# SamsungLabs/imvoxelnet

Hardware: AMD Instinct MI355X
Metric: images/sec/node (KITTI 3x384x1280, 216x248x12 vox) (higher is better)
Workload: dtype f32 (fp16 (hi, lo) pair MFMA operands: the Winograd-domain neck GEMMs and the chained 2-D trunk); 1 GPU; kitti_mono_1x3x384x1280_vox216x248x12_resnet50_fpn64_kittineck_anchor3dhead; batch_per_gpu=4, global_batch=4, parallelism=dp1, api=ImVoxelNet.simple_test(img, img_metas), detections_last_step=64

## Files before the change

imvoxelnet_amd/_lib.py:

```python
import ctypes as C
import os

_HERE = os.path.dirname(os.path.abspath(__file__))
LIB_PATH = os.environ.get('IVX_LIB_PATH') or os.path.join(_HERE, 'csrc', 'libimvoxel_hip.so')
_lib = None


class IvxError(RuntimeError):
    pass


class ConvDesc(C.Structure):
    _fields_ = [(n, C.c_int32) for n in
                ('B', 'D', 'H', 'W', 'Cin', 'Cout', 'KD', 'KH', 'KW', 'sd', 'sh', 'sw', 'pd', 'ph', 'pw',
                 'relu', 'res_mode', 'res_h', 'res_w', 'wgt_layout', 'out_mode', 'res_after_act')] + [('post_scale', C.c_float),
                                                                  ('in_dtype', C.c_int32), ('out_dtype', C.c_int32), ('res_scale', C.c_float),
                                                                  ('wino_operands', C.c_int32)]


class ConvRouteOpts(C.Structure):
    _fields_ = [(n, C.c_int32) for n in ('winograd', 'winograd_tile', 'wino_operands', 'split')] + [('winograd_min_pos', C.c_int64), ('winograd_2d_min_ch', C.c_int32)]


class ConvRoute(C.Structure):
# ... 22 lines not shown
                ('sampling', C.c_int32)]


SAMPLING = {'nearest': 0, 'bilinear': 1}


def sampling_id(sampling):
    try:
        return SAMPLING[sampling]
    except (KeyError, TypeError):
        raise ValueError(f"sampling must be 'nearest' or 'bilinear', got {sampling!r}") from None


class BackprojectDesc(C.Structure):
    _fields_ = [(n, C.c_int32) for n in ('B', 'V', 'FH', 'FW', 'C', 'X', 'Y', 'Z')] + [('voxel_size', C.c_float * 3)] + \
               [(n, C.c_int32) for n in ('feat_dtype', 'mode', 'sampling', 'first')]


class LiftLists(C.Structure):
    _fields_ = [('S', C.c_int32), ('R', C.c_int32), ('view_slot', C.c_void_p), ('row', C.c_void_p), ('first', C.c_void_p)]


class PairIO(C.Structure):
    _fields_ = [('in_scale', C.c_void_p), ('res_scale', C.c_void_p), ('res_dtype', C.c_int32), ('out_scale', C.c_void_p), ('amax_in', C.c_void_p),
                ('amax_res', C.c_void_p), ('amax_out', C.c_void_p), ('wbound', C.c_float), ('sbound', C.c_float)]


class BottleneckDesc(C.Structure):
    _fields_ = [(n, C.c_int32) for n in ('B', 'H', 'W', 'P')]


class BottleneckIO(C.Structure):
    _fields_ = [('in_scale', C.c_void_p), ('amax_in', C.c_void_p), ('out_scale', C.c_void_p), ('amax_out', C.c_void_p), ('wbound', C.c_float * 3),
                ('sbound', C.c_float * 3)]


class SampleMeta(C.Structure):
    _fields_ = [('intrinsic', C.c_float * 16), ('extrinsics', C.c_void_p), ('origin', C.c_float * 3), ('img_h', C.c_int32), ('img_w', C.c_int32),
                ('ori_h', C.c_int32)]


class IndoorTailDesc(C.Structure):
    _fields_ = [('B', C.c_int32), ('n_levels', C.c_int32), ('k', C.c_int32 * 4), ('n_classes', C.c_int32), ('n_reg', C.c_int32),
                ('use_rotate_nms', C.c_int32), ('max_num', C.c_int32), ('score_thr', C.c_float), ('nms_thr', C.c_float)]


class TraceRec(C.Structure):
    _fields_ = [('step', C.c_int32), ('stage', C.c_int32), ('is3d', C.c_int32), ('ms', C.c_float), ('start_ms', C.c_float), ('flops', C.c_double),
                ('bytes', C.c_double), ('name', C.c_char * 48)]


class PlanInfo(C.Structure):
    _fields_ = [(n, C.c_int64) for n in ('cam_bytes', 'arena', 'ws_off', 'ws_bytes', 'ws2_off', 'ws2_bytes', 'total', 'scal_off', 'scal_bytes')] + \
               [(n, C.c_int32) for n in ('slot_bytes', 'n_sides', 's0', 's1', 'n_steps', 'n_tensors')]


class PlanStep(C.Structure):
    _fields_ = [(n, C.c_int32) for n in ('kind', 'in_', 'res', 'out', 'out2', 'fuse_out', 'fuse', 'side', 'join', 'tile', 'pio', 'amax_n', 'amax_in_n',
                                         'n_extra_in', 'n_extra_out')] + \
               [('extra_in', C.c_int32 * 12), ('extra_out', C.c_int32 * 4)] + \
               [(n, C.c_int64) for n in ('split', 'ws', 'amax_out', 'amax_in')] + [('name', C.c_char * 48)]


class PlanTensor(C.Structure):
    _fields_ = [(n, C.c_int64) for n in ('off', 'bytes', 'used', 'slot')] + \
               [(n, C.c_int32) for n in ('first', 'last', 'fmt', 'esz', 'caller_owned', 'boundary')]


class ImagePrepDesc(C.Structure):
    _fields_ = [(n, C.c_int32) for n in ('src_h', 'src_w', 'src_row_bytes', 'dst_h', 'dst_w', 'pad_h', 'pad_w', 'to_rgb')] + \
               [('mean', C.c_float * 3), ('std', C.c_float * 3)]


def declare_plan_view(L):
    key = [C.c_void_p, C.c_char_p, C.c_int32, C.c_int32, C.c_int32, C.c_int32]
    L.ivx_model_plan_info.argtypes = key + [C.POINTER(PlanInfo)]
    L.ivx_model_plan_step.argtypes = key + [C.c_int32, C.POINTER(PlanStep)]
    L.ivx_model_plan_tensor.argtypes = key + [C.c_int32, C.POINTER(PlanTensor)]


EXPORTS = ['ivx_model_plan_info', 'ivx_model_plan_step', 'ivx_model_plan_tensor', 'ivx_bottleneck_proj_supported', 'ivx_bottleneck_proj_pack', 'ivx_bottleneck_proj_fwd_pio', 'ivx_anchor_head_decode', 'ivx_fcos3d_head_decode', 'ivx_nms_rotated_bev', 'ivx_nms_aligned3d', 'ivx_bottleneck_supported', 'ivx_bottleneck_fwd_pio', 'ivx_amax_f32', 'ivx_stem_pool_filter_bytes', 'ivx_stem_pool_pack_filters', 'ivx_stem_pool_out_dims', 'ivx_stem_pool_fwd_pair', 'ivx_conv_winograd_set_variant', 'ivx_ubench_mfma', 'ivx_ubench_copy', 'ivx_version', 'ivx_last_error', 'ivx_conv_out_dims', 'ivx_conv_fwd', 'ivx_conv_fwd_naive', 'ivx_conv_set_tile_override', 'ivx_conv_set_epilogue_mode', 'ivx_conv_set_plan_mode', 'ivx_topk_set_mode', 'ivx_conv_workspace_bytes', 'ivx_conv_fwd_ws', 'ivx_conv_set_halo_mode', 'ivx_bf16_pair_split', 'ivx_f16_pair_split', 'ivx_conv_pair_supported', 'ivx_bf16_pair_pack_filters', 'ivx_conv_route', 'ivx_conv_pio_workspace_bytes', 'ivx_conv_fwd_pio', 'ivx_conv_fwd_pio_naive', 'ivx_pair_pack_filters', 'ivx_nchw_to_nhwc_amax', 'ivx_maxpool2d_fwd_pair', 'ivx_f16_pair_merge', 'ivx_model_calibrate_fp8', 'ivx_model_calibrate_fp8_ex', 'ivx_amax_bf16', 'ivx_conv_winograd_output_blocks', 'ivx_conv_winograd_issued_fraction', 'ivx_conv_winograd_output_amax', 'ivx_conv_winograd_input_amax', 'ivx_conv_winograd_fused_supported', 'ivx_conv_winograd_fused_blocks', 'ivx_conv_winograd_gemm_output_amax',
           'ivx_conv_winograd_bg_supported', 'ivx_conv_winograd_bg_bytes', 'ivx_conv_winograd_bg_layer_offset', 'ivx_conv_winograd_bg_plan',
           'ivx_conv_winograd_input_bg', 'ivx_conv_winograd_gemm_bg', 'ivx_conv_winograd_output_bg',
           'ivx_conv_winograd_supported', 'ivx_conv_winograd_weight_elems', 'ivx_conv_winograd_weights', 'ivx_conv_winograd_workspace_bytes',
           'ivx_conv_winograd_input', 'ivx_conv_winograd_gemm', 'ivx_conv_winograd_output', 'ivx_conv_winograd_fwd',
           'ivx_maxpool2d_fwd', 'ivx_maxpool2d_fwd_bf16', 'ivx_maxpool2d_fwd_fp8', 'ivx_global_avgpool_fwd', 'ivx_global_avgpool_fwd_bf16', 'ivx_upsample_trilinear2x_fwd', 'ivx_dcn_im2col_fwd', 'ivx_dcn_im2col_fwd_bf16', 'ivx_dcn_im2col_fwd_pair', 'ivx_nchw_to_nhwc', 'ivx_image_s2d_bf16', 'ivx_nhwc_to_nchw', 'ivx_backproject_mean_fwd', 'ivx_backproject_mean_fwd_amax', 'ivx_backproject_amax_blocks', 'ivx_backproject_mean_fwd_bf16', 'ivx_upsample_trilinear2x_fwd_bf16', 'ivx_backproject_sum_fwd', 'ivx_volume_normalize_fwd',
           'ivx_backproject_accum_fwd', 'ivx_backproject_accum_fwd_bf16', 'ivx_volume_mean_fwd', 'ivx_backproject_fwd_ex', 'ivx_backproject_gather_fwd',
           'ivx_backproject_lists_fwd',
           'ivx_anchor_head_workspace_bytes', 'ivx_anchor_head_get_bboxes', 'ivx_fcos_head_workspace_bytes',
           'ivx_fcos_head_level_candidates', 'ivx_nms_workspace_bytes',
           'ivx_nms_bev', 'ivx_boxes_overlap_bev', 'ivx_aligned_3d_nms', 'ivx_aligned_3d_nms_workspace_bytes', 'ivx_aligned_3d_nms_ws', 'ivx_multiclass_nms_workspace_bytes', 'ivx_multiclass_nms_bev',
           'ivx_create', 'ivx_destroy', 'ivx_weights_load', 'ivx_weights_finalize', 'ivx_model_workspace_bytes', 'ivx_model_forward',
           'ivx_backbone_fpn_workspace_bytes', 'ivx_backbone_fpn_fwd', 'ivx_neck3d_workspace_bytes', 'ivx_neck3d_out_dims',
           'ivx_neck3d_kitti_fwd', 'ivx_neck3d_nuscenes_fwd', 'ivx_neck3d_levels', 'ivx_neck3d_fast_fwd', 'ivx_neck3d_unet_fwd',
           'ivx_model_forward_levels', 'ivx_model_anchors', 'ivx_compute_projection', 'ivx_voxel_new_origin', 'ivx_fold_batchnorm',
           'ivx_model_trace', 'ivx_model_trace_count', 'ivx_model_trace_read',
           'ivx_model_detect_workspace_bytes', 'ivx_model_max_detections', 'ivx_model_detect', 'ivx_layout_head_decode', 'ivx_layout_extrinsics',
           'ivx_indoor_tail_workspace_bytes', 'ivx_indoor_tail_get_bboxes',
           'ivx_rescale_size', 'ivx_image_prep_u8',
           'ivx_kitti_image_box_overlap', 'ivx_kitti_compute_statistics', 'ivx_kitti_collect_scores', 'ivx_kitti_fused_statistics']


def lib():
    global _lib
    if _lib is not None:
        return _lib
    if not os.path.exists(LIB_PATH):
        raise IvxError(f'{LIB_PATH} is missing: build it with `python -m imvoxelnet_amd._build` '
                       '(or __graft_entry__.build()).  There is no CPU fallback.')
    L = C.CDLL(LIB_PATH)
    vp, i32, i64, f32 = C.c_void_p, C.c_int32, C.c_int64, C.c_float
    L.ivx_version.restype = C.c_int
    L.ivx_last_error.restype = C.c_char_p
    L.ivx_conv_out_dims.argtypes = [C.POINTER(ConvDesc), C.POINTER(i32), C.POINTER(i32), C.POINTER(i32)]
    for name in ('ivx_conv_fwd', 'ivx_conv_fwd_naive'):
        getattr(L, name).argtypes = [C.POINTER(ConvDesc), vp, vp, vp, vp, vp, vp, vp]
    L.ivx_conv_set_tile_override.argtypes = [C.c_int]
    L.ivx_conv_set_halo_mode.argtypes = [C.c_int]
    L.ivx_conv_set_epilogue_mode.argtypes = [C.c_int]
    L.ivx_conv_set_plan_mode.argtypes = [C.c_int]
    L.ivx_conv_winograd_output_blocks.argtypes = [C.POINTER(ConvDesc), i32]
    L.ivx_conv_winograd_output_blocks.restype = i32
    L.ivx_conv_winograd_output_amax.argtypes = [C.POINTER(ConvDesc), i32, vp, vp, vp, vp, vp, i64, vp, vp]
    L.ivx_conv_winograd_input_amax.argtypes = [C.POINTER(ConvDesc), i32, vp, vp, i64, vp, i32, vp]
    L.ivx_conv_winograd_fused_supported.argtypes = [C.POINTER(ConvDesc), i32]
    L.ivx_conv_winograd_fused_blocks.argtypes = [C.POINTER(ConvDesc), i32]
    L.ivx_conv_winograd_fused_blocks.restype = i32
    L.ivx_conv_winograd_gemm_output_amax.argtypes = [C.POINTER(ConvDesc), i32, vp, vp, vp, vp, vp, vp, i64, vp, vp]
    L.ivx_conv_winograd_bg_supported.argtypes = [C.POINTER(ConvDesc), i32]
    L.ivx_conv_winograd_bg_bytes.argtypes = [C.POINTER(ConvDesc), i32]
    L.ivx_conv_winograd_bg_bytes.restype = i64
    L.ivx_conv_winograd_bg_layer_offset.argtypes = [C.POINTER(ConvDesc), i32]
    L.ivx_conv_winograd_bg_layer_offset.restype = i64
    L.ivx_conv_winograd_bg_plan.argtypes = [C.POINTER(ConvDesc), vp, i32, C.POINTER(i32), vp, i64, vp]
    L.ivx_conv_winograd_input_bg.argtypes = [C.POINTER(ConvDesc), i32, vp, vp, i64, vp, i32, vp, vp]
    L.ivx_conv_winograd_gemm_bg.argtypes = [C.POINTER(ConvDesc), i32, vp, vp, i64, vp, vp]
    L.ivx_conv_winograd_output_bg.argtypes = [C.POINTER(ConvDesc), i32, vp, vp, vp, vp, vp, i64, vp, vp, vp]
    L.ivx_bf16_pair_split.argtypes = [vp, i64, vp, vp]
    L.ivx_f16_pair_split.argtypes = [vp, i64, f32, vp, vp]
    L.ivx_conv_pair_supported.argtypes = [C.POINTER(ConvDesc)]
    L.ivx_bf16_pair_pack_filters.argtypes = [vp, i32, i32, i32, i32, vp]
    L.ivx_conv_route.argtypes = [C.POINTER(ConvDesc), i32, C.POINTER(ConvRouteOpts), C.POINTER(ConvRoute)]
    L.ivx_conv_pio_workspace_bytes.argtypes = [C.POINTER(ConvDesc), C.POINTER(PairIO)]
    L.ivx_conv_pio_workspace_bytes.restype = i64
    L.ivx_amax_f32.argtypes = [vp, i64, vp, vp]
    L.ivx_stem_pool_filter_bytes.restype = i64
    L.ivx_stem_pool_filter_bytes.argtypes = []
    L.ivx_stem_pool_pack_filters.argtypes = [vp, vp, vp, vp]
    L.ivx_stem_pool_out_dims.argtypes = [i32, i32, C.POINTER(i32), C.POINTER(i32)]
    L.ivx_stem_pool_fwd_pair.argtypes = [vp, i32, i32, i32, vp, vp, vp, f32, f32, vp, vp, vp, vp, vp]
    L.ivx_bottleneck_supported.argtypes = [C.POINTER(BottleneckDesc)]
    L.ivx_bottleneck_fwd_pio.argtypes = [C.POINTER(BottleneckDesc), C.POINTER(BottleneckIO)] + [vp] * 12
    L.ivx_bottleneck_proj_supported.argtypes = [C.POINTER(BottleneckDesc), i32]
    L.ivx_bottleneck_proj_pack.argtypes = [vp, vp, vp, vp, vp, vp, i32, i32, vp, vp, vp, C.POINTER(f32), C.POINTER(f32), C.POINTER(f32)]
    L.ivx_bottleneck_proj_fwd_pio.argtypes = [C.POINTER(BottleneckDesc), i32, C.POINTER(BottleneckIO), f32] + [vp] * 12
    L.ivx_conv_fwd_pio.argtypes = [C.POINTER(ConvDesc), C.POINTER(PairIO), vp, vp, vp, vp, vp, vp, vp, i64, vp]
    L.ivx_conv_fwd_pio_naive.argtypes = [C.POINTER(ConvDesc), C.POINTER(PairIO), vp, vp, vp, vp, vp, vp, vp]
    L.ivx_pair_pack_filters.argtypes = [vp, i32, i32, i32, vp, vp, vp, vp, C.POINTER(f32), C.POINTER(f32)]
    L.ivx_nchw_to_nhwc_amax.argtypes = [vp, i32, i32, i64, i32, vp, vp, vp]
    L.ivx_maxpool2d_fwd_pair.argtypes = [vp, i32, i32, i32, i32, i32, i32, i32, vp, vp, f32, f32, vp, vp, vp]
    L.ivx_f16_pair_merge.argtypes = [vp, i64, vp, vp, vp]
    L.ivx_conv_workspace_bytes.argtypes = [C.POINTER(ConvDesc)]
    L.ivx_conv_workspace_bytes.restype = i64
    L.ivx_conv_fwd_ws.argtypes = [C.POINTER(ConvDesc), vp, vp, vp, vp, vp, vp, vp, i64, vp]
    D = C.POINTER(ConvDesc)
    L.ivx_conv_winograd_supported.argtypes = [D, i32]
    L.ivx_conv_winograd_issued_fraction.argtypes = [D]
    L.ivx_conv_winograd_issued_fraction.restype = C.c_float
    L.ivx_conv_winograd_weight_elems.argtypes = [D, i32]
    L.ivx_conv_winograd_weight_elems.restype = i64
    L.ivx_conv_winograd_weights.argtypes = [D, i32, vp, vp, vp]
    L.ivx_conv_winograd_workspace_bytes.argtypes = [D, i32]
    L.ivx_conv_winograd_workspace_bytes.restype = i64
    L.ivx_conv_winograd_input.argtypes = [D, i32, vp, vp, i64, vp]
    L.ivx_conv_winograd_gemm.argtypes = [D, i32, vp, vp, i64, vp]
    L.ivx_conv_winograd_output.argtypes = [D, i32, vp, vp, vp, vp, vp, i64, vp]
    L.ivx_conv_winograd_fwd.argtypes = [D, i32, vp, vp, vp, vp, vp, vp, vp, i64, vp]
    L.ivx_maxpool2d_fwd.argtypes = [vp, i32, i32, i32, i32, i32, i32, i32, vp, vp]
    L.ivx_global_avgpool_fwd.argtypes = [vp, i32, i64, i32, vp, vp]
    L.ivx_global_avgpool_fwd_bf16.argtypes = [vp, i32, i64, i32, vp, vp]
    L.ivx_upsample_trilinear2x_fwd.argtypes = [vp, i32, i32, i32, i32, i32, vp, vp]
    L.ivx_dcn_im2col_fwd.argtypes = [vp, vp] + [i32] * 10 + [vp, vp]
    L.ivx_dcn_im2col_fwd_bf16.argtypes = [vp, vp] + [i32] * 10 + [vp, vp]
    L.ivx_dcn_im2col_fwd_pair.argtypes = [vp, vp, vp] + [i32] * 10 + [vp, vp, vp, vp]
    L.ivx_nchw_to_nhwc.argtypes = [vp, i32, i32, i64, i32, vp, vp]
    L.ivx_nhwc_to_nchw.argtypes = [vp, i32, i64, i32, vp, vp]
    L.ivx_rescale_size.argtypes = [i32, i32, i32, i32, C.POINTER(i32), C.POINTER(i32)]
    L.ivx_image_prep_u8.argtypes = [C.POINTER(ImagePrepDesc), vp, i64, i32, vp, vp]
    L.ivx_backproject_mean_fwd.argtypes = [vp, i32, i32, i32, i32, i32, vp, vp, vp, C.POINTER(f32), i32, i32, i32,
                                           vp, vp, vp]
    L.ivx_backproject_sum_fwd.argtypes = L.ivx_backproject_mean_fwd.argtypes
    L.ivx_backproject_mean_fwd_bf16.argtypes = L.ivx_backproject_mean_fwd.argtypes
    L.ivx_upsample_trilinear2x_fwd_bf16.argtypes = [vp, i32, i32, i32, i32, i32, vp, vp]
    L.ivx_volume_normalize_fwd.argtypes = [vp, vp, i64, i32, vp, vp]
    L.ivx_backproject_accum_fwd.argtypes = [vp, i32, i32, i32, i32, i32, vp, vp, vp, C.POINTER(f32), i32, i32, i32, vp, vp, i32, vp, vp, vp]
    L.ivx_backproject_accum_fwd_bf16.argtypes = L.ivx_backproject_accum_fwd.argtypes
    L.ivx_volume_mean_fwd.argtypes = [vp, vp, i64, i32, vp, i32, vp, vp]
    if hasattr(L, 'ivx_backproject_fwd_ex'):
        L.ivx_backproject_fwd_ex.argtypes = [C.POINTER(BackprojectDesc), vp, vp, vp, vp, vp, vp, vp, vp, vp]
    if hasattr(L, 'ivx_backproject_gather_fwd'):
        L.ivx_backproject_gather_fwd.argtypes = [C.POINTER(BackprojectDesc), i32, vp, vp, vp, vp, vp, vp, vp, vp]
    if hasattr(L, 'ivx_backproject_lists_fwd'):
        L.ivx_backproject_lists_fwd.argtypes = [C.POINTER(BackprojectDesc), C.POINTER(LiftLists), vp, vp, vp, vp, vp, vp, vp, vp, vp]
    L.ivx_anchor_head_workspace_bytes.argtypes = [C.POINTER(AnchorHeadDesc)]
    L.ivx_anchor_head_workspace_bytes.restype = i64
    L.ivx_anchor_head_get_bboxes.argtypes = [C.POINTER(AnchorHeadDesc), vp, vp, vp, i64, vp, vp, vp, vp, vp, vp, vp, vp]
    L.ivx_fcos_head_workspace_bytes.argtypes = [i32, i32, i32]
    L.ivx_fcos_head_workspace_bytes.restype = i64
    L.ivx_fcos_head_level_candidates.argtypes = [vp, vp, vp, vp, f32] + [i32] * 12 + [vp, i64, vp, vp, vp, vp]
    L.ivx_nms_workspace_bytes.argtypes = [i32]
    L.ivx_nms_workspace_bytes.restype = i64
    L.ivx_nms_bev.argtypes = [vp, i32, f32, i32, vp, i64, vp, vp, vp]
    L.ivx_boxes_overlap_bev.argtypes = [vp, i32, vp, i32, i32, vp, vp]
    L.ivx_aligned_3d_nms.argtypes = [vp, vp, vp, i32, f32, vp, vp, vp]
    L.ivx_aligned_3d_nms_workspace_bytes.argtypes = [i32]
    L.ivx_aligned_3d_nms_workspace_bytes.restype = i64
    L.ivx_aligned_3d_nms_ws.argtypes = [vp, vp, vp, i32, f32, vp, i64, vp, vp, vp]
    L.ivx_multiclass_nms_workspace_bytes.argtypes = [i32, i32]
    L.ivx_multiclass_nms_workspace_bytes.restype = i64
    L.ivx_multiclass_nms_bev.argtypes = [vp, vp, i32, i32, i32, f32, f32, i32, i32, vp, i64, vp, vp, vp, vp]
# ... 59 lines not shown
```

imvoxelnet_amd/csrc/api_common.cpp:

```cpp
#include <stdarg.h>
#include <stdio.h>
#include <string.h>

#include "../../include/imvoxel.h"

static thread_local char g_err[512] = "";

void ivx_set_error(const char *fmt, ...) {
  va_list ap;
  va_start(ap, fmt);
  vsnprintf(g_err, sizeof(g_err), fmt, ap);
  va_end(ap);
}

extern "C" int ivx_version(void) { return 470;  }
extern "C" const char *ivx_last_error(void) { return g_err; }

extern "C" __attribute__((weak)) int ivx_dcn_im2col_fwd_bf16(const void *, const float *, int32_t, int32_t, int32_t, int32_t, int32_t, int32_t, int32_t,
                                                             int32_t, int32_t, int32_t, void *, ivx_stream_t) {
  ivx_set_error("ivx_dcn_im2col_fwd_bf16: bf16 storage is not available in this build");
  return IVX_ERR_UNSUPPORTED;
}
extern "C" __attribute__((weak)) int ivx_global_avgpool_fwd_bf16(const void *, int32_t, int64_t, int32_t, float *, ivx_stream_t) {
  ivx_set_error("ivx_global_avgpool_fwd_bf16: bf16 storage is not available in this build");
  return IVX_ERR_UNSUPPORTED;
}

extern "C" __attribute__((weak)) int ivx_backproject_fwd_ex(const ivx_backproject_desc *, const void *, const float *, const float *, const int32_t *, void *,
                                                            int32_t *, void *, uint8_t *, ivx_stream_t) {
  ivx_set_error("ivx_backproject_fwd_ex: bilinear sampling is not available in this build");
  return IVX_ERR_UNSUPPORTED;
}

extern "C" int ivx_anchor_head_decode(const ivx_anchor_head_desc *d, const float *head_out, const float *anchors, void *workspace, int64_t workspace_bytes,
                                      float *out_boxes, float *out_scores, int64_t *out_labels, int32_t *out_count, int64_t *cand_idx, float *cand_boxes,
                                      float *cand_scores, ivx_stream_t stream) {
  return ivx_anchor_head_get_bboxes(d, head_out, anchors, workspace, workspace_bytes, out_boxes, out_scores, out_labels, out_count, cand_idx, cand_boxes,
                                    cand_scores, stream);
}
extern "C" int ivx_fcos3d_head_decode(const float *head_out, const uint8_t *valid0, const float *level_vs, const float *level_new_origin, float scale,
                                      int32_t B, int32_t nx, int32_t ny, int32_t nz, int32_t CH, int32_t n_classes, int32_t n_reg, int32_t level, int32_t X,
                                      int32_t Y, int32_t Z, int32_t nms_pre, void *workspace, int64_t workspace_bytes, float *cand_boxes,
                                      float *cand_scores, int32_t *cand_count, ivx_stream_t stream) {
  return ivx_fcos_head_level_candidates(head_out, valid0, level_vs, level_new_origin, scale, B, nx, ny, nz, CH, n_classes, n_reg, level, X, Y, Z, nms_pre,
                                        workspace, workspace_bytes, cand_boxes, cand_scores, cand_count, stream);
}
extern "C" int ivx_nms_rotated_bev(const float *boxes_sorted, int32_t n, float thresh, void *workspace, int64_t workspace_bytes, int64_t *keep,
                                   int32_t *num_out, ivx_stream_t stream) {
  return ivx_nms_bev(boxes_sorted, n, thresh, 1, workspace, workspace_bytes, keep, num_out, stream);
}
extern "C" int ivx_nms_aligned3d(const float *boxes, const float *scores, const int64_t *classes, int32_t n, float thresh, int64_t *pick,
                                 int32_t *num_out, ivx_stream_t stream) {
  return ivx_aligned_3d_nms(boxes, scores, classes, n, thresh, pick, num_out, stream);
}

static const int WINO_MIN_CH = 64;
static const int WINO_2D_MIN_CH = 128;
static const int64_t WINO_MIN_POS = 2000;
static const int64_t WINO_TILE6_MIN_PLANE = 16384;
static const int SPLIT_MIN_COUT = 64;
static const int64_t SPLIT_MIN_POS = 256;
static const int WINO_OVER_PAIR_MIN_CH = 256;
static const int64_t WINO_OVER_PAIR_MIN_POS = 200000;

static int32_t wino_operands(const ivx_conv_desc *d, int32_t cin_real, const ivx_conv_route_opts *o, int tile) {
  return tile >= 4 && o->wino_operands == IVX_F16_PAIR && cin_real % (d->wgt_layout == 1 ? 32 : 16) == 0 ? IVX_F16_PAIR : 0;
}

extern "C" int ivx_conv_route(const ivx_conv_desc *d, int32_t cin_real, const ivx_conv_route_opts *o, ivx_conv_route_out *r) {
  if (!d || !o || !r) {
    ivx_set_error("ivx_conv_route: null argument");
    return IVX_ERR_INVALID_ARG;
  }
  memset(r, 0, sizeof(*r));
  r->run = *d;
  const bool f32 = d->in_dtype == IVX_F32 && d->out_dtype == IVX_F32 && d->Cin == cin_real;
  const bool wino2d = d->KD == 1 && d->KH == 3 && d->KW == 3 && d->sd == 1 && d->sh == 1 && d->sw == 1;
  const bool wino3d = d->KD == 3 && d->KH == 3 && d->sd == 1 && d->sh == 1;
  const int min_ch = !wino2d ? WINO_MIN_CH : o->winograd_2d_min_ch > 0 ? o->winograd_2d_min_ch : WINO_2D_MIN_CH;
  r->wino_candidate = f32 && (wino2d || wino3d) && d->Cout % 4 == 0 && cin_real % 4 == 0 && (cin_real >= min_ch || d->Cout >= min_ch);
  r->split_candidate = f32 && o->split && o->wino_operands == IVX_F16_PAIR && d->KD == 3 && d->KH == 3 && d->KW == 3 && cin_real % 32 == 0 &&
                       d->Cout >= SPLIT_MIN_COUT;
  ivx_conv_desc w = *d;
  if (r->wino_candidate && wino2d) {
    w.D = d->H; w.H = d->W; w.W = d->B > 0 ? 1 : 0;
    w.KD = 3; w.KH = 3; w.KW = 1;
    w.pd = d->ph; w.ph = d->pw; w.pw = 0;
  }
  if (d->B <= 0) {
    r->run = w;
    r->run.wino_operands = wino_operands(d, cin_real, o, o->winograd_tile);
    return IVX_OK;
  }
  const int64_t npos = (int64_t)d->B * d->D * d->H * d->W;
  r->prefers_winograd = r->wino_candidate && wino2d && o->winograd && o->wino_operands == IVX_F16_PAIR && cin_real >= WINO_OVER_PAIR_MIN_CH &&
                        d->Cout >= WINO_OVER_PAIR_MIN_CH && cin_real % 32 == 0 && npos >= WINO_OVER_PAIR_MIN_POS;
  if (r->wino_candidate && o->winograd && (d->res_mode == 0 || d->res_mode == 1) &&
      npos >= (o->winograd_min_pos >= 0 ? o->winograd_min_pos : WINO_MIN_POS)) {
// ... 58 lines not shown
```

imvoxelnet_amd/csrc/model.cpp:

```cpp
#include <hip/hip_runtime_api.h>
#include <math.h>
#include <stdarg.h>
#include <string.h>

#include <algorithm>
#include <cstdlib>
#include <map>
#include <memory>
#include <string>
#include <vector>

#include "../../include/imvoxel.h"
#include "../../include/imvoxel_lab.h"

void ivx_set_error(const char *fmt, ...);

extern "C" {
__attribute__((weak)) int ivx_conv_winograd_bg_supported(const ivx_conv_desc *d, int32_t tile);
__attribute__((weak)) int64_t ivx_conv_winograd_bg_bytes(const ivx_conv_desc *d, int32_t n_layers);
__attribute__((weak)) int64_t ivx_conv_winograd_bg_layer_offset(const ivx_conv_desc *d, int32_t layer);
__attribute__((weak)) int ivx_conv_winograd_bg_plan(const ivx_conv_desc *d, const uint8_t *valid, int32_t n_layers, const int32_t *out_slices, void *block,
                                                    int64_t block_bytes, ivx_stream_t stream);
__attribute__((weak)) int ivx_conv_winograd_input_bg(const ivx_conv_desc *d, int32_t tile, const void *in, void *workspace, int64_t workspace_bytes,
                                                     const float *partials, int32_t n_partials, const int32_t *bg, ivx_stream_t stream);
__attribute__((weak)) int ivx_conv_winograd_gemm_bg(const ivx_conv_desc *d, int32_t tile, const float *u, void *workspace, int64_t workspace_bytes,
                                                    const int32_t *bg, ivx_stream_t stream);
__attribute__((weak)) int ivx_conv_winograd_output_bg(const ivx_conv_desc *d, int32_t tile, const float *scale, const float *shift, const void *res,
                                                      void *out, void *workspace, int64_t workspace_bytes, float *partials, const int32_t *bg,
                                                      ivx_stream_t stream);
}

#define M_REQUIRE(cond, ...)        \
  do {                              \
    if (!(cond)) {                  \
      ivx_set_error(__VA_ARGS__);   \
      return IVX_ERR_INVALID_ARG;   \
    }                               \
  } while (0)
#define M_HIP(call, what)                                                        \
  do {                                                                           \
    hipError_t e_ = (call);                                                      \
    if (e_ != hipSuccess) {                                                      \
      ivx_set_error("%s: %s", what, hipGetErrorString(e_));                      \
      return IVX_ERR_HIP;                                                        \
    }                                                                            \
  } while (0)
#define M_TRY(call)                 \
  do {                              \
    int rc_ = (call);               \
    if (rc_ != IVX_OK) return rc_;  \
  } while (0)

namespace {

inline int64_t align256(int64_t v) { return (v + 255) / 256 * 256; }

inline uint16_t f32_to_f16_bits(float f) {
  uint32_t x;
  memcpy(&x, &f, 4);
  const uint32_t sign = (x >> 16) & 0x8000u, ax = x & 0x7fffffffu;
  if (ax >= 0x7f800000u) return (uint16_t)(sign | (ax > 0x7f800000u ? 0x7e00u : 0x7c00u));
  if (ax < 0x38800000u) {
    float a;
    memcpy(&a, &ax, 4);
    const float r = a * 16777216.0f;
    return (uint16_t)(sign | (uint32_t)lrintf(r));
  }
  const uint32_t mant = ax & 0x7fffffu, exp = (ax >> 23) - 127 + 15;
  uint32_t h = (exp << 10) | (mant >> 13);
  const uint32_t rem = mant & 0x1fffu;
  if (rem > 0x1000u || (rem == 0x1000u && (h & 1u))) ++h;
  return (uint16_t)(sign | h);
}
inline uint16_t f32_to_bf16_bits(float f) {
  uint32_t x;
  memcpy(&x, &f, 4);
  if ((x & 0x7fffffffu) > 0x7f800000u) return (uint16_t)((x >> 16) | 0x40u);
  x += 0x7fffu + ((x >> 16) & 1u);
  return (uint16_t)(x >> 16);
}
inline float f16_bits_to_f32(uint16_t h) {
  const uint32_t sign = (uint32_t)(h & 0x8000u) << 16, e = (h >> 10) & 31u, m = h & 0x3ffu;
  float f;
  if (e == 0) {
    f = (float)m * 5.9604644775390625e-08f;
    uint32_t x;
    memcpy(&x, &f, 4);
    x |= sign;
    memcpy(&f, &x, 4);
    return f;
  }
  const uint32_t x = sign | (e == 31 ? 0x7f800000u | (m << 13) : ((e - 15 + 127) << 23) | (m << 13));
  memcpy(&f, &x, 4);
  return f;
}

struct HostTensor {
  std::vector<int64_t> shape;
  std::vector<float> data;
};

struct ConvLayer {
  std::string name;
  int dims = 3;
  int cin = 0, cout = 0;
  int k[3] = {1, 1, 1}, s[3] = {1, 1, 1}, p[3] = {0, 0, 0};
  bool relu = false;
  bool conv_t = false;
  bool dcn_cols = false;
  int cout_zero = 0;
  bool linear = false;
  std::vector<std::string> w_keys;
  std::vector<std::string> b_keys;
  std::string bn;
  int cin_pad = 0, layout = 0;
  bool wino_cand = false, identity_epilogue = true;
  float *w = nullptr, *w0 = nullptr, *scale = nullptr, *shift = nullptr;
  std::map<int, float *> u;
  bool stem_s2d = false;
  bool out_f32 = false;
  bool f32 = false;
  int fp8_role = 0;
  int stage = -1;
  int fp8_eff = 0;
  std::vector<float> w_tap, scale_h, shift_h;
  float *wq = nullptr, *scale_q = nullptr, *shift_q = nullptr;
  int layout_q = 0;
  double out_scale_q = 1.0;
  bool pair_ok = false;
  float *wpair = nullptr, *scale_p = nullptr;
  bool split_cand = false;
  float *wsplit = nullptr;
  float wbound = 0.f, sbound = 0.f;
  int proj_peer = -1;
  bool proj_keep = false;
  float *wproj = nullptr, *scale_proj = nullptr, *shift_proj = nullptr;
  float proj_wb3 = 0.f, proj_sb = 0.f, proj_wbd = 0.f;
  float *wstem = nullptr;
};

enum StepKind { ST_IMG2CL, ST_IMG_S2D, ST_CONV, ST_MAXPOOL, ST_LIFT, ST_TAIL, ST_UPSAMPLE, ST_DCN_COL, ST_AVGPOOL, ST_LAYOUT, ST_FCOS, ST_INDOOR_TAIL };

struct Step {
  StepKind kind;
  int layer = -1;
  int in = -1, res = -1, out = -1, out2 = -1;
  int res_mode = 0;
  int res_after_act = 0;
  float post_scale = 1.0f;
  int aux = 0;
};

struct TInfo {
  int B = 0, D = 0, H = 0, W = 0, C = 0;
  int64_t bytes = 0, off = -1;
  int first = -1, last = -1;
  bool raw = false;
  int esz = 4;
  int fmt = 0;
  int64_t slot = -1;
  int64_t elems() const { return (int64_t)B * D * H * W * C; }
};

struct PlanStep {
  ivx_conv_desc d;
  int tile = 0;
  int64_t ws = 0;
  int64_t amax_out = -1, amax_in = -1;
  int amax_n = 0, amax_in_n = 0;
  int pio = 0;
  int64_t split = 0;
  int bound_layer = -1;
  int fuse = 0, fuse_out = -1;
  int side = 0, join = 0;
  int64_t bg = -1;
};

struct Plan {
  std::vector<TInfo> t;
  std::vector<PlanStep> ps;
  int64_t arena = 0, ws_off = 0, ws_bytes = 0, tail_ws = 0, total = 0;
  ivx_anchor_head_desc tail;
  int64_t cam_bytes = 0, cam_proj = 0, cam_origin = 0, cam_crop = 0, cam_lvl_vs[3] = {0, 0, 0}, cam_lvl_no[3] = {0, 0, 0};
  int n_views = 1;
  ivx_indoor_tail_desc itail;
  int max_det = 0;
  int64_t scal_off = 0, scal_bytes = 0;
  int64_t ws2_off = 0, ws2_bytes = 0;
  int n_sides = 0;
  int s0 = 0, s1 = 0;
  int bg_first = -1, bg_layers = 0;
  int64_t bg_off = -1, bg_bytes = 0;
  int32_t bg_zo[9] = {0, 0, 0, 0, 0, 0, 0, 0, 0};
};

}

struct ivx_model {
  ivx_model_cfg cfg;
  std::vector<ConvLayer> layers;
  std::vector<Step> steps;
  int n_tensors = 0;
  int trunk0 = 0, trunk1 = 0, lift_step = -1, neck0 = 0, neck1 = 0, head_step = -1, tail_step = -1;
  int t_img = -1, t_fpn0 = -1, t_volume = -1, t_valid = -1, t_neck = -1, t_head = -1;
  std::vector<int> t_levels;
  int head0 = -1;
  std::vector<int> t_headout, t_cb, t_cs, t_cc;
  float head_scales[3] = {1.f, 1.f, 1.f};
  int t_c5 = -1, t_angle = -1, t_layout = -1, layout_step = -1;
  std::vector<std::vector<char>> cam_ring;
  size_t cam_next = 0;
  std::map<std::string, HostTensor> weights;
  bool finalized = false;
  std::vector<float> anchors_host;
  int anchors_h = 0, anchors_w = 0;
  float *anchors_dev = nullptr;
  size_t anchors_cap = 0;
  std::vector<float> anchors_given;
  std::map<std::string, std::unique_ptr<Plan>> plans;
  std::vector<void *> owned;
  std::vector<float> pack_a, pack_b;
  bool fp8_on = false;
  float *calib_dev = nullptr;
  bool trace_on = false;
  bool trace_skip = false;
  int trace_level = 2;
  struct TraceRec {
    int step, stage, is3d; double flops, bytes; hipEvent_t e0, e1; std::string name;
    const int32_t *rows_dev = nullptr;
    double rows_dense = 0.0;
  };
  std::vector<TraceRec> trace;
  std::vector<hipEvent_t> event_pool;
  size_t events_used = 0;
  hipStream_t side = nullptr;
  hipEvent_t ev_fork = nullptr;
  std::vector<hipEvent_t> ev_join;
};

namespace {

int new_tensor(ivx_model *m) { return m->n_tensors++; }

int add_conv(ivx_model *m, ConvLayer L, int in, int res = -1, int res_mode = 0) {
  m->layers.push_back(std::move(L));
  Step s;
  s.kind = ST_CONV;
  s.layer = (int)m->layers.size() - 1;
  s.in = in;
  s.res = res;
  s.res_mode = res >= 0 ? (res_mode ? res_mode : 1) : 0;
  s.out = new_tensor(m);
  m->steps.push_back(s);
  return s.out;
}

ConvLayer conv2d(const std::string &name, int cin, int cout, int k, int stride, int pad, bool relu, const std::string &w,
                 const std::string &b, const std::string &bn) {
  ConvLayer L;
  L.name = name; L.dims = 2; L.cin = cin; L.cout = cout;
  L.k[0] = 1; L.k[1] = k; L.k[2] = k;
  L.s[0] = 1; L.s[1] = stride; L.s[2] = stride;
  L.p[0] = 0; L.p[1] = pad; L.p[2] = pad;
  L.relu = relu; L.w_keys = {w}; L.b_keys = {b}; L.bn = bn;
  return L;
}

ConvLayer conv3d(const std::string &name, int cin, int cout, const int s[3], const int p[3], bool relu, const std::string &w,
                 const std::string &b, const std::string &bn) {
  ConvLayer L;
  L.name = name; L.dims = 3; L.cin = cin; L.cout = cout;
  for (int a = 0; a < 3; ++a) { L.k[a] = 3; L.s[a] = s[a]; L.p[a] = p[a]; }
  L.relu = relu; L.w_keys = {w}; L.b_keys = {b}; L.bn = bn;
  return L;
}

// ... 791 lines not shown
      if (!(pl->ps[i].pio && pl->ps[i + 1].pio && pl->ps[i + 2].pio) || s1.res >= 0 || s2.res >= 0 || s2.in != s1.out || s3.in != s2.out ||
          s3.res != s1.in || s3.res_mode != 1 || s3.res_after_act || s3.post_scale != 1.0f)
        continue;
      if (!is1x1(L1) || !is1x1(L3) || !(L2.k[0] == 1 && L2.k[1] == 3 && L2.k[2] == 3 && L2.s[1] == 1 && L2.s[2] == 1 && L2.p[1] == 1 && L2.p[2] == 1) ||
          L2.dcn_cols || !L1.relu || !L2.relu || !L3.relu || L1.cin != 4 * P || L2.cin != P || L2.cout != P || L3.cin != P || L3.cout != 4 * P)
        continue;
      if (x.fmt != IVX_F16_PAIR || y1.fmt != IVX_F16_PAIR || y2.fmt != IVX_F16_PAIR || o.fmt != IVX_F16_PAIR || x.D != 1 || x.slot < 0 || o.slot < 0 ||
          y1.last != i + 1 || y2.last != i + 2)
        continue;
      ivx_bottleneck_desc bd = {x.B, x.H, x.W, P};
      if (!ivx_bottleneck_supported(&bd)) continue;
      pl->ps[i].fuse = 1; pl->ps[i].fuse_out = s3.out;
      pl->ps[i + 1].fuse = pl->ps[i + 2].fuse = 2;
      pl->t[s3.out].first = i;
      i += 2;
    }
  static const bool side_on = !(getenv("IVX_SIDE_STREAM") && atoi(getenv("IVX_SIDE_STREAM")) == 0);
  if (side_on && c.with_trunk)
    for (int i = std::max(r.s0, m->trunk0); i + 2 < std::min(r.s1, m->trunk1); ++i) {
      const Step &s0 = m->steps[i];
      if (s0.kind != ST_CONV || pl->ps[i].tile != 0 || pl->ps[i].fuse != 0 || s0.res >= 0) continue;
      const std::string &nm = m->layers[s0.layer].name;
      if (nm.size() < 10 || nm.compare(nm.size() - 10, 10, "downsample") != 0) continue;
      int j = -1;
      for (int k = i + 1; k < std::min(r.s1, m->trunk1) && k <= i + 6; ++k)
        if (m->steps[k].res == s0.out) { j = k; break; }
      if (j < 0 || j < i + 2) continue;
      bool ok = true;
      for (int k = i + 1; k < j && ok; ++k) ok = m->steps[k].in != s0.out && m->steps[k].res != s0.out && pl->ps[k].side == 0 && pl->ps[k].join == 0;
      if (!ok) continue;
      pl->ps[i].side = pl->ps[j].join = ++pl->n_sides;
      pl->t[s0.in].last = std::max(pl->t[s0.in].last, j);
    }
  std::vector<int> keep = {m->t_fpn0, m->t_volume, m->t_valid, m->t_neck, m->t_head, m->t_angle, m->t_layout};
  keep.insert(keep.end(), m->t_levels.begin(), m->t_levels.end());
  for (int t : keep)
    if (t >= 0 && pl->t[t].first >= r.s0) pl->t[t].last = r.s1;
  struct Blk { int64_t off, size; };
  std::vector<Blk> free_list;
  int64_t top = 0;
  {
    const TInfo &vol = pl->t[m->t_volume];
    const int Bs = vol.B > 0 ? vol.B : 1;
    auto take = [&](int64_t bytes) { const int64_t at = top; top += align256(bytes); return at; };
    pl->n_views = n_views;
    pl->cam_proj = take((int64_t)Bs * n_views * 12 * 4);
    pl->cam_origin = take((int64_t)Bs * 3 * 4);
    pl->cam_crop = take((int64_t)Bs * 2 * 4);
    for (int l = 0; l < 3; ++l) { pl->cam_lvl_vs[l] = take((int64_t)Bs * 3 * 4); pl->cam_lvl_no[l] = take((int64_t)Bs * 3 * 4); }
    pl->cam_bytes = top;
  }
  auto release = [&](int64_t off, int64_t size) {
    free_list.push_back({off, size});
    std::sort(free_list.begin(), free_list.end(), [](const Blk &a, const Blk &b) { return a.off < b.off; });
    std::vector<Blk> merged;
    for (const Blk &b : free_list) {
      if (!merged.empty() && merged.back().off + merged.back().size == b.off) merged.back().size += b.size;
      else merged.push_back(b);
    }
    free_list.swap(merged);
  };
  for (int i = r.s0; i < r.s1; ++i) {
    const Step &s = m->steps[i];
    const int extra = s.kind == ST_FCOS ? m->t_cc[s.aux] : pl->ps[i].fuse_out;
    for (int t : {s.out, s.out2, extra}) {
      if (t < 0 || pl->t[t].first != i) continue;
      TInfo &ti = pl->t[t];
      bool placed = false;
      for (size_t f = 0; f < free_list.size(); ++f)
        if (free_list[f].size >= ti.bytes) {
          ti.off = free_list[f].off;
          free_list[f].off += ti.bytes; free_list[f].size -= ti.bytes;
          if (free_list[f].size == 0) free_list.erase(free_list.begin() + f);
          placed = true;
          break;
        }
      if (!placed) { ti.off = top; top += ti.bytes; }
    }
    for (int t = 0; t < m->n_tensors; ++t) {
      TInfo &ti = pl->t[t];
      if (ti.off >= 0 && ti.first >= r.s0 && ti.last == i && ti.first != -2) release(ti.off, ti.bytes);
    }
  }
  for (int i = r.s0; i < r.s1; ++i) {
    const Step &s = m->steps[i];
    PlanStep &pc = pl->ps[i];
    if (s.kind != ST_CONV || pc.tile == 0 || pc.d.wino_operands != IVX_F16_PAIR) continue;
    for (int j = i - 1; j >= r.s0; --j) {
      const Step &q = m->steps[j];
      if (q.out != s.in) continue;
      PlanStep &pp = pl->ps[j];
      if (q.kind == ST_LIFT && m->cfg.sampling == IVX_SAMPLE_NEAREST) {
        const TInfo &vol = pl->t[q.out];
        const int32_t nb = ivx_backproject_amax_blocks(vol.B, n_views, vol.D, vol.H, vol.W);
        if (nb > 0) {
          if (pp.amax_out < 0) { pp.amax_out = top; pp.amax_n = nb; top += align256((int64_t)nb * 4); }
          pc.amax_in = pp.amax_out;
          pc.amax_in_n = pp.amax_n;
        }
      }
      if (q.kind == ST_CONV && pp.tile > 0) {
        if (pp.amax_out < 0) {
          const int32_t nb = ivx_conv_winograd_output_blocks(&pp.d, pp.tile);
          M_REQUIRE(nb > 0, "layer %s: %s", m->layers[q.layer].name.c_str(), ivx_last_error());
          pp.amax_out = top;
          pp.amax_n = nb;
          top += align256((int64_t)nb * 4);
        }
        pc.amax_in = pp.amax_out;
        pc.amax_in_n = pp.amax_n;
      }
      break;
    }
  }
  const bool bg_on = !(getenv("IVX_NECK_BACKGROUND") && atoi(getenv("IVX_NECK_BACKGROUND")) == 0);
  if (bg_on && ivx_conv_winograd_bg_plan && ivx_conv_winograd_bg_supported && m->lift_step >= r.s0 && m->lift_step < r.s1 && c.storage == IVX_F32) {
    std::vector<int> chain_t = {m->steps[m->lift_step].out};
    std::vector<int> chain_s;
    for (int i = m->lift_step + 1; i < r.s1 && (int)chain_s.size() < 9; ++i) {
      const Step &s = m->steps[i];
      const PlanStep &ps = pl->ps[i];
      if (s.kind != ST_CONV || s.in != chain_t.back() || ps.tile != 6 || !ivx_conv_winograd_bg_supported(&ps.d, ps.tile)) break;
      if (s.res >= 0 && (s.res_mode != 1 || std::find(chain_t.begin(), chain_t.end(), s.res) == chain_t.end())) break;
      if (!chain_s.empty()) {
        const ivx_conv_desc &d0 = pl->ps[chain_s[0]].d;
        if (ps.d.B != d0.B || ps.d.D != d0.D || ps.d.H != d0.H) break;
      }
      int32_t xo, yo, zo;
      M_TRY(ivx_conv_out_dims(&ps.d, &xo, &yo, &zo));
      pl->bg_zo[chain_s.size()] = zo;
      chain_s.push_back(i);
      chain_t.push_back(s.out);
    }
    if (!chain_s.empty()) {
      const ivx_conv_desc &d0 = pl->ps[chain_s[0]].d;
      pl->bg_first = chain_s[0];
      pl->bg_layers = (int)chain_s.size();
      pl->bg_bytes = ivx_conv_winograd_bg_bytes(&d0, pl->bg_layers);
      M_REQUIRE(pl->bg_bytes > 0, "background plan: %s", ivx_last_error());
      top = align256(top);
      pl->bg_off = top;
      top += align256(pl->bg_bytes);
      for (size_t l = 0; l < chain_s.size(); ++l) pl->ps[chain_s[l]].bg = pl->bg_off + ivx_conv_winograd_bg_layer_offset(&d0, (int32_t)l);
    }
  }
  if (n_slots > 0) {
    top = align256(top);
    pl->scal_off = top;
    pl->scal_bytes = (int64_t)n_slots * 512;
    top += pl->scal_bytes;
  }
  pl->arena = align256(top);
  pl->ws_off = pl->arena;
  pl->ws_bytes = align256(pl->ws_bytes);
  pl->total = pl->arena + pl->ws_bytes;
  if (pl->n_sides > 0) {
    for (int i = r.s0; i < r.s1; ++i)
      if (pl->ps[i].side > 0) pl->ws2_bytes = std::max(pl->ws2_bytes, pl->ps[i].ws);
    pl->ws2_bytes = align256(pl->ws2_bytes);
    pl->ws2_off = pl->total;
    pl->total += pl->ws2_bytes;
  }
  return IVX_OK;
}

std::string plan_key(const char *what, int B, int V, int H, int W) {
  char buf[96];
  snprintf(buf, sizeof(buf), "%s:%d:%d:%d:%d", what, B, V, H, W);
  return buf;
}

TInfo tinfo(int B, int D, int H, int W, int C, int esz = 4) {
  TInfo t; t.B = B; t.D = D; t.H = H; t.W = W; t.C = C; t.esz = esz; t.bytes = align256(t.elems() * esz);
  return t;
}

int get_plan(ivx_model *m, const char *what, Range r, int B, int V, int H, int W, const std::map<int, TInfo> &inputs, Plan **out,
             hipStream_t stream) {
  M_REQUIRE(m->finalized, "%s: call ivx_weights_finalize first", what);
  const std::string key = plan_key(what, B, V, H, W);
  auto it = m->plans.find(key);
  if (it == m->plans.end()) {
    std::unique_ptr<Plan> pl(new Plan());
    M_TRY(make_plan(m, r, inputs, V, pl.get(), stream));
    it = m->plans.emplace(key, std::move(pl)).first;
  }
  *out = it->second.get();
  return IVX_OK;
}

struct Bind {
  std::map<int, void *> ext;
  const float *proj = nullptr, *new_origin = nullptr;
  const int32_t *crop = nullptr;
  int V = 1;
  float *boxes = nullptr, *scores = nullptr;
  int64_t *labels = nullptr;
  int32_t *count = nullptr;
  const float *lvl_vs[3] = {nullptr, nullptr, nullptr}, *lvl_no[3] = {nullptr, nullptr, nullptr};
  const ivx_sample_meta *metas = nullptr;
  float *proj_dev = nullptr;
  float *angles_host = nullptr, *layout_host = nullptr;
};

int trace_begin(ivx_model *m, int step, int stage, int is3d, double flops, double bytes, const std::string &name, hipStream_t st) {
  if (!m->trace_on) return IVX_OK;
  m->trace_skip = m->trace_level == 3 && stage != 2;
  if (m->trace_skip) return IVX_OK;
  while (m->event_pool.size() < m->events_used + 2) {
    hipEvent_t e;
    M_HIP(hipEventCreate(&e), "hipEventCreate");
    m->event_pool.push_back(e);
  }
  ivx_model::TraceRec r{step, stage, is3d, flops, bytes, m->event_pool[m->events_used], m->event_pool[m->events_used + 1], name};
  m->events_used += 2;
  M_HIP(hipEventRecord(r.e0, st), "hipEventRecord");
  m->trace.push_back(r);
  return IVX_OK;
}

int trace_end(ivx_model *m, hipStream_t st) {
  if (!m->trace_on || m->trace_skip) return IVX_OK;
  M_HIP(hipEventRecord(m->trace.back().e1, st), "hipEventRecord");
  return IVX_OK;
}

int ensure_anchors(ivx_model *m, const ivx_anchor_head_desc &d, hipStream_t st, const char *who) {
  if (m->anchors_h == d.H && m->anchors_w == d.W && m->anchors_dev) return IVX_OK;
  const size_t n = (size_t)d.H * d.W * d.num_anchors * 7;
  if (!m->anchors_given.empty()) {
    M_REQUIRE(m->anchors_given.size() == n, "%s: the loaded anchors have %zu values, the %d x %d grid needs %zu", who, m->anchors_given.size(),
              d.H, d.W, n);
    m->anchors_host = m->anchors_given;
  } else {
    make_anchors(m->cfg, d.H, d.W, &m->anchors_host);
  }
  M_HIP(hipStreamSynchronize(st), "hipStreamSynchronize (anchors)");
  if (m->anchors_dev && m->anchors_cap < n) {
    auto it = std::find(m->owned.begin(), m->owned.end(), (void *)m->anchors_dev);
    if (it != m->owned.end()) m->owned.erase(it);
    (void)hipFree(m->anchors_dev);
    m->anchors_dev = nullptr;
  }
  if (!m->anchors_dev) {
    void *p = nullptr;
    M_HIP(hipMalloc(&p, std::max<size_t>(n, 1) * sizeof(float)), "hipMalloc (anchors)");
    m->owned.push_back(p);
    m->anchors_dev = (float *)p;
    m->anchors_cap = n;
  }
  M_HIP(hipMemcpyAsync(m->anchors_dev, m->anchors_host.data(), n * sizeof(float), hipMemcpyHostToDevice, st), "hipMemcpyAsync (anchors)");
  M_HIP(hipStreamSynchronize(st), "hipStreamSynchronize (anchors)");
  m->anchors_h = d.H; m->anchors_w = d.W;
  return IVX_OK;
}

int run_steps(ivx_model *m, const Plan &pl, Range r, const Bind &bd, void *workspace, int64_t workspace_bytes, hipStream_t st,
              const char *who) {
  M_REQUIRE(workspace && ((uintptr_t)workspace & 255) == 0, "%s: workspace must be non-null and 256-byte aligned", who);
  if (workspace_bytes < pl.total) {
    ivx_set_error("%s: workspace too small (%lld < %lld); size it with the matching *_workspace_bytes call", who, (long long)workspace_bytes,
                  (long long)pl.total);
    return IVX_ERR_WORKSPACE;
  }
  char *base = (char *)workspace;
  void *ws = base + pl.ws_off;
  auto ptr = [&](int t) -> void * {
    auto it = bd.ext.find(t);
    if (it != bd.ext.end()) return it->second;
    return base + pl.t[t].off;
  };
  auto slotp = [&](int t) -> uint32_t * { return (t >= 0 && pl.t[t].slot >= 0) ? (uint32_t *)(base + pl.scal_off + pl.t[t].slot * 512) : nullptr; };
  auto scalep = [&](int t) -> float * { uint32_t *q = slotp(t); return q ? (float *)(q + IVX_AMAX_SLOTS) : nullptr; };
  if (pl.scal_bytes > 0 && r.s0 <= m->trunk0 && r.s1 > m->trunk0)
    M_HIP(hipMemsetAsync(base + pl.scal_off, 0, (size_t)pl.scal_bytes, st), "hipMemsetAsync (amax slots)");
  auto wino_input = [&](const PlanStep &ps, const void *in) -> int {
    const float *part = ps.amax_in >= 0 ? (const float *)(base + ps.amax_in) : nullptr;
    if (ps.bg >= 0) return ivx_conv_winograd_input_bg(&ps.d, ps.tile, in, ws, pl.ws_bytes, part, ps.amax_in_n, (const int32_t *)(base + ps.bg), st);
    return ivx_conv_winograd_input_amax(&ps.d, ps.tile, in, ws, pl.ws_bytes, part, ps.amax_in_n, st);
  };
  auto wino_gemm = [&](const PlanStep &ps, const ConvLayer &L) -> int {
    const float *u = L.u.at(ps.tile * 8 + ps.d.wino_operands);
    if (ps.bg >= 0) return ivx_conv_winograd_gemm_bg(&ps.d, ps.tile, u, ws, pl.ws_bytes, (const int32_t *)(base + ps.bg), st);
    return ivx_conv_winograd_gemm(&ps.d, ps.tile, u, ws, pl.ws_bytes, st);
  };
  auto wino_output = [&](const PlanStep &ps, const ConvLayer &L, const void *res, void *out) -> int {
    float *part = ps.amax_out >= 0 ? (float *)(base + ps.amax_out) : nullptr;
    if (ps.bg >= 0) return ivx_conv_winograd_output_bg(&ps.d, ps.tile, L.scale, L.shift, res, out, ws, pl.ws_bytes, part, (const int32_t *)(base + ps.bg), st);
    return ivx_conv_winograd_output_amax(&ps.d, ps.tile, L.scale, L.shift, res, out, ws, pl.ws_bytes, part, st);
  };
  auto bg_plan = [&](const Step &lift) -> int {
    if (pl.bg_first < 0) return IVX_OK;
    return ivx_conv_winograd_bg_plan(&pl.ps[pl.bg_first].d, (const uint8_t *)ptr(lift.out2), pl.bg_layers, pl.bg_zo, base + pl.bg_off, pl.bg_bytes, st);
  };
  const bool span2d = m->trace_on && m->trace_level == 1 && m->cfg.with_trunk;
  std::vector<char> forked((size_t)std::max(pl.n_sides, 1), 0);
  double span_flops = 0.0, span_bytes = 0.0;
  for (int i = r.s0; i < r.s1; ++i) {
    const Step &s = m->steps[i];
    const TInfo &in = pl.t[s.in];
    const bool in_span = span2d && i >= m->trunk0 && i < m->trunk1;
    if (in_span && i == m->trunk0) M_TRY(trace_begin(m, i, 6, 0, 0.0, 0.0, "2-D trunk (ResNet-50 + FPN level 0)", st));
    const bool was_on = m->trace_on;
    if (in_span) {
      m->trace_on = false;
      {
        const PlanStep &ps = pl.ps[i];
        auto tb = [&](int t) { return t >= 0 ? (double)pl.t[t].elems() * pl.t[t].esz : 0.0; };
        if (s.kind == ST_CONV && ps.fuse != 2) {
          const ConvLayer &L = m->layers[s.layer];
          if (ps.fuse == 1) {
            const ConvLayer &L2 = m->layers[m->steps[i + 1].layer], &L3 = m->layers[m->steps[i + 2].layer];
            span_bytes += tb(s.in) + tb(ps.fuse_out) + 4.0 * ((double)L.cout * L.cin + 9.0 * L2.cout * L2.cin + (double)L3.cout * L3.cin);
          } else if (ps.fuse == 5) {
            const ConvLayer &L2 = m->layers[m->steps[i + 1].layer], &L3 = m->layers[m->steps[i + 2].layer];
            span_bytes += tb(s.in) + tb(ps.fuse_out) + 4.0 * ((double)L.cout * L.cin + 9.0 * L2.cout * L2.cin + (double)L3.cout * (L3.cin + L.cin));
          } else {
            span_bytes += tb(s.in) + tb(s.out) + tb(s.res) + (double)pl.t[s.in].esz * L.cout * L.cin_pad * L.k[0] * L.k[1] * L.k[2];
          }
        } else if (s.kind == ST_MAXPOOL && ps.fuse == 4) {
          span_bytes += tb(s.out) + tb(m->t_img);
        } else if (s.kind == ST_IMG2CL && ps.fuse == 3) {
          span_bytes += tb(s.in);
        } else if (s.kind != ST_CONV && s.kind != ST_LAYOUT) {
          span_bytes += tb(s.in) + tb(s.out) + tb(s.res);
        }
      }
      if (s.kind == ST_CONV) {
        const PlanStep &ps = pl.ps[i];
        const TInfo &o = pl.t[s.out];
        const ConvLayer &L = m->layers[s.layer];
        if (ps.tile) {
          int32_t a_, b_, zo;
          M_TRY(ivx_conv_out_dims(&ps.d, &a_, &b_, &zo));
          const int n = ps.tile + 2;
          const double tiles = (double)o.B * ((ps.d.D + 2 * ps.d.pd - 2 + ps.tile - 1) / ps.tile) * ((ps.d.H + 2 * ps.d.ph - 2 + ps.tile - 1) / ps.tile);
          span_flops += (ps.d.wino_operands ? 3.0 : 1.0) * ivx_conv_winograd_issued_fraction(&ps.d) * 2.0 * n * n * tiles * zo * ps.d.Cout * ps.d.KW * ps.d.Cin;
        } else {
          span_flops += ((ps.pio || (ps.fuse == 2 && L.wstem)) ? 3.0 : 1.0) * 2.0 * o.elems() * L.cin * L.k[0] * L.k[1] * L.k[2];
        }
      }
    }
    struct Restore { ivx_model *m; bool on; ~Restore() { m->trace_on = on; } } restore{m, was_on};
    switch (s.kind) {
      case ST_IMG2CL:
        if (pl.ps[i].fuse == 3) {
          M_TRY(ivx_amax_f32((const float *)ptr(s.in), in.elems(), slotp(s.out), st));
          break;
        }
        if (slotp(s.out))
          M_TRY(ivx_nchw_to_nhwc_amax((const float *)ptr(s.in), in.B, 3, (int64_t)in.H * in.W, 4, (float *)ptr(s.out), slotp(s.out), st));
        else
          M_TRY(ivx_nchw_to_nhwc((const float *)ptr(s.in), in.B, 3, (int64_t)in.H * in.W, 4, (float *)ptr(s.out), st));
        break;
      case ST_IMG_S2D:
        M_TRY(ivx_image_s2d_bf16((const float *)ptr(s.in), in.B, in.H, in.W, ptr(s.out), st));
        break;
      case ST_MAXPOOL:
        if (m->cfg.storage == IVX_BF16) {
          M_TRY(ivx_maxpool2d_fwd_bf16(ptr(s.in), in.B, in.H, in.W, in.C, 3, 2, 1, ptr(s.out), st));
          break;
        }
        if (pl.ps[i].pio) {
          const ConvLayer &Ls = m->layers[pl.ps[i].bound_layer];
          int t_img4 = -1;
          for (int j = r.s0; j < i; ++j)
            if (m->steps[j].out == s.in) t_img4 = m->steps[j].in;
          M_REQUIRE(slotp(t_img4), "internal: the pair max-pool needs the image's amax slots");
          if (pl.ps[i].fuse == 4) {
            int t_img = -1;
            for (int j = r.s0; j < i; ++j)
              if (m->steps[j].out == t_img4) t_img = m->steps[j].in;
            M_REQUIRE(t_img >= 0, "internal: the one-launch stem needs the image");
            const TInfo &im = pl.t[t_img];
            const double px = (double)in.elems() / in.C;
// ... 1004 lines not shown
```

imvoxelnet_amd/csrc/winograd.hip:

```cpp
#include "ivx_common.h"
#include <stdlib.h>
int ivx_conv_launch_fold4w(const _Float16 *V, long long vs, const _Float16 *U, long long us, int M, int Cin_stored, int Cout, int Z, const IvxWinoFold &f,
                           hipStream_t st);

int ivx_conv_grouped_launch(const ivx_conv_desc *d, int groups, const float *in, long long g_in, const float *wgt, long long g_w,
                            float *out, long long g_out, hipStream_t st, const unsigned *cp_src, unsigned *cp_dst, const int *m_dev);
int ivx_conv_grouped_rows_dev_ok(const ivx_conv_desc *d, int groups);
int ivx_conv_grouped_fold4(const ivx_conv_desc *d, int groups, const float *in, long long g_in, const float *wgt, long long g_w, const IvxWinoFold *f,
                           hipStream_t st);
int ivx_conv_fold4_blocks(long long M, int Cout);

namespace {

constexpr int WINO_BG_HDR = 4;

struct WinoP {
  const float *in, *scale, *shift, *res;
  float *out;
  float *V, *Mw;
  long long vs, ms;
  int B, X, Y, Z, C;
  int Xo, Yo, Zo, Co;
  int TX, TY;
  int px, py;
  int relu, res_mode, res_after_act;
  float post_scale;
  float *pmax;
  const unsigned *hdr;
  const int *bg;
#ifdef IVX_CONV_TIMELINE
  unsigned long long *tl;
#endif
};
#ifdef IVX_CONV_TIMELINE
#define WINO_TL_BEGIN const unsigned long long wtl0 = __builtin_amdgcn_s_memrealtime();
#define WINO_TL_END(p)                                                                                              \
  if ((p).tl && threadIdx.x == 0) {                                                                                \
    unsigned long long *t_ = (p).tl + (size_t)blockIdx.x * 8;                                                       \
    t_[0] = wtl0; t_[1] = wtl0; t_[2] = wtl0; t_[3] = __builtin_amdgcn_s_memrealtime();                             \
    t_[4] = __builtin_amdgcn_s_getreg(63492); t_[5] = __builtin_amdgcn_s_getreg(63508);                             \
  }
#else
#define WINO_TL_BEGIN
#define WINO_TL_END(p)
#endif

__device__ __forceinline__ bool wino_amax_bad(const float amax) { return !(amax < 3.0e38f); }
__device__ __forceinline__ float wino_pow2_scale(const float amax, const float gain_log2) {
  if (wino_amax_bad(amax)) return 0.00390625f;
  if (!(amax > 0.f)) return 1.0f;
  int e;
  (void)frexpf(amax, &e);
  int k = 15 - (int)gain_log2 - e;
  k = k < -120 ? -120 : (k > 120 ? 120 : k);
  return ldexpf(1.0f, k);
}
__device__ __forceinline__ float wino_pair_vscale(const unsigned *hdr) { return wino_pow2_scale(__uint_as_float(hdr[0]), 8.f); }
__device__ __forceinline__ float wino_mscale(const unsigned *hdr) { return hdr ? 1.0f / (wino_pair_vscale(hdr) * __uint_as_float(hdr[1])) : 1.0f; }

__device__ __forceinline__ float vabsmax(const float v) { return fabsf(v); }
__device__ __forceinline__ float vabsmax(const float2 v) { return fmaxf(fabsf(v.x), fabsf(v.y)); }
__device__ __forceinline__ float vabsmax(const float4 v) { return fmaxf(fmaxf(fabsf(v.x), fabsf(v.y)), fmaxf(fabsf(v.z), fabsf(v.w))); }
__device__ __forceinline__ void wino_block_max_store(float m, float *pmax) {
#pragma unroll
  for (int o = 32; o > 0; o >>= 1) m = fmaxf(m, __shfl_xor(m, o));
  __shared__ float wmax[4];
  if ((threadIdx.x & 63) == 0) wmax[threadIdx.x >> 6] = m;
  __syncthreads();
  if (threadIdx.x == 0) pmax[blockIdx.x] = fmaxf(fmaxf(wmax[0], wmax[1]), fmaxf(wmax[2], wmax[3]));
}
__global__ __launch_bounds__(256) void wino_amax_partials_kernel(const float *__restrict__ part, int n, unsigned *out) {
  float m = 0.f;
  for (int t = blockIdx.x * blockDim.x + threadIdx.x; t < n; t += gridDim.x * blockDim.x) m = fmaxf(m, part[t]);
#pragma unroll
  for (int o = 32; o > 0; o >>= 1) m = fmaxf(m, __shfl_xor(m, o));
  if ((threadIdx.x & 63) == 0) atomicMax(out, __float_as_uint(m));
}

__global__ __launch_bounds__(1024) void wino_amax_partials_write_kernel(const float *__restrict__ part, int n, unsigned *out) {
  __shared__ float red[16];
  float m = 0.f;
  for (int t = threadIdx.x; t < n; t += 1024) m = fmaxf(m, part[t]);
#pragma unroll
  for (int o = 32; o > 0; o >>= 1) m = fmaxf(m, __shfl_xor(m, o));
  if ((threadIdx.x & 63) == 0) red[threadIdx.x >> 6] = m;
  __syncthreads();
  if (threadIdx.x < 64) {
    m = threadIdx.x < 16 ? red[threadIdx.x] : 0.f;
#pragma unroll
    for (int o = 8; o > 0; o >>= 1) m = fmaxf(m, __shfl_xor(m, o));
    if (threadIdx.x == 0) *out = __float_as_uint(m);
  }
}

typedef float wf32x4 __attribute__((ext_vector_type(4)));
__device__ __forceinline__ float wino_amax4(const wf32x4 v, const float m) {
  return fmaxf(fmaxf(m, fmaxf(fabsf(v[0]), fabsf(v[1]))), fmaxf(fabsf(v[2]), fabsf(v[3])));
}
__global__ __launch_bounds__(256) void wino_amax_kernel(const wf32x4 *__restrict__ x, size_t n4, unsigned *out) {
  float m = 0.f;
  const size_t stride = (size_t)gridDim.x * blockDim.x;
  size_t t = (size_t)blockIdx.x * blockDim.x + threadIdx.x;
  for (; t + 3 * stride < n4; t += 4 * stride) {
    const wf32x4 a = __builtin_nontemporal_load(x + t), b = __builtin_nontemporal_load(x + t + stride);
    const wf32x4 c = __builtin_nontemporal_load(x + t + 2 * stride), d = __builtin_nontemporal_load(x + t + 3 * stride);
    m = wino_amax4(d, wino_amax4(c, wino_amax4(b, wino_amax4(a, m))));
  }
  for (; t < n4; t += stride) m = wino_amax4(__builtin_nontemporal_load(x + t), m);
#pragma unroll
  for (int o = 32; o > 0; o >>= 1) m = fmaxf(m, __shfl_xor(m, o));
  __shared__ float wmax[4];
  if ((threadIdx.x & 63) == 0) wmax[threadIdx.x >> 6] = m;
  __syncthreads();
  if (threadIdx.x == 0) atomicMax(out, __float_as_uint(fmaxf(fmaxf(wmax[0], wmax[1]), fmaxf(wmax[2], wmax[3]))));
}

__global__ __launch_bounds__(256) void wino_pair_inplace_kernel(float *buf, size_t n16, unsigned *hdr) {
  const float s = wino_pow2_scale(__uint_as_float(hdr[0]), 0.f);
  const size_t t = (size_t)blockIdx.x * blockDim.x + threadIdx.x;
  if (t == 0) hdr[1] = __float_as_uint(s);
  if (t >= n16) return;
  float4 v[4];
#pragma unroll
  for (int q = 0; q < 4; ++q) v[q] = reinterpret_cast<const float4 *>(buf)[4 * t + q];
  typedef _Float16 h8 __attribute__((ext_vector_type(8)));
  h8 hi[2], lo[2];
#pragma unroll
  for (int q = 0; q < 4; ++q) {
    const float x[4] = {v[q].x, v[q].y, v[q].z, v[q].w};
#pragma unroll
    for (int e = 0; e < 4; ++e) {
      const float y = __builtin_fminf(__builtin_fmaxf(x[e] * s, -65504.f), 65504.f);
      const _Float16 h = (_Float16)y;
      hi[q >> 1][(q & 1) * 4 + e] = h;
      lo[q >> 1][(q & 1) * 4 + e] = (_Float16)(y - (float)h);
    }
  }
  h8 *o = reinterpret_cast<h8 *>(buf + 16 * t);
  o[0] = hi[0]; o[1] = hi[1]; o[2] = lo[0]; o[3] = lo[1];
}

template <int W> struct VecT;
template <> struct VecT<4> { typedef float4 T; };
template <> struct VecT<2> { typedef float2 T; };
template <> struct VecT<1> { typedef float T; };
__device__ __forceinline__ float vzero(float *) { return 0.f; }
__device__ __forceinline__ float vone(float *) { return 1.f; }
__device__ __forceinline__ float4 vzero(float4 *) { return make_float4(0.f, 0.f, 0.f, 0.f); }
__device__ __forceinline__ float2 vzero(float2 *) { return make_float2(0.f, 0.f); }
__device__ __forceinline__ float4 vone(float4 *) { return make_float4(1.f, 1.f, 1.f, 1.f); }
__device__ __forceinline__ float2 vone(float2 *) { return make_float2(1.f, 1.f); }
__device__ __forceinline__ float4 operator+(float4 a, float4 b) { return make_float4(a.x + b.x, a.y + b.y, a.z + b.z, a.w + b.w); }
// ... 36 lines not shown
  static __device__ __forceinline__ void out(const V (&m)[6], V (&y)[4]) {
    const V s1 = m[1] + m[2], d1 = m[1] - m[2], s2 = m[3] + m[4], d2 = m[3] - m[4];
    y[0] = (m[0] + s1) + s2;
    y[1] = d1 + 2.0f * d2;
    y[2] = s1 + 4.0f * s2;
    y[3] = (d1 + 8.0f * d2) + m[5];
  }
  static __device__ __forceinline__ void wgt(const float (&g)[3], float (&u)[6]) {
    u[0] = 0.25f * g[0];
    u[1] = (-1.0f / 6.0f) * (g[0] + g[1] + g[2]);
    u[2] = (-1.0f / 6.0f) * (g[0] - g[1] + g[2]);
    u[3] = (1.0f / 24.0f) * g[0] + (1.0f / 12.0f) * g[1] + (1.0f / 6.0f) * g[2];
    u[4] = (1.0f / 24.0f) * g[0] - (1.0f / 12.0f) * g[1] + (1.0f / 6.0f) * g[2];
    u[5] = g[2];
  }
};

template <typename V> struct Wino1D<6, V> {
  static __device__ __forceinline__ void in(const V (&d)[8], V (&t)[8]) {
    t[0] = (d[0] - d[6]) + 5.25f * (d[4] - d[2]);
    t[7] = (d[7] - d[1]) + 5.25f * (d[3] - d[5]);
    const V a12 = (d[2] + d[6]) - 4.25f * d[4], b12 = (d[1] + d[5]) - 4.25f * d[3];
    t[1] = a12 + b12;
    t[2] = a12 - b12;
    const V a34 = (d[6] + 0.25f * d[2]) - 1.25f * d[4], b34 = (0.5f * d[1] - 2.5f * d[3]) + 2.0f * d[5];
    t[3] = a34 + b34;
    t[4] = a34 - b34;
    const V a56 = d[6] + 4.0f * (d[2] - 1.25f * d[4]), b56 = (2.0f * d[1] - 2.5f * d[3]) + 0.5f * d[5];
    t[5] = a56 + b56;
    t[6] = a56 - b56;
  }
  static __device__ __forceinline__ void out(const V (&m)[8], V (&y)[6]) {
    const V sa = m[1] + m[2], da = m[1] - m[2], sb = m[3] + m[4], db = m[3] - m[4], sc = m[5] + m[6], dc = m[5] - m[6];
    y[0] = ((m[0] + sa) + sb) + sc;
    y[1] = (da + 2.0f * db) + 0.5f * dc;
    y[2] = (sa + 4.0f * sb) + 0.25f * sc;
    y[3] = (da + 8.0f * db) + 0.125f * dc;
    y[4] = (sa + 16.0f * sb) + 0.0625f * sc;
    y[5] = ((da + 32.0f * db) + 0.03125f * dc) + m[7];
  }
  static __device__ __forceinline__ void wgt(const float (&g)[3], float (&u)[8]) {
    u[0] = g[0];
    u[1] = (-2.0f / 9.0f) * (g[0] + g[1] + g[2]);
    u[2] = (-2.0f / 9.0f) * (g[0] - g[1] + g[2]);
    u[3] = (1.0f / 90.0f) * g[0] + (1.0f / 45.0f) * g[1] + (2.0f / 45.0f) * g[2];
    u[4] = (1.0f / 90.0f) * g[0] - (1.0f / 45.0f) * g[1] + (2.0f / 45.0f) * g[2];
    u[5] = (32.0f / 45.0f) * g[0] + (16.0f / 45.0f) * g[1] + (8.0f / 45.0f) * g[2];
    u[6] = (32.0f / 45.0f) * g[0] - (16.0f / 45.0f) * g[1] + (8.0f / 45.0f) * g[2];
    u[7] = g[2];
  }
};

typedef _Float16 wf16x2 __attribute__((ext_vector_type(2)));
typedef unsigned u32x2w __attribute__((ext_vector_type(2)));
__device__ __forceinline__ float wino_sat16(const float x) {
  return (x > 65504.f && x < __builtin_inff()) ? 65504.f : ((x < -65504.f && x > -__builtin_inff()) ? -65504.f : x);
}
__device__ __forceinline__ void wino_pair2(const float2 v, const float s, unsigned *hi, unsigned *lo, const bool sat = false) {
  float x0 = v.x * s, x1 = v.y * s;
  if (sat) { x0 = wino_sat16(x0); x1 = wino_sat16(x1); }
  wf16x2 h, l;
  h[0] = (_Float16)x0;
  h[1] = (_Float16)x1;
  l[0] = (_Float16)(x0 - (float)h[0]);
  l[1] = (_Float16)(x1 - (float)h[1]);
  *hi = __builtin_bit_cast(unsigned, h);
  *lo = __builtin_bit_cast(unsigned, l);
}

template <int MT, int VW, int PAIR = 0>
__global__ __launch_bounds__(256) void wino_input_kernel(const WinoP p) {
  WINO_TL_BEGIN
  typedef typename VecT<VW>::T V;
  constexpr int N = MT + 2;
  static_assert(!PAIR || VW == 2, "pair operands: two channels per lane (one dword of hi, one of lo)");
  const int CV = p.C / VW;
  const long long per_tile = (long long)p.Z * CV;
  const int *lst = p.bg ? p.bg + WINO_BG_HDR : nullptr;
  const long long total = (lst ? (long long)p.bg[0] : (long long)p.B * p.TX * p.TY) * per_tile;
  const V *in = reinterpret_cast<const V *>(p.in);
  V *Vw = reinterpret_cast<V *>(p.V);
  const float vscale = PAIR ? wino_pair_vscale(p.hdr) : 1.0f;
  const bool sat = PAIR ? wino_amax_bad(__uint_as_float(p.hdr[0])) : false;
  for (long long t = (long long)blockIdx.x * blockDim.x + threadIdx.x; t < total; t += (long long)gridDim.x * blockDim.x) {
    const long long zc = t % per_tile;
    long long q = t / per_tile;
    if (lst) q = lst[q];
    const int ty = (int)(q % p.TY);
    q /= p.TY;
    const int tx = (int)(q % p.TX);
    const int b = (int)(q / p.TX);
    const int x0 = MT * tx - p.px, y0 = MT * ty - p.py;
    V w[N][N];
#pragma unroll
    for (int j = 0; j < N; ++j) {
      const int y = y0 + j;
      V d[N];
#pragma unroll
      for (int i = 0; i < N; ++i) {
        const int x = x0 + i;
        const bool ok = (unsigned)x < (unsigned)p.X && (unsigned)y < (unsigned)p.Y;
        d[i] = ok ? in[(((long long)b * p.X + x) * p.Y + y) * per_tile + zc] : vzero((V *)nullptr);
      }
      V c[N];
      Wino1D<MT, V>::in(d, c);
#pragma unroll
      for (int i = 0; i < N; ++i) w[i][j] = c[i];
    }
#pragma unroll
    for (int i = 0; i < N; ++i) {
      V v[N];
      Wino1D<MT, V>::in(w[i], v);
      if constexpr (PAIR) {
        const int cv = (int)(zc % CV);
        const bool odd = cv & 1;
        const long long dw = 2 * (t - cv) + ((cv >> 3) << 4) + (cv & 6) + (odd ? 8 : 0);
        u32x2w *Vp = reinterpret_cast<u32x2w *>(reinterpret_cast<unsigned *>(p.V) + dw);
        const long long pstride = p.vs / 2;
#pragma unroll
        for (int j = 0; j < N; ++j) {
          unsigned hi, lo;
          wino_pair2(v[j], vscale, &hi, &lo, sat);
          const unsigned give = odd ? hi : lo, got = (unsigned)__shfl_xor((int)give, 1);
          u32x2w o;
          o.x = odd ? got : hi;
          o.y = odd ? lo : got;
          Vp[(long long)(N * i + j) * pstride] = o;
        }
      } else {
#pragma unroll
        for (int j = 0; j < N; ++j) Vw[(long long)(N * i + j) * (p.vs / VW) + t] = v[j];
      }
    }
  }
  WINO_TL_END(p)
}

__device__ __forceinline__ float wino_finish(const WinoP &p, float acc, float sc, float sf, float r) {
  float v = acc * sc + sf;
  if (p.res_mode && !p.res_after_act) v += r;
  if (p.relu) v = v > 0.f ? v : 0.f;
  if (p.res_mode && p.res_after_act) v += r;
  return v * p.post_scale;
}
__device__ __forceinline__ float4 wino_finish_v(const WinoP &p, float4 a, float4 sc, float4 sf, float4 r) {
  return make_float4(wino_finish(p, a.x, sc.x, sf.x, r.x), wino_finish(p, a.y, sc.y, sf.y, r.y), wino_finish(p, a.z, sc.z, sf.z, r.z),
                     wino_finish(p, a.w, sc.w, sf.w, r.w));
}
__device__ __forceinline__ float wino_finish_v(const WinoP &p, float a, float sc, float sf, float r) { return wino_finish(p, a, sc, sf, r); }
__device__ __forceinline__ float2 wino_finish_v(const WinoP &p, float2 a, float2 sc, float2 sf, float2 r) {
  return make_float2(wino_finish(p, a.x, sc.x, sf.x, r.x), wino_finish(p, a.y, sc.y, sf.y, r.y));
}

template <int MT, int VW>
__global__ __launch_bounds__(256) void wino_output_kernel(const WinoP p) {
  WINO_TL_BEGIN
  typedef typename VecT<VW>::T V;
  constexpr int N = MT + 2;
  const int CV = p.Co / VW;
  const long long per_tile = (long long)p.Zo * CV;
  const long long total = (long long)p.B * p.TX * p.TY * per_tile;
  const V *Mw = reinterpret_cast<const V *>(p.Mw);
  const V *res = reinterpret_cast<const V *>(p.res);
  V *out = reinterpret_cast<V *>(p.out);
  const float mscale = wino_mscale(p.hdr);
  const int *src = p.bg ? p.bg + WINO_BG_HDR + p.B * p.TX * p.TY : nullptr;
  float omax = 0.f;
  for (long long t = (long long)blockIdx.x * blockDim.x + threadIdx.x; t < total; t += (long long)gridDim.x * blockDim.x) {
    const long long zc = t % per_tile;
    const int cv = (int)(zc % CV);
    long long q = t / per_tile;
    const long long tm = src ? (long long)src[q] * per_tile + zc : t;
    const int ty = (int)(q % p.TY);
    q /= p.TY;
    const int tx = (int)(q % p.TX);
    const int b = (int)(q / p.TX);
    V r[MT][N];
#pragma unroll
    for (int j = 0; j < N; ++j) {
      V m[N];
#pragma unroll
      for (int i = 0; i < N; ++i) m[i] = Mw[(long long)(N * i + j) * (p.ms / VW) + tm];
      V y[MT];
      Wino1D<MT, V>::out(m, y);
#pragma unroll
      for (int a = 0; a < MT; ++a) r[a][j] = y[a];
    }
    const V sc = mscale * (p.scale ? reinterpret_cast<const V *>(p.scale)[cv] : vone((V *)nullptr));
    const V sf = p.shift ? reinterpret_cast<const V *>(p.shift)[cv] : vzero((V *)nullptr);
#pragma unroll
    for (int a = 0; a < MT; ++a) {
      const int x = MT * tx + a;
      if (x >= p.Xo) continue;
      V yy[MT];
      Wino1D<MT, V>::out(r[a], yy);
#pragma unroll
      for (int e = 0; e < MT; ++e) {
        const int y = MT * ty + e;
        if (y >= p.Yo) continue;
        const long long o = (((long long)b * p.Xo + x) * p.Yo + y) * per_tile + zc;
        V rr = vzero((V *)nullptr);
        if (p.res_mode) rr = res[o];
        const V val = wino_finish_v(p, yy[e], sc, sf, rr);
        out[o] = val;
        if (p.pmax) omax = fmaxf(omax, vabsmax(val));
      }
    }
  }
  if (p.pmax) wino_block_max_store(omax, p.pmax);
  WINO_TL_END(p)
}

template <int MT> struct WinoAt;
template <> struct WinoAt<6> {
  static __device__ __forceinline__ float c(int e, int j) {
    constexpr float A[6][8] = {{1, 1, 1, 1, 1, 1, 1, 0},          {0, 1, -1, 2, -2, 0.5f, -0.5f, 0},
                               {0, 1, 1, 4, 4, 0.25f, 0.25f, 0},   {0, 1, -1, 8, -8, 0.125f, -0.125f, 0},
                               {0, 1, 1, 16, 16, 0.0625f, 0.0625f, 0}, {0, 1, -1, 32, -32, 0.03125f, -0.03125f, 1}};
    return A[e][j];
  }
};
template <> struct WinoAt<4> {
  static __device__ __forceinline__ float c(int e, int j) {
    constexpr float A[4][6] = {{1, 1, 1, 1, 1, 0}, {0, 1, -1, 2, -2, 0}, {0, 1, 1, 4, 4, 0}, {0, 1, -1, 8, -8, 1}};
    return A[e][j];
  }
};
__device__ __forceinline__ float vfma(float s, float a, float c) { return fmaf(s, a, c); }
__device__ __forceinline__ float2 vfma(float s, float2 a, float2 c) { return make_float2(fmaf(s, a.x, c.x), fmaf(s, a.y, c.y)); }
__device__ __forceinline__ float4 vfma(float s, float4 a, float4 c) {
  return make_float4(fmaf(s, a.x, c.x), fmaf(s, a.y, c.y), fmaf(s, a.z, c.z), fmaf(s, a.w, c.w));
}

typedef unsigned u32x2 __attribute__((ext_vector_type(2)));
template <int VW> struct BufIO;
template <> struct BufIO<2> {
  static __device__ __forceinline__ float2 load(__amdgpu_buffer_rsrc_t r, unsigned voff, unsigned soff) {
    const u32x2 v = __builtin_amdgcn_raw_buffer_load_b64(r, voff, soff, 0);
    return make_float2(__uint_as_float(v.x), __uint_as_float(v.y));
  }
  static __device__ __forceinline__ void store(__amdgpu_buffer_rsrc_t r, unsigned voff, unsigned soff, float2 f) {
    u32x2 v;
    v.x = __float_as_uint(f.x);
    v.y = __float_as_uint(f.y);
    __builtin_amdgcn_raw_buffer_store_b64(v, r, voff, soff, 0);
  }
};
template <> struct BufIO<1> {
  static __device__ __forceinline__ float load(__amdgpu_buffer_rsrc_t r, unsigned voff, unsigned soff) {
    return __uint_as_float(__builtin_amdgcn_raw_buffer_load_b32(r, voff, soff, 0));
  }
  static __device__ __forceinline__ void store(__amdgpu_buffer_rsrc_t r, unsigned voff, unsigned soff, float f) {
    __builtin_amdgcn_raw_buffer_store_b32(__float_as_uint(f), r, voff, soff, 0);
  }
};

template <int J, typename V>
__device__ __forceinline__ void wino6_acc_column(V (&acc)[6], const V y) {
#pragma unroll
  for (int e = 0; e < 6; ++e) {
    const float cf = WinoAt<6>::c(e, J);
    if (cf == 1.0f) acc[e] = acc[e] + y;
    else if (cf == -1.0f) acc[e] = acc[e] - y;
    else if (cf != 0.0f) acc[e] = vfma(cf, y, acc[e]);
  }
}

template <int J, int VW> struct Wino6Columns {
  typedef typename VecT<VW>::T V;
  static __device__ __forceinline__ void run(V (&acc)[6][6], const V (&col)[8], const __amdgpu_buffer_rsrc_t rm, const unsigned vo,
                                             const unsigned ps) {
    V nxt[8];
    if (J + 1 < 8) {
#pragma unroll
      for (int i = 0; i < 8; ++i) nxt[i] = BufIO<VW>::load(rm, vo, (unsigned)(8 * i + J + 1) * ps);
    }
    __builtin_amdgcn_sched_barrier(0);
    V y[6];
    Wino1D<6, V>::out(col, y);
#pragma unroll
    for (int a = 0; a < 6; ++a) wino6_acc_column<J>(acc[a], y[a]);
    __builtin_amdgcn_sched_barrier(0);
    Wino6Columns<J + 1, VW>::run(acc, nxt, rm, vo, ps);
  }
};
template <int VW> struct Wino6Columns<8, VW> {
  typedef typename VecT<VW>::T V;
  static __device__ __forceinline__ void run(V (&)[6][6], const V (&)[8], const __amdgpu_buffer_rsrc_t, const unsigned, const unsigned) {}
};

template <int VW, int WPE, int RPF = 0>
__global__ __launch_bounds__(256, WPE) void wino_output_buf_kernel(const WinoP p, const unsigned m_bytes, const unsigned out_bytes) {
  WINO_TL_BEGIN
  typedef typename VecT<VW>::T V;
  constexpr int MT = 6, N = 8, EB = VW * 4;
  const int CV = p.Co / VW;
  const long long per_tile = (long long)p.Zo * CV;
  const long long total = (long long)p.B * p.TX * p.TY * per_tile;
  const __amdgpu_buffer_rsrc_t rm = __builtin_amdgcn_make_buffer_rsrc((void *)p.Mw, 0, m_bytes, 0x00020000);
  const __amdgpu_buffer_rsrc_t ro = __builtin_amdgcn_make_buffer_rsrc((void *)p.out, 0, out_bytes, 0x00020000);
  const __amdgpu_buffer_rsrc_t rr = __builtin_amdgcn_make_buffer_rsrc((void *)(p.res ? p.res : p.out), 0, p.res ? out_bytes : 0u, 0x00020000);
  const unsigned ps = (unsigned)(p.ms * 4);
  const float mscale = wino_mscale(p.hdr);
  const int *src = p.bg ? p.bg + WINO_BG_HDR + p.B * p.TX * p.TY : nullptr;
  float omax = 0.f;
  for (long long t = (long long)blockIdx.x * blockDim.x + threadIdx.x; t < total; t += (long long)gridDim.x * blockDim.x) {
    const long long zc = t % per_tile;
    const int cv = (int)(zc % CV);
    long long q = t / per_tile;
    const unsigned vo = (unsigned)((src ? (long long)src[q] * per_tile + zc : t) * EB);
    const int ty = (int)(q % p.TY);
    q /= p.TY;
    const int tx = (int)(q % p.TX);
    const int b = (int)(q / p.TX);
    const V sc = mscale * (p.scale ? reinterpret_cast<const V *>(p.scale)[cv] : vone((V *)nullptr));
    const V sf = p.shift ? reinterpret_cast<const V *>(p.shift)[cv] : vzero((V *)nullptr);
    const int xb = MT * tx, yb = MT * ty;
    const unsigned o00 = (unsigned)(((((long long)b * p.Xo + xb) * p.Yo + yb) * per_tile + zc) * EB);
    const unsigned row = (unsigned)(p.Yo * per_tile * EB), colb = (unsigned)(per_tile * EB);
    V rres[RPF ? MT : 1][RPF ? MT : 1];
    if constexpr (RPF) {
#pragma unroll
      for (int a = 0; a < MT; ++a)
#pragma unroll
        for (int e = 0; e < MT; ++e)
          rres[a][e] = BufIO<VW>::load(rr, (xb + a < p.Xo && yb + e < p.Yo) ? o00 : 0x80000000u, (unsigned)a * row + (unsigned)e * colb);
      __builtin_amdgcn_sched_barrier(0);
    }
    V acc[MT][MT];
#pragma unroll
    for (int a = 0; a < MT; ++a)
#pragma unroll
      for (int e = 0; e < MT; ++e) acc[a][e] = vzero((V *)nullptr);
    V col[N];
#pragma unroll
    for (int i = 0; i < N; ++i) col[i] = BufIO<VW>::load(rm, vo, (unsigned)(N * i) * ps);
    Wino6Columns<0, VW>::run(acc, col, rm, vo, ps);
#pragma unroll
    for (int a = 0; a < MT; ++a) {
#pragma unroll
      for (int e = 0; e < MT; ++e) {
        const unsigned vo_ae = (xb + a < p.Xo && yb + e < p.Yo) ? o00 : 0x80000000u;
        const unsigned so = (unsigned)a * row + (unsigned)e * colb;
        V rv;
        if constexpr (RPF) rv = rres[a][e];
        else rv = BufIO<VW>::load(rr, vo_ae, so);
        const V val = wino_finish_v(p, acc[a][e], sc, sf, rv);
        BufIO<VW>::store(ro, vo_ae, so, val);
        omax = fmaxf(omax, (vo_ae >> 31) ? 0.f : vabsmax(val));
      }
      __builtin_amdgcn_sched_barrier(0);
    }
  }
  if (p.pmax) wino_block_max_store(omax, p.pmax);
  WINO_TL_END(p)
}

template <int MT>
__global__ __launch_bounds__(256) void wino_weight_kernel(const float *__restrict__ w, float *__restrict__ U, int Co, int KW, int Ci,
                                                          int kmode, unsigned *amax) {
  constexpr int N = MT + 2;
  const long long total = (long long)Co * KW * Ci;
  long long t = (long long)blockIdx.x * blockDim.x + threadIdx.x;
  if (t >= total) t = total - 1;
  const int ci = (int)(t % Ci);
  const int kz = (int)((t / Ci) % KW);
  const int co = (int)(t / ((long long)Ci * KW));
  float h[N][3];
#pragma unroll
  for (int e = 0; e < 3; ++e) {
    float g[3], c[N];
#pragma unroll
    for (int a = 0; a < 3; ++a) g[a] = w[((((long long)co * 3 + a) * 3 + e) * KW + kz) * Ci + ci];
    Wino1D<MT, float>::wgt(g, c);
#pragma unroll
    for (int i = 0; i < N; ++i) h[i][e] = c[i];
  }
  const long long K = (long long)KW * Ci;
  float umax = 0.f;
  const long long k = kmode == 1 ? ((long long)(ci >> 5) * KW + kz) * 32 + (ci & 31) : (long long)kz * Ci + ci;
#pragma unroll
  for (int i = 0; i < N; ++i) {
    float u[N];
    Wino1D<MT, float>::wgt(h[i], u);
#pragma unroll
    for (int j = 0; j < N; ++j) {
      U[((long long)(N * i + j) * Co + co) * K + k] = u[j];
      umax = fmaxf(umax, fabsf(u[j]));
    }
  }
  if (amax) {
#pragma unroll
    for (int o = 32; o > 0; o >>= 1) umax = fmaxf(umax, __shfl_xor(umax, o));
    if ((threadIdx.x & 63) == 0) atomicMax(amax, __float_as_uint(umax));
  }
}

struct WinoDims {
  int Xo, Yo, Zo, TX, TY, n2;
  int64_t v_elems, m_elems;
  int64_t v_stride, m_stride;
};

thread_local int g_wino_out_variant = -1;
thread_local int g_wino_in_variant = -1;

int wino_dims(const ivx_conv_desc *d, int tile, WinoDims *w, const char *who) {
  IVX_REQUIRE(d, "%s: null descriptor", who);
  IVX_REQUIRE(tile == 2 || tile == 4 || tile == 6, "%s: tile must be 2, 4 or 6 (F(m x m, 3x3)), got %d", who, tile);
  IVX_REQUIRE(d->KD == 3 && d->KH == 3 && d->sd == 1 && d->sh == 1, "%s: needs a 3x3 kernel with stride 1 on the first two axes", who);
  IVX_REQUIRE(d->KW >= 1 && d->KW <= 8 && d->sw >= 1 && d->pd >= 0 && d->ph >= 0 && d->pw >= 0, "%s: bad z kernel / stride / padding", who);
  IVX_REQUIRE(d->B > 0 && d->D > 0 && d->H > 0 && d->W > 0, "%s: non-positive dims", who);
  IVX_REQUIRE(d->Cin > 0 && d->Cin % 4 == 0 && d->Cout > 0 && d->Cout % 4 == 0, "%s: Cin and Cout must be multiples of 4", who);
  IVX_REQUIRE(d->in_dtype == IVX_F32 && d->out_dtype == IVX_F32, "%s: fp32 only", who);
  IVX_REQUIRE(d->wino_operands == IVX_F32 || (d->wino_operands == IVX_F16_PAIR && tile >= 4 && d->Cin % 16 == 0 &&
                                               (d->wgt_layout == 0 || d->Cin % 32 == 0)),
              "%s: wino_operands is IVX_F32 or IVX_F16_PAIR (tile 4 / 6, Cin %% 16 == 0; wgt_layout 1: Cin %% 32 == 0)", who);
  IVX_REQUIRE(d->out_mode == 0 && (d->res_mode == 0 || d->res_mode == 1), "%s: out_mode 0 and res_mode 0/1 only", who);
  IVX_REQUIRE(d->wgt_layout == 0 || (d->wgt_layout == 1 && d->Cin % 32 == 0), "%s: wgt_layout 1 needs Cin %% 32 == 0", who);
  int32_t Xo, Yo, Zo;
  if (ivx_conv_out_dims(d, &Xo, &Yo, &Zo) != IVX_OK) return IVX_ERR_INVALID_ARG;
  w->Xo = Xo; w->Yo = Yo; w->Zo = Zo;
  w->TX = (Xo + tile - 1) / tile; w->TY = (Yo + tile - 1) / tile;
  w->n2 = (tile + 2) * (tile + 2);
  w->v_elems = (int64_t)d->B * w->TX * w->TY * d->W * d->Cin;
  w->m_elems = (int64_t)d->B * w->TX * w->TY * Zo * d->Cout;
  w->v_stride = w->v_elems;
  w->m_stride = w->m_elems;
  return IVX_OK;
}

ivx_conv_desc wino_group_desc(const ivx_conv_desc *d, const WinoDims &w) {
  ivx_conv_desc g = *d;
  g.D = w.TX; g.H = w.TY;
  g.KD = 1; g.KH = 1; g.pd = 0; g.ph = 0; g.sd = 1; g.sh = 1;
  g.relu = 0; g.res_mode = 0; g.res_h = 0; g.res_w = 0; g.res_after_act = 0; g.post_scale = 1.0f;
  return g;
// ... 23 lines not shown
  int *layers;
  int B, TX, TY, nl, lstride, nb;
  int zo[WINO_BG_MAXL];
};
constexpr int WINO_BG_LDS_TILES = 16384;

__device__ __forceinline__ int wino_bg_scan(const int v, int *wsum, int *total) {
  const int lane = threadIdx.x & 63, wave = threadIdx.x >> 6;
  int incl = v;
#pragma unroll
  for (int o = 1; o < 64; o <<= 1) {
    const int x = __shfl_up(incl, o);
    if (lane >= o) incl += x;
  }
  __syncthreads();
  if (lane == 63) wsum[wave] = incl;
  __syncthreads();
  int base = 0, tot = 0;
#pragma unroll
  for (int w = 0; w < 16; ++w) {
    const int x = wsum[w];
    base += w < wave ? x : 0;
    tot += x;
  }
  *total = tot;
  return base + incl - v;
}

__global__ __launch_bounds__(1024) void wino_bg_plan_kernel(const WinoBgPlanP p) {
  __shared__ int rep[WINO_BG_KEYS];
  __shared__ int wsum[16];
  __shared__ unsigned char qlds[2][WINO_BG_LDS_TILES];
  const int tid = threadIdx.x, l = blockIdx.x;
  const int n = p.B * p.TX * p.TY;
  const int chunk = (n + 1023) / 1024;
  const int t0 = min(tid * chunk, n), t1 = min(t0 + chunk, n);
  unsigned char *qa = n <= WINO_BG_LDS_TILES ? qlds[0] : p.scratch + (size_t)(2 * l) * p.nb;
  unsigned char *qb = n <= WINO_BG_LDS_TILES ? qlds[1] : p.scratch + (size_t)(2 * l + 1) * p.nb;
  const int cap = l, LK = cap + 1, K = LK * LK * LK * LK;
  int *blk = p.layers + (size_t)l * p.lstride, *list = blk + WINO_BG_HDR, *src = list + n;
  auto key = [&](int t) {
    const int ty = t % p.TY, tx = (t / p.TY) % p.TX;
    return ((min(tx, cap) * LK + min(p.TX - 1 - tx, cap)) * LK + min(ty, cap)) * LK + min(p.TY - 1 - ty, cap);
  };
  for (int t = tid; t < n; t += 1024) qa[t] = p.z1[t];
  for (int k = tid; k < K; k += 1024) rep[k] = 0x7fffffff;
  __syncthreads();
  for (int e = 0; e < l; ++e) {
    for (int t = tid; t < n; t += 1024) {
      const int ty = t % p.TY, tx = (t / p.TY) % p.TX, b0 = t - tx * p.TY - ty;
      int q = 1;
      for (int dx = -1; dx <= 1; ++dx)
        for (int dy = -1; dy <= 1; ++dy) {
          const int xx = tx + dx, yy = ty + dy;
          if ((unsigned)xx < (unsigned)p.TX && (unsigned)yy < (unsigned)p.TY) q &= qa[b0 + xx * p.TY + yy];
        }
      qb[t] = (unsigned char)q;
    }
    __syncthreads();
    unsigned char *sw = qa; qa = qb; qb = sw;
  }
  int cnt = 0;
  for (int t = t0; t < t1; ++t) {
    if (!qa[t]) ++cnt;
    else atomicMin(&rep[key(t)], t);
  }
  int na;
  int o = wino_bg_scan(cnt, wsum, &na);
  for (int t = t0; t < t1; ++t)
    if (!qa[t]) { list[o] = t; src[t] = o; ++o; }
  const int kchunk = (K + 1023) / 1024, k0 = min(tid * kchunk, K), k1 = min(k0 + kchunk, K);
  cnt = 0;
  for (int k = k0; k < k1; ++k) cnt += rep[k] != 0x7fffffff;
  int nk;
  int r = wino_bg_scan(cnt, wsum, &nk);
  for (int k = k0; k < k1; ++k)
    if (rep[k] != 0x7fffffff) { list[na + r] = rep[k]; rep[k] = r; ++r; }
  __syncthreads();
  for (int t = t0; t < t1; ++t)
    if (qa[t]) src[t] = na + rep[key(t)];
  if (tid == 0) { blk[0] = na + nk; blk[1] = (na + nk) * p.zo[l]; blk[2] = na; blk[3] = nk; }
}

struct WinoBgLayout { int64_t z1, scratch, layers, lstride, total, nb; int n; };
WinoBgLayout wino_bg_layout(int B, int TX, int TY, int n_layers) {
  WinoBgLayout L;
  L.n = B * TX * TY;
  L.nb = ivx_align_up((int64_t)L.n, 256);
  L.z1 = 0; L.scratch = L.nb;
  L.layers = L.nb + (L.n <= WINO_BG_LDS_TILES ? 0 : 2 * (int64_t)WINO_BG_MAXL * L.nb);
  L.lstride = ivx_align_up((int64_t)(WINO_BG_HDR + 2 * (int64_t)L.n) * 4, 256) / 4;
  L.total = L.layers + (int64_t)n_layers * L.lstride * 4;
  return L;
}
unsigned wino_blocks(int64_t items) {
  const int64_t b = (items + 255) / 256;
  return (unsigned)(b < 1 ? 1 : (b > (1 << 20) ? (1 << 20) : b));
}

}

extern "C" int ivx_conv_winograd_set_variant(int32_t output_variant, int32_t input_variant) {
  g_wino_out_variant = output_variant;
  g_wino_in_variant = input_variant;
  return IVX_OK;
}

extern "C" int ivx_conv_winograd_supported(const ivx_conv_desc *d, int32_t tile) {
  WinoDims w;
  if (wino_dims(d, tile, &w, "ivx_conv_winograd_supported") != IVX_OK) return 0;
  if (w.v_stride * 4 >= (1LL << 31) || w.m_stride >= (1LL << 31) - 512 * (int64_t)d->Cout) return 0;
  if ((int64_t)d->Cout * d->KW * d->Cin * 4 >= (1LL << 31)) return 0;
  return 1;
}

extern "C" int64_t ivx_conv_winograd_weight_elems(const ivx_conv_desc *d, int32_t tile) {
  WinoDims w;
  if (wino_dims(d, tile, &w, "ivx_conv_winograd_weight_elems") != IVX_OK) return -1;
  return (int64_t)(w.n2 + (d->wino_operands == IVX_F16_PAIR ? 1 : 0)) * d->Cout * d->KW * d->Cin;
}

extern "C" int ivx_conv_winograd_weights(const ivx_conv_desc *d, int32_t tile, const float *wgt, float *u, ivx_stream_t stream) {
  WinoDims w;
  int rc = wino_dims(d, tile, &w, "ivx_conv_winograd_weights");
  if (rc != IVX_OK) return rc;
  IVX_REQUIRE(wgt && u, "ivx_conv_winograd_weights: null argument");
  const int64_t total = (int64_t)d->Cout * d->KW * d->Cin;
  const dim3 grid((unsigned)((total + 255) / 256));
  const bool pair = d->wino_operands == IVX_F16_PAIR;
  unsigned *hdr = pair ? reinterpret_cast<unsigned *>(u + (int64_t)w.n2 * total) : nullptr;
  if (pair && hipMemsetAsync(hdr, 0, 8, (hipStream_t)stream) != hipSuccess) {
    ivx_set_error("ivx_conv_winograd_weights: hipMemsetAsync failed");
    return IVX_ERR_HIP;
  }
  if (tile == 2)
    hipLaunchKernelGGL(wino_weight_kernel<2>, grid, dim3(256), 0, (hipStream_t)stream, wgt, u, d->Cout, d->KW, d->Cin, d->wgt_layout, hdr);
  else if (tile == 4)
    hipLaunchKernelGGL(wino_weight_kernel<4>, grid, dim3(256), 0, (hipStream_t)stream, wgt, u, d->Cout, d->KW, d->Cin, d->wgt_layout, hdr);
  else
    hipLaunchKernelGGL(wino_weight_kernel<6>, grid, dim3(256), 0, (hipStream_t)stream, wgt, u, d->Cout, d->KW, d->Cin, d->wgt_layout, hdr);
  if (pair) {
    const size_t n16 = (size_t)w.n2 * total / 16;
    hipLaunchKernelGGL(wino_pair_inplace_kernel, dim3((unsigned)((n16 + 255) / 256)), dim3(256), 0, (hipStream_t)stream, u, n16, hdr);
  }
  IVX_CHECK_LAUNCH("ivx_conv_winograd_weights");
  return IVX_OK;
}

extern "C" int64_t ivx_conv_winograd_workspace_bytes(const ivx_conv_desc *d, int32_t tile) {
  WinoDims w;
  if (wino_dims(d, tile, &w, "ivx_conv_winograd_workspace_bytes") != IVX_OK) return -1;
  return ivx_align_up(w.n2 * w.v_stride * 4, 256) + ivx_align_up(w.n2 * w.m_stride * 4, 256) + 256;
}

namespace {
#ifdef IVX_CONV_TIMELINE
unsigned long long *g_wino_timeline = nullptr;
#endif
int wino_setup(const ivx_conv_desc *d, int tile, const void *in, const float *scale, const float *shift, const void *res, void *out,
               void *workspace, int64_t workspace_bytes, WinoDims *w, WinoP *p, const char *who) {
  int rc = wino_dims(d, tile, w, who);
  if (rc != IVX_OK) return rc;
  IVX_REQUIRE(workspace, "%s: null workspace", who);
  if (!ivx_conv_winograd_supported(d, tile)) {
    ivx_set_error("%s: one transformed plane must stay below 2 GiB (use ivx_conv_fwd)", who);
    return IVX_ERR_UNSUPPORTED;
  }
  const int64_t need = ivx_conv_winograd_workspace_bytes(d, tile);
  if (workspace_bytes < need) {
    ivx_set_error("%s: workspace too small (%lld < %lld); size it with ivx_conv_winograd_workspace_bytes", who,
                  (long long)workspace_bytes, (long long)need);
    return IVX_ERR_WORKSPACE;
  }
  p->in = (const float *)in; p->scale = scale; p->shift = shift; p->res = d->res_mode ? (const float *)res : nullptr;
  p->out = (float *)out;
  p->V = (float *)workspace;
  p->Mw = (float *)((char *)workspace + ivx_align_up(w->n2 * w->v_stride * 4, 256));
  p->vs = w->v_stride; p->ms = w->m_stride;
  p->B = d->B; p->X = d->D; p->Y = d->H; p->Z = d->W; p->C = d->Cin;
  p->Xo = w->Xo; p->Yo = w->Yo; p->Zo = w->Zo; p->Co = d->Cout;
  p->TX = w->TX; p->TY = w->TY; p->px = d->pd; p->py = d->ph;
  p->relu = d->relu; p->res_mode = d->res_mode; p->res_after_act = d->res_after_act;
  p->post_scale = d->post_scale == 0.f ? 1.0f : d->post_scale;
  p->pmax = nullptr;
  p->bg = nullptr;
#ifdef IVX_CONV_TIMELINE
  p->tl = g_wino_timeline;
#endif
  p->hdr = d->wino_operands == IVX_F16_PAIR
               ? (const unsigned *)((char *)workspace + ivx_align_up(w->n2 * w->v_stride * 4, 256) + ivx_align_up(w->n2 * w->m_stride * 4, 256))
               : nullptr;
  return IVX_OK;
}
}

static int wino_bg_check(const ivx_conv_desc *d, int32_t tile, const void *bg, const char *who) {
  if (bg && !ivx_conv_winograd_bg_supported(d, tile)) {
    ivx_set_error("%s: the layer does not take the background form (ivx_conv_winograd_bg_supported)", who);
    return IVX_ERR_UNSUPPORTED;
  }
  return IVX_OK;
}

static int wino_input_impl(const ivx_conv_desc *d, int32_t tile, const void *in, void *workspace, int64_t workspace_bytes,
                           const float *partials, int32_t n_partials, const int32_t *bg, ivx_stream_t stream) {
  WinoDims w;
  WinoP p;
  float dummy;
  IVX_REQUIRE(in, "ivx_conv_winograd_input: null argument");
  int rc = wino_setup(d, tile, in, nullptr, nullptr, &dummy, &dummy, workspace, workspace_bytes, &w, &p, "ivx_conv_winograd_input");
  if (rc != IVX_OK) return rc;
  if ((rc = wino_bg_check(d, tile, bg, "ivx_conv_winograd_input")) != IVX_OK) return rc;
  p.bg = bg;
  if (d->wino_operands == IVX_F16_PAIR) {
    static const bool one_wg = !(getenv("IVX_WINO_AMAX_ONE_WG") && atoi(getenv("IVX_WINO_AMAX_ONE_WG")) == 0);
    const bool write_form = partials && n_partials <= 65536 && one_wg;
    if (!write_form && hipMemsetAsync((void *)p.hdr, 0, 4, (hipStream_t)stream) != hipSuccess) {
      ivx_set_error("ivx_conv_winograd_input: hipMemsetAsync failed");
      return IVX_ERR_HIP;
    }
    if (write_form) {
      hipLaunchKernelGGL(wino_amax_partials_write_kernel, dim3(1), dim3(1024), 0, (hipStream_t)stream, partials, n_partials, (unsigned *)p.hdr);
    } else if (partials) {
      const int pb = (n_partials + 255) / 256;
      hipLaunchKernelGGL(wino_amax_partials_kernel, dim3((unsigned)(pb > 64 ? 64 : pb)), dim3(256), 0, (hipStream_t)stream, partials, n_partials,
                         (unsigned *)p.hdr);
    } else {
      const size_t n4 = (size_t)d->B * d->D * d->H * d->W * d->Cin / 4;
      const size_t ab = (n4 + 1023) / 1024;
      hipLaunchKernelGGL(wino_amax_kernel, dim3((unsigned)(ab > 1536 ? 1536 : (ab < 1 ? 1 : ab))), dim3(256), 0, (hipStream_t)stream,
                         (const wf32x4 *)in, n4, (unsigned *)p.hdr);
    }
    if (tile == 4)
      hipLaunchKernelGGL((wino_input_kernel<4, 2, 1>), dim3(wino_blocks(w.v_elems / 2)), dim3(256), 0, (hipStream_t)stream, p);
    else
      hipLaunchKernelGGL((wino_input_kernel<6, 2, 1>), dim3(wino_blocks(w.v_elems / 2)), dim3(256), 0, (hipStream_t)stream, p);
  } else if (tile == 2)
    hipLaunchKernelGGL((wino_input_kernel<2, 4>), dim3(wino_blocks(w.v_elems / 4)), dim3(256), 0, (hipStream_t)stream, p);
  else if (tile == 4)
    hipLaunchKernelGGL((wino_input_kernel<4, 2>), dim3(wino_blocks(w.v_elems / 2)), dim3(256), 0, (hipStream_t)stream, p);
  else if (g_wino_in_variant == 1)
    hipLaunchKernelGGL((wino_input_kernel<6, 1>), dim3(wino_blocks(w.v_elems)), dim3(256), 0, (hipStream_t)stream, p);
  else
    hipLaunchKernelGGL((wino_input_kernel<6, 2>), dim3(wino_blocks(w.v_elems / 2)), dim3(256), 0, (hipStream_t)stream, p);
  IVX_CHECK_LAUNCH("ivx_conv_winograd_input");
  return IVX_OK;
}

extern "C" int ivx_conv_winograd_input(const ivx_conv_desc *d, int32_t tile, const void *in, void *workspace, int64_t workspace_bytes,
                                       ivx_stream_t stream) {
  return wino_input_impl(d, tile, in, workspace, workspace_bytes, nullptr, 0, nullptr, stream);
}

extern "C" int ivx_conv_winograd_input_amax(const ivx_conv_desc *d, int32_t tile, const void *in, void *workspace, int64_t workspace_bytes,
                                            const float *partials, int32_t n_partials, ivx_stream_t stream) {
  IVX_REQUIRE(!partials || n_partials > 0, "ivx_conv_winograd_input_amax: partials without a count");
  return wino_input_impl(d, tile, in, workspace, workspace_bytes, partials, n_partials, nullptr, stream);
}

extern "C" int ivx_conv_winograd_input_bg(const ivx_conv_desc *d, int32_t tile, const void *in, void *workspace, int64_t workspace_bytes,
                                          const float *partials, int32_t n_partials, const int32_t *bg, ivx_stream_t stream) {
  IVX_REQUIRE(!partials || n_partials > 0, "ivx_conv_winograd_input_bg: partials without a count");
  return wino_input_impl(d, tile, in, workspace, workspace_bytes, partials, n_partials, bg, stream);
}

static int wino_gemm_impl(const ivx_conv_desc *d, int32_t tile, const float *u, void *workspace, int64_t workspace_bytes, const int32_t *bg,
                          ivx_stream_t stream) {
  WinoDims w;
  WinoP p;
  float dummy;
  IVX_REQUIRE(u, "ivx_conv_winograd_gemm: null argument");
  int rc = wino_setup(d, tile, &dummy, nullptr, nullptr, &dummy, &dummy, workspace, workspace_bytes, &w, &p, "ivx_conv_winograd_gemm");
  if (rc != IVX_OK) return rc;
  ivx_conv_desc g = wino_group_desc(d, w);
  const long long el = d->wino_operands == IVX_F16_PAIR ? 2 : 1;
  g.in_dtype = d->wino_operands;
  const unsigned *us = p.hdr ? reinterpret_cast<const unsigned *>(u + (int64_t)w.n2 * d->Cout * d->KW * d->Cin + 1) : nullptr;
  if ((rc = wino_bg_check(d, tile, bg, "ivx_conv_winograd_gemm")) != IVX_OK) return rc;
  rc = ivx_conv_grouped_launch(&g, w.n2, p.V, el * w.v_stride, u, el * d->Cout * d->KW * d->Cin, p.Mw, w.m_stride, (hipStream_t)stream, us,
                               p.hdr ? const_cast<unsigned *>(p.hdr) + 1 : nullptr, bg ? bg + 1 : nullptr);
  if (rc != IVX_OK) return rc;
  IVX_CHECK_LAUNCH("ivx_conv_winograd_gemm");
  return IVX_OK;
}

extern "C" int ivx_conv_winograd_gemm(const ivx_conv_desc *d, int32_t tile, const float *u, void *workspace, int64_t workspace_bytes,
                                      ivx_stream_t stream) {
  return wino_gemm_impl(d, tile, u, workspace, workspace_bytes, nullptr, stream);
}

extern "C" int ivx_conv_winograd_gemm_bg(const ivx_conv_desc *d, int32_t tile, const float *u, void *workspace, int64_t workspace_bytes,
                                         const int32_t *bg, ivx_stream_t stream) {
  return wino_gemm_impl(d, tile, u, workspace, workspace_bytes, bg, stream);
}

extern "C" int ivx_conv_winograd_fused_supported(const ivx_conv_desc *d, int32_t tile) {
  WinoDims w;
  if (tile != 4 || !d || d->wino_operands != IVX_F16_PAIR || d->KW != 3 || d->sw != 1 || d->pw != 1 || d->wgt_layout != 1 || d->Cin % 32 || d->Cout % 4)
    return 0;
  if (!ivx_conv_winograd_supported(d, tile) || wino_dims(d, tile, &w, "ivx_conv_winograd_fused_supported") != IVX_OK) return 0;
  if ((int64_t)w.n2 * w.v_stride * 4 >= (1LL << 31) || (int64_t)w.n2 * d->Cout * d->KW * d->Cin * 4 >= (1LL << 31)) return 0;
  return 1;
}

extern "C" int32_t ivx_conv_winograd_fused_blocks(const ivx_conv_desc *d, int32_t tile) {
  WinoDims w;
  if (!ivx_conv_winograd_fused_supported(d, tile) || wino_dims(d, tile, &w, "ivx_conv_winograd_fused_blocks") != IVX_OK) return -1;
  return ivx_conv_fold4_blocks((long long)d->B * w.TX * w.TY * w.Zo, d->Cout);
}

extern "C" int ivx_conv_winograd_gemm_output_amax(const ivx_conv_desc *d, int32_t tile, const float *u, const float *scale, const float *shift,
                                                  const void *res, void *out, void *workspace, int64_t workspace_bytes, float *partials,
                                                  ivx_stream_t stream) {
  WinoDims w;
  WinoP p;
  float dummy;
  IVX_REQUIRE(u && out, "ivx_conv_winograd_gemm_output: null argument");
  IVX_REQUIRE(!d || d->res_mode == 0 || res, "ivx_conv_winograd_gemm_output: res_mode set but res is NULL");
  if (!ivx_conv_winograd_fused_supported(d, tile)) {
    ivx_set_error("ivx_conv_winograd_gemm_output: the fused form takes F(4x4,3x3) on IVX_F16_PAIR operands, a 3-tap z kernel with stride 1 and padding 1, "
                  "wgt_layout 1, Cin %% 32 == 0, and all 36 planes of V below 2 GiB (ivx_conv_winograd_fused_supported)");
    return IVX_ERR_UNSUPPORTED;
  }
  int rc = wino_setup(d, tile, &dummy, scale, shift, res, out, workspace, workspace_bytes, &w, &p, "ivx_conv_winograd_gemm_output");
  if (rc != IVX_OK) return rc;
  ivx_conv_desc g = wino_group_desc(d, w);
  g.in_dtype = d->wino_operands;
  IvxWinoFold f;
  f.out = p.out; f.res = p.res; f.scale = p.scale; f.shift = p.shift;
  f.hdr_v = p.hdr;
  f.uscale = u + (int64_t)w.n2 * d->Cout * d->KW * d->Cin + 1;
  f.pmax = partials;
  f.B = d->B; f.TX = w.TX; f.TY = w.TY; f.Z = w.Zo; f.Xo = w.Xo; f.Yo = w.Yo; f.Co = d->Cout;
  f.relu = p.relu; f.res_mode = p.res_mode; f.res_after_act = p.res_after_act; f.post_scale = p.post_scale;
  static const int fold_waves = getenv("IVX_FOLD4_WAVES") ? atoi(getenv("IVX_FOLD4_WAVES")) : 1;
  if (fold_waves == 2 && d->Cout % 8 == 0)
    rc = ivx_conv_launch_fold4w(reinterpret_cast<const _Float16 *>(p.V), 2 * w.v_stride, reinterpret_cast<const _Float16 *>(u), 2LL * d->Cout * d->KW * d->Cin,
                                d->B * w.TX * w.TY * w.Zo, 2 * d->Cin, d->Cout, w.Zo, f, (hipStream_t)stream);
  else
    rc = ivx_conv_grouped_fold4(&g, w.n2, p.V, 2 * w.v_stride, u, 2LL * d->Cout * d->KW * d->Cin, &f, (hipStream_t)stream);
  if (rc != IVX_OK) return rc;
  IVX_CHECK_LAUNCH("ivx_conv_winograd_gemm_output");
  return IVX_OK;
}

namespace {
int wino_output_variant(const ivx_conv_desc *d, const WinoDims &w, bool with_partials) {
  const bool buf_ok = (int64_t)w.n2 * w.m_stride * 4 < (1LL << 32) && (int64_t)d->B * w.Xo * w.Yo * w.Zo * d->Cout * 4 < (1LL << 31);
  int v = (g_wino_out_variant >= 0 && !with_partials) ? g_wino_out_variant : (d->res_mode ? 4 : 1);
  if (v >= 2 && !buf_ok) v = 0;
  if (v >= 4 && !d->res_mode) v = v == 4 ? 2 : 3;
  return v;
}
unsigned wino_output_grid(const ivx_conv_desc *d, int tile, const WinoDims &w, bool with_partials) {
  if (tile == 2) return wino_blocks(w.m_elems / 4);
  if (tile == 4) return wino_blocks(w.m_elems / 2);
  const int v = wino_output_variant(d, w, with_partials);
  return (v == 2 || v == 0 || v == 4) ? wino_blocks(w.m_elems / 2) : wino_blocks(w.m_elems);
}
}

extern "C" int32_t ivx_conv_winograd_output_blocks(const ivx_conv_desc *d, int32_t tile) {
  WinoDims w;
  if (wino_dims(d, tile, &w, "ivx_conv_winograd_output_blocks") != IVX_OK) return -1;
  return (int32_t)wino_output_grid(d, tile, w, true);
}

static int wino_output_impl(const ivx_conv_desc *d, int32_t tile, const float *scale, const float *shift, const void *res, void *out,
                            void *workspace, int64_t workspace_bytes, float *partials, const int32_t *bg, ivx_stream_t stream) {
  WinoDims w;
  WinoP p;
  float dummy;
  IVX_REQUIRE(out, "ivx_conv_winograd_output: null argument");
  IVX_REQUIRE(!d || d->res_mode == 0 || res, "ivx_conv_winograd_output: res_mode set but res is NULL");
  int rc = wino_setup(d, tile, &dummy, scale, shift, res, out, workspace, workspace_bytes, &w, &p, "ivx_conv_winograd_output");
  if (rc != IVX_OK) return rc;
  if ((rc = wino_bg_check(d, tile, bg, "ivx_conv_winograd_output")) != IVX_OK) return rc;
  p.pmax = partials;
  p.bg = bg;
  if (tile == 2)
    hipLaunchKernelGGL((wino_output_kernel<2, 4>), dim3(wino_blocks(w.m_elems / 4)), dim3(256), 0, (hipStream_t)stream, p);
  else if (tile == 4)
    hipLaunchKernelGGL((wino_output_kernel<4, 2>), dim3(wino_blocks(w.m_elems / 2)), dim3(256), 0, (hipStream_t)stream, p);
  else {
    const int v = wino_output_variant(d, w, partials != nullptr);
    const unsigned mb = (unsigned)((int64_t)w.n2 * w.m_stride * 4), ob = (unsigned)((int64_t)d->B * w.Xo * w.Yo * w.Zo * d->Cout * 4);
    if (v == 2)
      hipLaunchKernelGGL((wino_output_buf_kernel<2, 3>), dim3(wino_blocks(w.m_elems / 2)), dim3(256), 0, (hipStream_t)stream, p, mb, ob);
    else if (v == 3)
      hipLaunchKernelGGL((wino_output_buf_kernel<1, 5>), dim3(wino_blocks(w.m_elems)), dim3(256), 0, (hipStream_t)stream, p, mb, ob);
    else if (v == 4)
      hipLaunchKernelGGL((wino_output_buf_kernel<2, 2, 1>), dim3(wino_blocks(w.m_elems / 2)), dim3(256), 0, (hipStream_t)stream, p, mb, ob);
    else if (v == 5)
      hipLaunchKernelGGL((wino_output_buf_kernel<1, 4, 1>), dim3(wino_blocks(w.m_elems)), dim3(256), 0, (hipStream_t)stream, p, mb, ob);
    else if (v == 1)
      hipLaunchKernelGGL((wino_output_kernel<6, 1>), dim3(wino_blocks(w.m_elems)), dim3(256), 0, (hipStream_t)stream, p);
    else
      hipLaunchKernelGGL((wino_output_kernel<6, 2>), dim3(wino_blocks(w.m_elems / 2)), dim3(256), 0, (hipStream_t)stream, p);
  }
  IVX_CHECK_LAUNCH("ivx_conv_winograd_output");
  return IVX_OK;
}

extern "C" int ivx_conv_winograd_output(const ivx_conv_desc *d, int32_t tile, const float *scale, const float *shift, const void *res,
                                        void *out, void *workspace, int64_t workspace_bytes, ivx_stream_t stream) {
  return wino_output_impl(d, tile, scale, shift, res, out, workspace, workspace_bytes, nullptr, nullptr, stream);
}

extern "C" int ivx_conv_winograd_output_amax(const ivx_conv_desc *d, int32_t tile, const float *scale, const float *shift, const void *res,
                                             void *out, void *workspace, int64_t workspace_bytes, float *partials, ivx_stream_t stream) {
  return wino_output_impl(d, tile, scale, shift, res, out, workspace, workspace_bytes, partials, nullptr, stream);
}

extern "C" int ivx_conv_winograd_output_bg(const ivx_conv_desc *d, int32_t tile, const float *scale, const float *shift, const void *res,
                                           void *out, void *workspace, int64_t workspace_bytes, float *partials, const int32_t *bg,
                                           ivx_stream_t stream) {
  return wino_output_impl(d, tile, scale, shift, res, out, workspace, workspace_bytes, partials, bg, stream);
}

extern "C" int ivx_conv_winograd_bg_supported(const ivx_conv_desc *d, int32_t tile) {
  WinoDims w;
  if (tile != 6 || !d || d->pd != 1 || d->ph != 1 || !ivx_conv_winograd_supported(d, tile)) return 0;
  if (wino_dims(d, tile, &w, "ivx_conv_winograd_bg_supported") != IVX_OK) return 0;
  ivx_conv_desc g = wino_group_desc(d, w);
  g.in_dtype = d->wino_operands;
  return ivx_conv_grouped_rows_dev_ok(&g, w.n2);
}

extern "C" int64_t ivx_conv_winograd_bg_bytes(const ivx_conv_desc *d, int32_t n_layers) {
  WinoDims w;
  if (wino_dims(d, 6, &w, "ivx_conv_winograd_bg_bytes") != IVX_OK) return -1;
  IVX_REQUIRE(n_layers >= 1 && n_layers <= WINO_BG_MAXL, "ivx_conv_winograd_bg_bytes: 1 .. %d layers", WINO_BG_MAXL) ;
  return wino_bg_layout(d->B, w.TX, w.TY, n_layers).total;
}

extern "C" int64_t ivx_conv_winograd_bg_layer_offset(const ivx_conv_desc *d, int32_t layer) {
  WinoDims w;
  if (wino_dims(d, 6, &w, "ivx_conv_winograd_bg_layer_offset") != IVX_OK) return -1;
  IVX_REQUIRE(layer >= 0 && layer < WINO_BG_MAXL, "ivx_conv_winograd_bg_layer_offset: bad layer");
  const WinoBgLayout L = wino_bg_layout(d->B, w.TX, w.TY, layer + 1);
  return L.layers + (int64_t)layer * L.lstride * 4;
}

extern "C" int ivx_conv_winograd_bg_plan(const ivx_conv_desc *d, const uint8_t *valid, int32_t n_layers, const int32_t *out_slices, void *block,
                                         int64_t block_bytes, ivx_stream_t stream) {
  WinoDims w;
  int rc = wino_dims(d, 6, &w, "ivx_conv_winograd_bg_plan");
  if (rc != IVX_OK) return rc;
  IVX_REQUIRE(valid && out_slices && block, "ivx_conv_winograd_bg_plan: null argument");
  IVX_REQUIRE(n_layers >= 1 && n_layers <= WINO_BG_MAXL, "ivx_conv_winograd_bg_plan: 1 .. %d layers", WINO_BG_MAXL);
  IVX_REQUIRE(d->pd == 1 && d->ph == 1, "ivx_conv_winograd_bg_plan: the chain's layers pad x and y by 1");
  const WinoBgLayout L = wino_bg_layout(d->B, w.TX, w.TY, n_layers);
  if (block_bytes < L.total) {
    ivx_set_error("ivx_conv_winograd_bg_plan: block too small (%lld < %lld); size it with ivx_conv_winograd_bg_bytes", (long long)block_bytes,
                  (long long)L.total);
    return IVX_ERR_WORKSPACE;
  }
  char *base = (char *)block;
  WinoBgPlanP p;
  p.z1 = (const unsigned char *)(base + L.z1); p.scratch = (unsigned char *)(base + L.scratch);
  p.layers = (int *)(base + L.layers);
  p.B = d->B; p.TX = w.TX; p.TY = w.TY; p.nl = n_layers; p.lstride = (int)L.lstride; p.nb = (int)L.nb;
  for (int l = 0; l < WINO_BG_MAXL; ++l) p.zo[l] = l < n_layers ? out_slices[l] : 0;
  hipLaunchKernelGGL(wino_bg_z1_kernel, dim3((unsigned)((L.n + 3) / 4)), dim3(256), 0, (hipStream_t)stream, valid, d->B, d->D, d->H, d->W, w.TX, w.TY,
                     (unsigned char *)(base + L.z1));
  hipLaunchKernelGGL(wino_bg_plan_kernel, dim3((unsigned)n_layers), dim3(1024), 0, (hipStream_t)stream, p);
  IVX_CHECK_LAUNCH("ivx_conv_winograd_bg_plan");
  return IVX_OK;
}

extern "C" int ivx_conv_winograd_fwd(const ivx_conv_desc *d, int32_t tile, const void *in, const float *u, const float *scale,
                                     const float *shift, const void *res, void *out, void *workspace, int64_t workspace_bytes,
                                     ivx_stream_t stream) {
  int rc = ivx_conv_winograd_input(d, tile, in, workspace, workspace_bytes, stream);
  if (rc != IVX_OK) return rc;
  rc = ivx_conv_winograd_gemm(d, tile, u, workspace, workspace_bytes, stream);
  if (rc != IVX_OK) return rc;
  return ivx_conv_winograd_output(d, tile, scale, shift, res, out, workspace, workspace_bytes, stream);
}

#ifdef IVX_CONV_TIMELINE
extern "C" int ivx_wino_set_timeline(void *buf) { g_wino_timeline = (unsigned long long *)buf; return 0; }
#endif
```

imvoxelnet_amd/ops.py:

```python
import ctypes as C

import torch

from . import _lib
from ._lib import ConvDesc, AnchorHeadDesc, check


def _stream():
    return C.c_void_p(torch.cuda.current_stream().cuda_stream)


FP8 = torch.float8_e4m3fn
_DT = {torch.float32: 0, torch.bfloat16: 1, FP8: 2}


def _chk(t, name, dtype=torch.float32):
    if not isinstance(t, torch.Tensor):
        raise TypeError(f'{name} must be a torch.Tensor')
    if not t.is_cuda:
        raise RuntimeError(f'{name} must be a device (HIP) tensor; the MI355X path has no CPU fallback')
    if t.dtype != dtype:
        raise TypeError(f'{name} must be {dtype}, got {t.dtype}')
    if not t.is_contiguous():
        raise ValueError(f'{name} must be contiguous')
# ... 123 lines not shown
    wsb = L.ivx_conv_workspace_bytes(C.byref(d))
    ws = torch.empty((wsb,), device=x.device, dtype=torch.uint8) if wsb > 0 else None
    check(L.ivx_conv_fwd_ws(C.byref(d), _ptr(x), _ptr(wgt), _ptr(scale), _ptr(shift), _ptr(res), _ptr(out), _ptr(ws), max(wsb, 0),
                            _stream()), 'ivx_conv_fwd_ws')
    return out


IVX_BF16_PAIR = 3


def bf16_pair_split(x, out=None):
    _chk(x, 'x')
    if x.shape[-1] % 16:
        raise ValueError('the channel count must be a multiple of 16')
    if out is None:
        out = torch.empty(x.shape[:-1] + (2 * x.shape[-1],), device=x.device, dtype=torch.bfloat16)
    else:
        _chk(out, 'out', torch.bfloat16)
    check(_lib.lib().ivx_bf16_pair_split(_ptr(x), x.numel(), _ptr(out), _stream()), 'ivx_bf16_pair_split')
    return out


def conv_pair_supported(x_shape, Cout, kernel, stride, padding, wgt_layout=1):
    B, D, H, W, Cin = x_shape
    d = ConvDesc(B, D, H, W, Cin, Cout, kernel[0], kernel[1], kernel[2], stride[0], stride[1], stride[2], padding[0], padding[1], padding[2],
                 0, 0, 0, 0, int(wgt_layout), 0, 0, 1.0, 0, 0, 1.0)
    return bool(_lib.lib().ivx_conv_pair_supported(C.byref(d)))


IVX_F16_PAIR = 4


def _wino_desc(B, D, H, W, Cin, Cout, kw, stride_w, padding, relu, wgt_layout, res_mode=0, res_after_act=False, post_scale=1.0, operands=0):
    return ConvDesc(B, D, H, W, Cin, Cout, 3, 3, kw, 1, 1, stride_w, padding[0], padding[1], padding[2], int(bool(relu)),
                    int(res_mode), 0, 0, int(wgt_layout), 0, int(bool(res_after_act)), float(post_scale), 0, 0, 1.0, int(operands))


def conv_winograd_supported(x_shape, Cout, kernel, stride, padding, tile=2, operands=0):
    if kernel[0] != 3 or kernel[1] != 3 or stride[0] != 1 or stride[1] != 1 or x_shape[4] % 4 or Cout % 4 or tile not in (2, 4, 6):
        return False
    B, D, H, W, Cin = x_shape
    d = _wino_desc(B, D, H, W, Cin, Cout, kernel[2], stride[2], padding, False, 0, operands=operands)
    return bool(_lib.lib().ivx_conv_winograd_supported(C.byref(d), tile))


def conv_winograd_weights(wgt, wgt_layout, tile=2, operands=0):
    _chk(wgt, 'wgt')
    Cout, kd, kh, kw, Cin = wgt.shape
    if kd != 3 or kh != 3:
        raise ValueError('Winograd F(m x m, 3x3) needs a 3x3 kernel on the first two axes')
    d = _wino_desc(1, 4, 4, max(kw, 1), Cin, Cout, kw, 1, (1, 1, kw // 2), False, wgt_layout, operands=operands)
    L = _lib.lib()
    n = L.ivx_conv_winograd_weight_elems(C.byref(d), tile)
    if n < 0:
        check(-1, 'ivx_conv_winograd_weight_elems')
    u = torch.empty(((tile + 2) ** 2 + (1 if operands else 0), Cout, kw * Cin), device=wgt.device, dtype=torch.float32)
    assert u.numel() == n
    check(L.ivx_conv_winograd_weights(C.byref(d), tile, _ptr(wgt), _ptr(u), _stream()), 'ivx_conv_winograd_weights')
    return u


winograd_trace = None


def winograd_bg_plan(valid, x_shape, Cout, out_slices, wgt_layout=1, operands=IVX_F16_PAIR):
    B, X, Y, Z, Cin = x_shape
    if tuple(valid.shape) != (B, X, Y, Z) or not valid.is_cuda or not valid.is_contiguous() or valid.element_size() != 1:
        raise ValueError('valid must be a contiguous [B,X,Y,Z] one-byte device tensor')
    d = _wino_desc(B, X, Y, Z, Cin, Cout, 3, 1, (1, 1, 1), False, wgt_layout, operands=operands)
    L = _lib.lib()
    nl = len(out_slices)
    nb = L.ivx_conv_winograd_bg_bytes(C.byref(d), nl)
    if nb < 0:
        check(-1, 'ivx_conv_winograd_bg_bytes')
    block = torch.zeros((nb,), device=valid.device, dtype=torch.uint8)
    zo = (C.c_int32 * nl)(*[int(z) for z in out_slices])
    check(L.ivx_conv_winograd_bg_plan(C.byref(d), _ptr(valid), nl, zo, _ptr(block), nb, _stream()), 'ivx_conv_winograd_bg_plan')
    n = B * ((X + 5) // 6) * ((Y + 5) // 6)
    views = []
    for l in range(nl):
        off = L.ivx_conv_winograd_bg_layer_offset(C.byref(d), l)
        views.append(block[off:off + 4 * (4 + 2 * n)].view(torch.int32))
    return block, views


def conv_winograd_fwd(x, u, scale=None, shift=None, kw=3, stride_w=1, padding=(1, 1, 1), relu=False, res=None, out=None,
                      wgt_layout=0, res_after_act=False, post_scale=1.0, operands=0, amax_in=None, want_amax=False, fused=False, bg=None):
    _chk(x, 'x')
    _chk(u, 'u')
    B, D, H, W, Cin = x.shape
    Cout = u.shape[1]
    tile = {16: 2, 36: 4, 64: 6}.get(u.shape[0] - (1 if operands else 0))
    if tile is None or tuple(u.shape[1:]) != (Cout, kw * Cin):
        raise ValueError(f'transformed filters {tuple(u.shape)} do not match kw {kw} / Cin {Cin}')
    d = _wino_desc(B, D, H, W, Cin, Cout, kw, stride_w, padding, relu, wgt_layout, 1 if res is not None else 0, res_after_act,
                   post_scale, operands)
    do, ho, wo = C.c_int32(), C.c_int32(), C.c_int32()
    L = _lib.lib()
    check(L.ivx_conv_out_dims(C.byref(d), C.byref(do), C.byref(ho), C.byref(wo)), 'ivx_conv_out_dims')
    oshape = (B, do.value, ho.value, wo.value, Cout)
    if res is not None:
        _chk(res, 'res')
        if tuple(res.shape) != oshape:
            raise ValueError(f'residual shape {tuple(res.shape)} != output shape')
    for t, n in ((scale, 'scale'), (shift, 'shift')):
        if t is not None:
            _chk(t, n)
            if t.numel() != Cout:
                raise ValueError(f'{n} must have {Cout} elements')
    if out is None:
        out = torch.empty(oshape, device=x.device, dtype=torch.float32)
    else:
        _chk(out, 'out')
    wsb = L.ivx_conv_winograd_workspace_bytes(C.byref(d), tile)
    if wsb < 0:
        check(-1, 'ivx_conv_winograd_workspace_bytes')
    ws = torch.empty((wsb,), device=x.device, dtype=torch.uint8)
    if fused:
        if not L.ivx_conv_winograd_fused_supported(C.byref(d), tile):
            raise ValueError('this layer does not take the fused GEMM + output form (ivx_conv_winograd_fused_supported)')
        part = None
        if want_amax:
            part = torch.empty((L.ivx_conv_winograd_fused_blocks(C.byref(d), tile),), device=x.device, dtype=torch.float32)
        if amax_in is not None:
            _chk(amax_in, 'amax_in')
        check(L.ivx_conv_winograd_input_amax(C.byref(d), tile, _ptr(x), _ptr(ws), wsb, _ptr(amax_in), 0 if amax_in is None else amax_in.numel(),
                                             _stream()), 'ivx_conv_winograd_input_amax')
        check(L.ivx_conv_winograd_gemm_output_amax(C.byref(d), tile, _ptr(u), _ptr(scale), _ptr(shift), _ptr(res), _ptr(out), _ptr(ws), wsb, _ptr(part),
                                                   _stream()), 'ivx_conv_winograd_gemm_output_amax')
        return (out, part) if want_amax else out
    if bg is not None:
        if not L.ivx_conv_winograd_bg_supported(C.byref(d), tile):
            raise ValueError('this layer does not take the background form (ivx_conv_winograd_bg_supported)')
        part = None
        if want_amax:
            part = torch.empty((L.ivx_conv_winograd_output_blocks(C.byref(d), tile),), device=x.device, dtype=torch.float32)
        if amax_in is not None:
            _chk(amax_in, 'amax_in')
        check(L.ivx_conv_winograd_input_bg(C.byref(d), tile, _ptr(x), _ptr(ws), wsb, _ptr(amax_in), 0 if amax_in is None else amax_in.numel(),
                                           _ptr(bg), _stream()), 'ivx_conv_winograd_input_bg')
        check(L.ivx_conv_winograd_gemm_bg(C.byref(d), tile, _ptr(u), _ptr(ws), wsb, _ptr(bg), _stream()), 'ivx_conv_winograd_gemm_bg')
        check(L.ivx_conv_winograd_output_bg(C.byref(d), tile, _ptr(scale), _ptr(shift), _ptr(res), _ptr(out), _ptr(ws), wsb, _ptr(part),
                                            _ptr(bg), _stream()), 'ivx_conv_winograd_output_bg')
        return (out, part) if want_amax else out
    if amax_in is not None or want_amax:
        part = None
        if want_amax:
            nb = L.ivx_conv_winograd_output_blocks(C.byref(d), tile)
            if nb < 0:
                check(-1, 'ivx_conv_winograd_output_blocks')
            part = torch.empty((nb,), device=x.device, dtype=torch.float32)
        if amax_in is not None:
            _chk(amax_in, 'amax_in')
        check(L.ivx_conv_winograd_input_amax(C.byref(d), tile, _ptr(x), _ptr(ws), wsb, _ptr(amax_in), 0 if amax_in is None else amax_in.numel(),
                                             _stream()), 'ivx_conv_winograd_input_amax')
        check(L.ivx_conv_winograd_gemm(C.byref(d), tile, _ptr(u), _ptr(ws), wsb, _stream()), 'ivx_conv_winograd_gemm')
        check(L.ivx_conv_winograd_output_amax(C.byref(d), tile, _ptr(scale), _ptr(shift), _ptr(res), _ptr(out), _ptr(ws), wsb, _ptr(part),
                                              _stream()), 'ivx_conv_winograd_output_amax')
        return (out, part) if want_amax else out
    if winograd_trace is None:
        check(L.ivx_conv_winograd_fwd(C.byref(d), tile, _ptr(x), _ptr(u), _ptr(scale), _ptr(shift), _ptr(res), _ptr(out), _ptr(ws),
                                      wsb, _stream()), 'ivx_conv_winograd_fwd')
        return out
    ev = [torch.cuda.Event(enable_timing=True) for _ in range(4)]
    ev[0].record()
    check(L.ivx_conv_winograd_input(C.byref(d), tile, _ptr(x), _ptr(ws), wsb, _stream()), 'ivx_conv_winograd_input')
# ... 818 lines not shown
```

include/imvoxel.h:

```cpp
#ifndef IMVOXEL_H_
#define IMVOXEL_H_

#include <stdint.h>

#ifdef __cplusplus
extern "C" {
#endif

#define IVX_OK 0
#define IVX_ERR_INVALID_ARG (-1)
#define IVX_ERR_HIP (-2)
#define IVX_ERR_UNSUPPORTED (-3)
#define IVX_ERR_WORKSPACE (-4)

typedef void *ivx_stream_t;

int ivx_version(void);
const char *ivx_last_error(void);

#define IVX_F32 0
#define IVX_BF16 1
#define IVX_FP8 2
#define IVX_BF16_PAIR 3
#define IVX_F16_PAIR 4
// ... 53 lines not shown
int64_t ivx_stem_pool_filter_bytes(void);
int ivx_stem_pool_pack_filters(const float *w, const float *scale, void *packed, float *scale_out);
int ivx_stem_pool_out_dims(int32_t H, int32_t W, int32_t *Hp, int32_t *Wp);
int ivx_stem_pool_fwd_pair(const float *img, int32_t B, int32_t H, int32_t W, const void *wfrag, const float *scale_p, const float *shift,
                           float wbound, float sbound, const uint32_t *amax_img, void *out, float *out_scale, uint32_t *amax_out,
                           ivx_stream_t stream);

typedef struct ivx_bottleneck_desc {
  int32_t B, H, W, P;
} ivx_bottleneck_desc;
typedef struct ivx_bottleneck_io {
  const float *in_scale;
  const uint32_t *amax_in;
  float *out_scale;
  uint32_t *amax_out;
  float wbound[3], sbound[3];
} ivx_bottleneck_io;
int ivx_bottleneck_supported(const ivx_bottleneck_desc *d);
int ivx_bottleneck_fwd_pio(const ivx_bottleneck_desc *d, const ivx_bottleneck_io *io, const void *in, const void *w1, const float *scale1,
                           const float *shift1, const void *w2, const float *scale2, const float *shift2, const void *w3, const float *scale3,
                           const float *shift3, void *out, ivx_stream_t stream);
int ivx_bottleneck_proj_supported(const ivx_bottleneck_desc *d, int32_t Cin);
int ivx_bottleneck_proj_pack(const float *w3, const float *scale3, const float *shift3, const float *wd, const float *scaled, const float *shiftd,
                             int32_t P, int32_t Cin, void *packed, float *scale_out, float *shift_out, float *wbound3, float *sbound, float *wboundd);
int ivx_bottleneck_proj_fwd_pio(const ivx_bottleneck_desc *d, int32_t Cin, const ivx_bottleneck_io *io, float wbound_shortcut, const void *in,
                                const void *w1, const float *scale1, const float *shift1, const void *w2, const float *scale2, const float *shift2,
                                const void *w3d, const float *scale3d, const float *shift3d, void *out, ivx_stream_t stream);

int ivx_conv_fwd_naive(const ivx_conv_desc *d, const void *in, const void *wgt, const float *scale,
                       const float *shift, const void *res, void *out, ivx_stream_t stream);

float ivx_conv_winograd_issued_fraction(const ivx_conv_desc *d);
int ivx_conv_winograd_supported(const ivx_conv_desc *d, int32_t tile);
int64_t ivx_conv_winograd_weight_elems(const ivx_conv_desc *d, int32_t tile);
int ivx_conv_winograd_weights(const ivx_conv_desc *d, int32_t tile, const float *wgt, float *u, ivx_stream_t stream);
int64_t ivx_conv_winograd_workspace_bytes(const ivx_conv_desc *d, int32_t tile);
int ivx_conv_winograd_input(const ivx_conv_desc *d, int32_t tile, const void *in, void *workspace, int64_t workspace_bytes,
                            ivx_stream_t stream);
int ivx_conv_winograd_gemm(const ivx_conv_desc *d, int32_t tile, const float *u, void *workspace, int64_t workspace_bytes,
                           ivx_stream_t stream);
int ivx_conv_winograd_output(const ivx_conv_desc *d, int32_t tile, const float *scale, const float *shift, const void *res,
                             void *out, void *workspace, int64_t workspace_bytes, ivx_stream_t stream);
int ivx_conv_winograd_fwd(const ivx_conv_desc *d, int32_t tile, const void *in, const float *u, const float *scale,
                          const float *shift, const void *res, void *out, void *workspace, int64_t workspace_bytes,
                          ivx_stream_t stream);
typedef struct ivx_conv_route_opts {
  int32_t winograd;
  int32_t winograd_tile;
  int32_t wino_operands;
  int32_t split;
  int64_t winograd_min_pos;
  int32_t winograd_2d_min_ch;
} ivx_conv_route_opts;
typedef struct ivx_conv_route {
  int32_t form;
  int32_t tile;
  int32_t wino_candidate, split_candidate;
  int32_t split_fits;
  int32_t prefers_winograd;
  ivx_conv_desc run;
} ivx_conv_route_out;
int ivx_conv_route(const ivx_conv_desc *d, int32_t cin_real, const ivx_conv_route_opts *o, ivx_conv_route_out *r);
int32_t ivx_conv_winograd_output_blocks(const ivx_conv_desc *d, int32_t tile);
int ivx_conv_winograd_output_amax(const ivx_conv_desc *d, int32_t tile, const float *scale, const float *shift, const void *res, void *out,
                                  void *workspace, int64_t workspace_bytes, float *partials, ivx_stream_t stream);
int ivx_conv_winograd_input_amax(const ivx_conv_desc *d, int32_t tile, const void *in, void *workspace, int64_t workspace_bytes,
                                 const float *partials, int32_t n_partials, ivx_stream_t stream);
int ivx_conv_winograd_fused_supported(const ivx_conv_desc *d, int32_t tile);
int32_t ivx_conv_winograd_fused_blocks(const ivx_conv_desc *d, int32_t tile);
int ivx_conv_winograd_gemm_output_amax(const ivx_conv_desc *d, int32_t tile, const float *u, const float *scale, const float *shift,
                                       const void *res, void *out, void *workspace, int64_t workspace_bytes, float *partials,
                                       ivx_stream_t stream);
int ivx_conv_winograd_bg_supported(const ivx_conv_desc *d, int32_t tile);
int64_t ivx_conv_winograd_bg_bytes(const ivx_conv_desc *d, int32_t n_layers);
int64_t ivx_conv_winograd_bg_layer_offset(const ivx_conv_desc *d, int32_t layer);
int ivx_conv_winograd_bg_plan(const ivx_conv_desc *d, const uint8_t *valid, int32_t n_layers, const int32_t *out_slices, void *block,
                              int64_t block_bytes, ivx_stream_t stream);
int ivx_conv_winograd_input_bg(const ivx_conv_desc *d, int32_t tile, const void *in, void *workspace, int64_t workspace_bytes,
                               const float *partials, int32_t n_partials, const int32_t *bg, ivx_stream_t stream);
int ivx_conv_winograd_gemm_bg(const ivx_conv_desc *d, int32_t tile, const float *u, void *workspace, int64_t workspace_bytes,
                              const int32_t *bg, ivx_stream_t stream);
int ivx_conv_winograd_output_bg(const ivx_conv_desc *d, int32_t tile, const float *scale, const float *shift, const void *res, void *out,
                                void *workspace, int64_t workspace_bytes, float *partials, const int32_t *bg, ivx_stream_t stream);


int ivx_dcn_im2col_fwd(const float *x, const float *offset_mask, int32_t B, int32_t H, int32_t W, int32_t C, int32_t kh,
                       int32_t kw, int32_t stride, int32_t pad, int32_t dil, int32_t om_channels, float *col,
                       ivx_stream_t stream);
int ivx_dcn_im2col_fwd_pair(const void *x, const float *x_scale, const float *offset_mask, int32_t B, int32_t H, int32_t W, int32_t C,
                            int32_t kh, int32_t kw, int32_t stride, int32_t pad, int32_t dil, int32_t om_channels, void *col,
                            float *col_scale, uint32_t *col_amax, ivx_stream_t stream);
int ivx_dcn_im2col_fwd_bf16(const void *x, const float *offset_mask, int32_t B, int32_t H, int32_t W, int32_t C, int32_t kh,
                            int32_t kw, int32_t stride, int32_t pad, int32_t dil, int32_t om_channels, void *col,
                            ivx_stream_t stream);

int ivx_maxpool2d_fwd(const float *in, int32_t B, int32_t H, int32_t W, int32_t C, int32_t k,
                      int32_t s, int32_t p, float *out, ivx_stream_t stream);
int ivx_maxpool2d_fwd_bf16(const void *in, int32_t B, int32_t H, int32_t W, int32_t C, int32_t k,
                           int32_t s, int32_t p, void *out, ivx_stream_t stream);
int ivx_maxpool2d_fwd_fp8(const void *in, int32_t B, int32_t H, int32_t W, int32_t C, int32_t k, int32_t s, int32_t p,
                          void *out, ivx_stream_t stream);

int ivx_upsample_trilinear2x_fwd(const float *in, int32_t B, int32_t D, int32_t H, int32_t W, int32_t C, float *out,
                                 ivx_stream_t stream);

int ivx_nchw_to_nhwc(const float *in, int32_t B, int32_t C, int64_t S, int32_t Cpad, float *out,
                     ivx_stream_t stream);
int ivx_image_s2d_bf16(const float *img, int32_t B, int32_t H, int32_t W, void *out, ivx_stream_t stream);
int ivx_nhwc_to_nchw(const float *in, int32_t B, int64_t S, int32_t C, float *out, ivx_stream_t stream);

#define IVX_IMAGE_PREP_MAX_DIM 32768
typedef struct ivx_image_prep_desc {
  int32_t src_h, src_w;
  int32_t src_row_bytes;
  int32_t dst_h, dst_w;
  int32_t pad_h, pad_w;
  int32_t to_rgb;
  float mean[3], std[3];
} ivx_image_prep_desc;

int ivx_rescale_size(int32_t src_h, int32_t src_w, int32_t scale_a, int32_t scale_b,
                     int32_t *dst_h, int32_t *dst_w);

int ivx_image_prep_u8(const ivx_image_prep_desc *d, const void *src, int64_t src_image_bytes,
                      int32_t n, float *out, ivx_stream_t stream);

int ivx_backproject_mean_fwd(const float *feat, int32_t B, int32_t V, int32_t FH, int32_t FW, int32_t C,
                             const float *proj, const float *new_origin, const int32_t *crop_hw,
                             const float *voxel_size , int32_t X, int32_t Y, int32_t Z,
                             float *volume, uint8_t *valid, ivx_stream_t stream);

int ivx_backproject_mean_fwd_bf16(const void *feat, int32_t B, int32_t V, int32_t FH, int32_t FW, int32_t C,
                                  const float *proj, const float *new_origin, const int32_t *crop_hw,
                                  const float *voxel_size, int32_t X, int32_t Y, int32_t Z, void *volume,
                                  uint8_t *valid, ivx_stream_t stream);
int ivx_upsample_trilinear2x_fwd_bf16(const void *in, int32_t B, int32_t D, int32_t H, int32_t W, int32_t C, void *out,
                                      ivx_stream_t stream);

int32_t ivx_backproject_amax_blocks(int32_t B, int32_t V, int32_t X, int32_t Y, int32_t Z);
int ivx_backproject_mean_fwd_amax(const float *feat, int32_t B, int32_t V, int32_t FH, int32_t FW, int32_t C, const float *proj,
                                  const float *new_origin, const int32_t *crop_hw, const float *voxel_size, int32_t X, int32_t Y,
                                  int32_t Z, float *volume, uint8_t *valid, float *partials, ivx_stream_t stream);
int ivx_backproject_sum_fwd(const float *feat, int32_t B, int32_t V, int32_t FH, int32_t FW, int32_t C,
                            const float *proj, const float *new_origin, const int32_t *crop_hw,
                            const float *voxel_size, int32_t X, int32_t Y, int32_t Z, float *volume_sum,
                            int32_t *count, ivx_stream_t stream);
int ivx_volume_normalize_fwd(float *volume, const int32_t *count, int64_t n_voxels, int32_t C, uint8_t *valid,
                             ivx_stream_t stream);

int ivx_backproject_accum_fwd(const float *feat, int32_t B, int32_t V, int32_t FH, int32_t FW, int32_t C, const float *proj,
                              const float *new_origin, const int32_t *crop_hw, const float *voxel_size , int32_t X, int32_t Y,
                              int32_t Z, float *volume_sum, int32_t *count, int32_t first, float *mean_out, uint8_t *valid_out,
                              ivx_stream_t stream);
int ivx_backproject_accum_fwd_bf16(const void *feat, int32_t B, int32_t V, int32_t FH, int32_t FW, int32_t C, const float *proj,
                                   const float *new_origin, const int32_t *crop_hw, const float *voxel_size , int32_t X, int32_t Y,
                                   int32_t Z, float *volume_sum, int32_t *count, int32_t first, void *mean_out, uint8_t *valid_out,
                                   ivx_stream_t stream);
int ivx_volume_mean_fwd(const float *volume_sum, const int32_t *count, int64_t n_voxels, int32_t C, void *out, int32_t out_dtype,
                        uint8_t *valid, ivx_stream_t stream);

#define IVX_SAMPLE_NEAREST 0
#define IVX_SAMPLE_BILINEAR 1
#define IVX_LIFT_MEAN 0
#define IVX_LIFT_SUM 1
#define IVX_LIFT_ACCUM 2
typedef struct ivx_backproject_desc {
// ... 227 lines not shown
```

Baseline: 282.0 images/s.

## Skip unread Winograd output tiles and chain amax through an in-launch atomic word

The neck background plan gains a consumer analysis: for each chained Winograd layer it records whether its output is read only by the next layer or a later residual, and a new need kernel builds a visit list so the output transform writes only the tiles a consumer will read. The output kernels also fold the per-block maxima into a single word with an atomic max, and the next layer's input transform reads that word directly instead of reducing partials in a separate pass. This removes output writes for unread tiles and the extra amax reduction per chained layer. The cost is extra planning logic, a visit-list indirection in the output loop, atomics, and the risk that a tensor read outside the chain is left stale if the consumer analysis misses a reader.

New measurement: 282.6 images/s, median of 2. About the same (+0.2%).

```diff
diff --git a/imvoxelnet_amd/_lib.py b/imvoxelnet_amd/_lib.py
--- a/imvoxelnet_amd/_lib.py
+++ b/imvoxelnet_amd/_lib.py
@@ -128,6 +128,8 @@
 EXPORTS = ['ivx_model_plan_info', 'ivx_model_plan_step', 'ivx_model_plan_tensor', 'ivx_bottleneck_proj_supported', 'ivx_bottleneck_proj_pack', 'ivx_bottleneck_proj_fwd_pio', 'ivx_anchor_head_decode', 'ivx_fcos3d_head_decode', 'ivx_nms_rotated_bev', 'ivx_nms_aligned3d', 'ivx_bottleneck_supported', 'ivx_bottleneck_fwd_pio', 'ivx_amax_f32', 'ivx_stem_pool_filter_bytes', 'ivx_stem_pool_pack_filters', 'ivx_stem_pool_out_dims', 'ivx_stem_pool_fwd_pair', 'ivx_conv_winograd_set_variant', 'ivx_ubench_mfma', 'ivx_ubench_copy', 'ivx_version', 'ivx_last_error', 'ivx_conv_out_dims', 'ivx_conv_fwd', 'ivx_conv_fwd_naive', 'ivx_conv_set_tile_override', 'ivx_conv_set_epilogue_mode', 'ivx_conv_set_plan_mode', 'ivx_topk_set_mode', 'ivx_conv_workspace_bytes', 'ivx_conv_fwd_ws', 'ivx_conv_set_halo_mode', 'ivx_bf16_pair_split', 'ivx_f16_pair_split', 'ivx_conv_pair_supported', 'ivx_bf16_pair_pack_filters', 'ivx_conv_route', 'ivx_conv_pio_workspace_bytes', 'ivx_conv_fwd_pio', 'ivx_conv_fwd_pio_naive', 'ivx_pair_pack_filters', 'ivx_nchw_to_nhwc_amax', 'ivx_maxpool2d_fwd_pair', 'ivx_f16_pair_merge', 'ivx_model_calibrate_fp8', 'ivx_model_calibrate_fp8_ex', 'ivx_amax_bf16', 'ivx_conv_winograd_output_blocks', 'ivx_conv_winograd_issued_fraction', 'ivx_conv_winograd_output_amax', 'ivx_conv_winograd_input_amax', 'ivx_conv_winograd_fused_supported', 'ivx_conv_winograd_fused_blocks', 'ivx_conv_winograd_gemm_output_amax',
            'ivx_conv_winograd_bg_supported', 'ivx_conv_winograd_bg_bytes', 'ivx_conv_winograd_bg_layer_offset', 'ivx_conv_winograd_bg_plan',
            'ivx_conv_winograd_input_bg', 'ivx_conv_winograd_gemm_bg', 'ivx_conv_winograd_output_bg',
+           'ivx_conv_winograd_bg_plan_ex', 'ivx_conv_winograd_bg_visit_offset', 'ivx_conv_winograd_output_bg_need', 'ivx_conv_winograd_amax_word',
+           'ivx_conv_winograd_input_bg_ready',
            'ivx_conv_winograd_supported', 'ivx_conv_winograd_weight_elems', 'ivx_conv_winograd_weights', 'ivx_conv_winograd_workspace_bytes',
            'ivx_conv_winograd_input', 'ivx_conv_winograd_gemm', 'ivx_conv_winograd_output', 'ivx_conv_winograd_fwd',
            'ivx_maxpool2d_fwd', 'ivx_maxpool2d_fwd_bf16', 'ivx_maxpool2d_fwd_fp8', 'ivx_global_avgpool_fwd', 'ivx_global_avgpool_fwd_bf16', 'ivx_upsample_trilinear2x_fwd', 'ivx_dcn_im2col_fwd', 'ivx_dcn_im2col_fwd_bf16', 'ivx_dcn_im2col_fwd_pair', 'ivx_nchw_to_nhwc', 'ivx_image_s2d_bf16', 'ivx_nhwc_to_nchw', 'ivx_backproject_mean_fwd', 'ivx_backproject_mean_fwd_amax', 'ivx_backproject_amax_blocks', 'ivx_backproject_mean_fwd_bf16', 'ivx_upsample_trilinear2x_fwd_bf16', 'ivx_backproject_sum_fwd', 'ivx_volume_normalize_fwd',
@@ -182,6 +184,13 @@
     L.ivx_conv_winograd_input_bg.argtypes = [C.POINTER(ConvDesc), i32, vp, vp, i64, vp, i32, vp, vp]
     L.ivx_conv_winograd_gemm_bg.argtypes = [C.POINTER(ConvDesc), i32, vp, vp, i64, vp, vp]
     L.ivx_conv_winograd_output_bg.argtypes = [C.POINTER(ConvDesc), i32, vp, vp, vp, vp, vp, i64, vp, vp, vp]
+    L.ivx_conv_winograd_bg_plan_ex.argtypes = [C.POINTER(ConvDesc), vp, i32, C.POINTER(i32), C.POINTER(i32), vp, i64, vp]
+    L.ivx_conv_winograd_bg_visit_offset.argtypes = [C.POINTER(ConvDesc)]
+    L.ivx_conv_winograd_bg_visit_offset.restype = i64
+    L.ivx_conv_winograd_output_bg_need.argtypes = [C.POINTER(ConvDesc), i32, vp, vp, vp, vp, vp, i64, vp, vp, i32, vp, vp]
+    L.ivx_conv_winograd_amax_word.argtypes = [C.POINTER(ConvDesc), i32, vp, i64]
+    L.ivx_conv_winograd_amax_word.restype = vp
+    L.ivx_conv_winograd_input_bg_ready.argtypes = [C.POINTER(ConvDesc), i32, vp, vp, i64, vp, vp, vp]
     L.ivx_bf16_pair_split.argtypes = [vp, i64, vp, vp]
     L.ivx_f16_pair_split.argtypes = [vp, i64, f32, vp, vp]
     L.ivx_conv_pair_supported.argtypes = [C.POINTER(ConvDesc)]
diff --git a/imvoxelnet_amd/csrc/api_common.cpp b/imvoxelnet_amd/csrc/api_common.cpp
--- a/imvoxelnet_amd/csrc/api_common.cpp
+++ b/imvoxelnet_amd/csrc/api_common.cpp
@@ -13,7 +13,7 @@
   va_end(ap);
 }
 
-extern "C" int ivx_version(void) { return 470;  }
+extern "C" int ivx_version(void) { return 480;  }
 extern "C" const char *ivx_last_error(void) { return g_err; }
 
 extern "C" __attribute__((weak)) int ivx_dcn_im2col_fwd_bf16(const void *, const float *, int32_t, int32_t, int32_t, int32_t, int32_t, int32_t, int32_t,
diff --git a/imvoxelnet_amd/csrc/model.cpp b/imvoxelnet_amd/csrc/model.cpp
--- a/imvoxelnet_amd/csrc/model.cpp
+++ b/imvoxelnet_amd/csrc/model.cpp
@@ -28,6 +28,14 @@
 __attribute__((weak)) int ivx_conv_winograd_output_bg(const ivx_conv_desc *d, int32_t tile, const float *scale, const float *shift, const void *res,
                                                       void *out, void *workspace, int64_t workspace_bytes, float *partials, const int32_t *bg,
                                                       ivx_stream_t stream);
+__attribute__((weak)) int ivx_conv_winograd_bg_plan_ex(const ivx_conv_desc *d, const uint8_t *valid, int32_t n_layers, const int32_t *out_slices,
+                                                       const int32_t *consumers, void *block, int64_t block_bytes, ivx_stream_t stream);
+__attribute__((weak)) int ivx_conv_winograd_output_bg_need(const ivx_conv_desc *d, int32_t tile, const float *scale, const float *shift, const void *res,
+                                                           void *out, void *workspace, int64_t workspace_bytes, float *partials, const int32_t *bg,
+                                                           int32_t need, void *amax_word, ivx_stream_t stream);
+__attribute__((weak)) void *ivx_conv_winograd_amax_word(const ivx_conv_desc *d, int32_t tile, void *workspace, int64_t workspace_bytes);
+__attribute__((weak)) int ivx_conv_winograd_input_bg_ready(const ivx_conv_desc *d, int32_t tile, const void *in, void *workspace, int64_t workspace_bytes,
+                                                           const int32_t *bg, const void *amax_word, ivx_stream_t stream);
 }
 
 #define M_REQUIRE(cond, ...)        \
@@ -174,6 +182,9 @@
   int fuse = 0, fuse_out = -1;
   int side = 0, join = 0;
   int64_t bg = -1;
+  int need = 0;
+  int amax_to = -1, amax_ready = 0;
+  int64_t tick = -1;
 };
 
 struct Plan {
@@ -192,6 +203,8 @@
   int bg_first = -1, bg_layers = 0;
   int64_t bg_off = -1, bg_bytes = 0;
   int32_t bg_zo[9] = {0, 0, 0, 0, 0, 0, 0, 0, 0};
+  int32_t bg_cons[27];
+  int64_t tick_off = 0, tick_bytes = 0;
 };
 
 }
@@ -1149,6 +1162,8 @@
       if (ti.off >= 0 && ti.first >= r.s0 && ti.last == i && ti.first != -2) release(ti.off, ti.bytes);
     }
   }
+  const bool inlaunch_on = !(getenv("IVX_WINO_AMAX_INLAUNCH") && atoi(getenv("IVX_WINO_AMAX_INLAUNCH")) == 0) && ivx_conv_winograd_output_bg_need &&
+                         ivx_conv_winograd_amax_word && ivx_conv_winograd_input_bg_ready;
   for (int i = r.s0; i < r.s1; ++i) {
     const Step &s = m->steps[i];
     PlanStep &pc = pl->ps[i];
@@ -1176,8 +1191,29 @@
         }
         pc.amax_in = pp.amax_out;
         pc.amax_in_n = pp.amax_n;
+        if (inlaunch_on && j == i - 1 && pp.amax_to == -1) {
+          pp.amax_to = i;
+          pc.amax_ready = 1;
+        } else {
+          if (pp.amax_to >= 0) pl->ps[pp.amax_to].amax_ready = 0;
+          pp.amax_to = -2;
+        }
       }
       break;
+    }
+  }
+  {
+    int n_tick = 0;
+    for (int i = r.s0; i < r.s1; ++i)
+      if (pl->ps[i].amax_to >= 0) ++n_tick;
+    if (n_tick > 0) {
+      top = align256(top);
+      pl->tick_off = top;
+      pl->tick_bytes = align256((int64_t)n_tick * 4);
+      n_tick = 0;
+      for (int i = r.s0; i < r.s1; ++i)
+        if (pl->ps[i].amax_to >= 0) pl->ps[i].tick = pl->tick_off + 4 * (int64_t)n_tick++;
+      top += pl->tick_bytes;
     }
   }
   const bool bg_on = !(getenv("IVX_NECK_BACKGROUND") && atoi(getenv("IVX_NECK_BACKGROUND")) == 0);
@@ -1209,6 +1245,38 @@
       pl->bg_off = top;
       top += align256(pl->bg_bytes);
       for (size_t l = 0; l < chain_s.size(); ++l) pl->ps[chain_s[l]].bg = pl->bg_off + ivx_conv_winograd_bg_layer_offset(&d0, (int32_t)l);
+      const bool skip_on = !(getenv("IVX_NECK_SKIP_UNREAD") && atoi(getenv("IVX_NECK_SKIP_UNREAD")) == 0) && ivx_conv_winograd_bg_plan_ex &&
+                           ivx_conv_winograd_output_bg_need;
+      std::vector<int> keep = {m->t_fpn0, m->t_volume, m->t_valid, m->t_neck, m->t_head, m->t_angle, m->t_layout};
+      keep.insert(keep.end(), m->t_levels.begin(), m->t_levels.end());
+      for (size_t l = 0; l < chain_s.size(); ++l) {
+        const int t = m->steps[chain_s[l]].out;
+        int32_t next = 0, resof = -1, other = skip_on ? 0 : 1;
+        if (std::find(keep.begin(), keep.end(), t) != keep.end() || pl->t[t].last >= r.s1) other = 1;
+        for (int j = 0; j < (int)m->steps.size(); ++j) {
+          const Step &q = m->steps[j];
+          const auto cj = std::find(chain_s.begin(), chain_s.end(), j);
+          const int lj = cj == chain_s.end() ? -1 : (int)(cj - chain_s.begin());
+          if (q.in == t) {
+            if (lj == (int)l + 1) next = 1;
+            else other = 1;
+          }
+          if (q.res == t) {
+            if (lj > (int)l && resof < 0) resof = lj;
+            else other = 1;
+          }
+          if (q.kind == ST_INDOOR_TAIL)
+            for (size_t v = 0; v < m->t_cb.size(); ++v)
+              if (m->t_cb[v] == t || m->t_cs[v] == t || m->t_cc[v] == t) other = 1;
+        }
+        pl->bg_cons[3 * l] = next; pl->bg_cons[3 * l + 1] = resof; pl->bg_cons[3 * l + 2] = other;
+        pl->ps[chain_s[l]].need = other ? 0 : 1;
+      }
+      for (size_t l = 0; l < chain_s.size(); ++l) {
+        const int t = m->steps[chain_s[l]].out;
+        M_REQUIRE(!pl->ps[chain_s[l]].need || (std::find(keep.begin(), keep.end(), t) == keep.end() && pl->t[t].last < r.s1),
+                  "internal: a kept tensor (%d) would be written in the need form", t);
+      }
     }
   }
   if (n_slots > 0) {
@@ -1341,8 +1409,18 @@
   auto scalep = [&](int t) -> float * { uint32_t *q = slotp(t); return q ? (float *)(q + IVX_AMAX_SLOTS) : nullptr; };
   if (pl.scal_bytes > 0 && r.s0 <= m->trunk0 && r.s1 > m->trunk0)
     M_HIP(hipMemsetAsync(base + pl.scal_off, 0, (size_t)pl.scal_bytes, st), "hipMemsetAsync (amax slots)");
+  if (pl.tick_bytes > 0)
+    M_HIP(hipMemsetAsync(base + pl.tick_off, 0, (size_t)pl.tick_bytes, st), "hipMemsetAsync (chained maxima)");
   auto wino_input = [&](const PlanStep &ps, const void *in) -> int {
     const float *part = ps.amax_in >= 0 ? (const float *)(base + ps.amax_in) : nullptr;
+    if (ps.amax_ready) {
+      const PlanStep *pp = nullptr;
+      for (int j = r.s0; j < r.s1 && !pp; ++j)
+        if (pl.ps[j].amax_to >= 0 && &pl.ps[pl.ps[j].amax_to] == &ps) pp = &pl.ps[j];
+      M_REQUIRE(pp && pp->tick >= 0, "internal: no producer word for the maxima of a chained layer");
+      return ivx_conv_winograd_input_bg_ready(&ps.d, ps.tile, in, ws, pl.ws_bytes, ps.bg >= 0 ? (const int32_t *)(base + ps.bg) : nullptr,
+                                              base + pp->tick, st);
+    }
     if (ps.bg >= 0) return ivx_conv_winograd_input_bg(&ps.d, ps.tile, in, ws, pl.ws_bytes, part, ps.amax_in_n, (const int32_t *)(base + ps.bg), st);
     return ivx_conv_winograd_input_amax(&ps.d, ps.tile, in, ws, pl.ws_bytes, part, ps.amax_in_n, st);
   };
@@ -1353,11 +1431,23 @@
   };
   auto wino_output = [&](const PlanStep &ps, const ConvLayer &L, const void *res, void *out) -> int {
     float *part = ps.amax_out >= 0 ? (float *)(base + ps.amax_out) : nullptr;
+    if (ps.need || ps.amax_to >= 0) {
+      void *word = nullptr;
+      if (ps.amax_to >= 0) {
+        M_REQUIRE(part && ps.tick >= 0, "internal: no word for the maxima of a chained layer");
+        word = base + ps.tick;
+      }
+      return ivx_conv_winograd_output_bg_need(&ps.d, ps.tile, L.scale, L.shift, res, out, ws, pl.ws_bytes, part,
+                                              ps.bg >= 0 ? (const int32_t *)(base + ps.bg) : nullptr, ps.need, word, st);
+    }
     if (ps.bg >= 0) return ivx_conv_winograd_output_bg(&ps.d, ps.tile, L.scale, L.shift, res, out, ws, pl.ws_bytes, part, (const int32_t *)(base + ps.bg), st);
     return ivx_conv_winograd_output_amax(&ps.d, ps.tile, L.scale, L.shift, res, out, ws, pl.ws_bytes, part, st);
   };
   auto bg_plan = [&](const Step &lift) -> int {
     if (pl.bg_first < 0) return IVX_OK;
+    if (ivx_conv_winograd_bg_plan_ex)
+      return ivx_conv_winograd_bg_plan_ex(&pl.ps[pl.bg_first].d, (const uint8_t *)ptr(lift.out2), pl.bg_layers, pl.bg_zo, pl.bg_cons, base + pl.bg_off,
+                                          pl.bg_bytes, st);
     return ivx_conv_winograd_bg_plan(&pl.ps[pl.bg_first].d, (const uint8_t *)ptr(lift.out2), pl.bg_layers, pl.bg_zo, base + pl.bg_off, pl.bg_bytes, st);
   };
   const bool span2d = m->trace_on && m->trace_level == 1 && m->cfg.with_trunk;
diff --git a/imvoxelnet_amd/csrc/winograd.hip b/imvoxelnet_amd/csrc/winograd.hip
--- a/imvoxelnet_amd/csrc/winograd.hip
+++ b/imvoxelnet_amd/csrc/winograd.hip
@@ -28,6 +28,9 @@
   float *pmax;
   const unsigned *hdr;
   const int *bg;
+  const int *vis;
+  unsigned *amax_dst;
+  unsigned *hdr_copy;
 #ifdef IVX_CONV_TIMELINE
   unsigned long long *tl;
 #endif
@@ -61,13 +64,17 @@
 __device__ __forceinline__ float vabsmax(const float v) { return fabsf(v); }
 __device__ __forceinline__ float vabsmax(const float2 v) { return fmaxf(fabsf(v.x), fabsf(v.y)); }
 __device__ __forceinline__ float vabsmax(const float4 v) { return fmaxf(fmaxf(fabsf(v.x), fabsf(v.y)), fmaxf(fabsf(v.z), fabsf(v.w))); }
-__device__ __forceinline__ void wino_block_max_store(float m, float *pmax) {
+__device__ __forceinline__ void wino_block_max_store(float m, float *pmax, unsigned *dst = nullptr) {
 #pragma unroll
   for (int o = 32; o > 0; o >>= 1) m = fmaxf(m, __shfl_xor(m, o));
   __shared__ float wmax[4];
   if ((threadIdx.x & 63) == 0) wmax[threadIdx.x >> 6] = m;
   __syncthreads();
-  if (threadIdx.x == 0) pmax[blockIdx.x] = fmaxf(fmaxf(wmax[0], wmax[1]), fmaxf(wmax[2], wmax[3]));
+  if (threadIdx.x == 0) {
+    const float v = fmaxf(fmaxf(wmax[0], wmax[1]), fmaxf(wmax[2], wmax[3]));
+    pmax[blockIdx.x] = v;
+    if (dst) (void)__hip_atomic_fetch_max(dst, __float_as_uint(v), __ATOMIC_RELAXED, __HIP_MEMORY_SCOPE_AGENT);
+  }
 }
 __global__ __launch_bounds__(256) void wino_amax_partials_kernel(const float *__restrict__ part, int n, unsigned *out) {
   float m = 0.f;
@@ -270,6 +277,7 @@
   V *Vw = reinterpret_cast<V *>(p.V);
   const float vscale = PAIR ? wino_pair_vscale(p.hdr) : 1.0f;
   const bool sat = PAIR ? wino_amax_bad(__uint_as_float(p.hdr[0])) : false;
+  if (PAIR && p.hdr_copy && blockIdx.x == 0 && threadIdx.x == 0) p.hdr_copy[0] = p.hdr[0];
   for (long long t = (long long)blockIdx.x * blockDim.x + threadIdx.x; t < total; t += (long long)gridDim.x * blockDim.x) {
     const long long zc = t % per_tile;
     long long q = t / per_tile;
@@ -347,7 +355,8 @@
   constexpr int N = MT + 2;
   const int CV = p.Co / VW;
   const long long per_tile = (long long)p.Zo * CV;
-  const long long total = (long long)p.B * p.TX * p.TY * per_tile;
+  const int *vis = p.vis;
+  const long long total = (vis ? (long long)vis[0] : (long long)p.B * p.TX * p.TY) * per_tile;
   const V *Mw = reinterpret_cast<const V *>(p.Mw);
   const V *res = reinterpret_cast<const V *>(p.res);
   V *out = reinterpret_cast<V *>(p.out);
@@ -358,6 +367,7 @@
     const long long zc = t % per_tile;
     const int cv = (int)(zc % CV);
     long long q = t / per_tile;
+    if (vis) q = vis[1 + q];
     const long long tm = src ? (long long)src[q] * per_tile + zc : t;
     const int ty = (int)(q % p.TY);
     q /= p.TY;
@@ -395,7 +405,7 @@
       }
     }
   }
-  if (p.pmax) wino_block_max_store(omax, p.pmax);
+  if (p.pmax) wino_block_max_store(omax, p.pmax, p.amax_dst);
   WINO_TL_END(p)
 }
 
@@ -484,7 +494,8 @@
   constexpr int MT = 6, N = 8, EB = VW * 4;
   const int CV = p.Co / VW;
   const long long per_tile = (long long)p.Zo * CV;
-  const long long total = (long long)p.B * p.TX * p.TY * per_tile;
+  const int *vis = p.vis;
+  const long long total = (vis ? (long long)vis[0] : (long long)p.B * p.TX * p.TY) * per_tile;
   const __amdgpu_buffer_rsrc_t rm = __builtin_amdgcn_make_buffer_rsrc((void *)p.Mw, 0, m_bytes, 0x00020000);
   const __amdgpu_buffer_rsrc_t ro = __builtin_amdgcn_make_buffer_rsrc((void *)p.out, 0, out_bytes, 0x00020000);
   const __amdgpu_buffer_rsrc_t rr = __builtin_amdgcn_make_buffer_rsrc((void *)(p.res ? p.res : p.out), 0, p.res ? out_bytes : 0u, 0x00020000);
@@ -496,6 +507,7 @@
     const long long zc = t % per_tile;
     const int cv = (int)(zc % CV);
     long long q = t / per_tile;
+    if (vis) q = vis[1 + q];
     const unsigned vo = (unsigned)((src ? (long long)src[q] * per_tile + zc : t) * EB);
     const int ty = (int)(q % p.TY);
     q /= p.TY;
@@ -540,7 +552,7 @@
       __builtin_amdgcn_sched_barrier(0);
     }
   }
-  if (p.pmax) wino_block_max_store(omax, p.pmax);
+  if (p.pmax) wino_block_max_store(omax, p.pmax, p.amax_dst);
   WINO_TL_END(p)
 }
 
@@ -730,15 +742,67 @@
   if (tid == 0) { blk[0] = na + nk; blk[1] = (na + nk) * p.zo[l]; blk[2] = na; blk[3] = nk; }
 }
 
-struct WinoBgLayout { int64_t z1, scratch, layers, lstride, total, nb; int n; };
+struct WinoBgNeedP {
+  int *layers;
+  unsigned char *mark;
+  int B, TX, TY, nl, lstride, nb;
+  int next[WINO_BG_MAXL], resof[WINO_BG_MAXL], dense[WINO_BG_MAXL];
+};
+__global__ __launch_bounds__(1024) void wino_bg_need_kernel(const WinoBgNeedP p) {
+  __shared__ int wsum[16];
+  __shared__ unsigned char mlds[WINO_BG_LDS_TILES];
+  const int tid = threadIdx.x, l = blockIdx.x;
+  const int n = p.B * p.TX * p.TY;
+  int *vis = p.layers + (size_t)l * p.lstride + WINO_BG_HDR + 2 * (size_t)n;
+  bool all = false;
+  for (int c = l; c >= 0 && c < p.nl; c = p.resof[c])
+    if (p.dense[c]) { all = true; break; }
+  if (all) {
+    for (int t = tid; t < n; t += 1024) vis[1 + t] = t;
+    if (tid == 0) vis[0] = n;
+    return;
+  }
+  unsigned char *mk = n <= WINO_BG_LDS_TILES ? mlds : p.mark + (size_t)l * p.nb;
+  for (int t = tid; t < n; t += 1024) mk[t] = 0;
+  __syncthreads();
+  for (int c = l; c >= 0 && c < p.nl; c = p.resof[c]) {
+    const int *cb = p.layers + (size_t)c * p.lstride;
+    for (int i = cb[2] + tid; i < cb[0]; i += 1024) mk[cb[WINO_BG_HDR + i]] = 1;
+    if (p.next[c] && c + 1 < p.nl) {
+      const int *nb = p.layers + (size_t)(c + 1) * p.lstride;
+      for (int i = tid; i < nb[0]; i += 1024) {
+        const int t = nb[WINO_BG_HDR + i];
+        const int ty = t % p.TY, tx = (t / p.TY) % p.TX, b0 = t - tx * p.TY - ty;
+        for (int dx = -1; dx <= 1; ++dx)
+          for (int dy = -1; dy <= 1; ++dy) {
+            const int xx = tx + dx, yy = ty + dy;
+            if ((unsigned)xx < (unsigned)p.TX && (unsigned)yy < (unsigned)p.TY) mk[b0 + xx * p.TY + yy] = 1;
+          }
+      }
+    }
+  }
+  __syncthreads();
+  const int chunk = (n + 1023) / 1024;
+  const int t0 = min(tid * chunk, n), t1 = min(t0 + chunk, n);
+  int cnt = 0;
+  for (int t = t0; t < t1; ++t) cnt += mk[t] != 0;
+  int nv;
+  int o = wino_bg_scan(cnt, wsum, &nv);
+  for (int t = t0; t < t1; ++t)
+    if (mk[t]) vis[1 + o++] = t;
+  if (tid == 0) vis[0] = nv;
+}
+
+struct WinoBgLayout { int64_t z1, scratch, layers, lstride, mark, total, nb; int n; };
 WinoBgLayout wino_bg_layout(int B, int TX, int TY, int n_layers) {
   WinoBgLayout L;
   L.n = B * TX * TY;
   L.nb = ivx_align_up((int64_t)L.n, 256);
   L.z1 = 0; L.scratch = L.nb;
   L.layers = L.nb + (L.n <= WINO_BG_LDS_TILES ? 0 : 2 * (int64_t)WINO_BG_MAXL * L.nb);
-  L.lstride = ivx_align_up((int64_t)(WINO_BG_HDR + 2 * (int64_t)L.n) * 4, 256) / 4;
-  L.total = L.layers + (int64_t)n_layers * L.lstride * 4;
+  L.lstride = ivx_align_up((int64_t)(WINO_BG_HDR + 3 * (int64_t)L.n + 1) * 4, 256) / 4;
+  L.mark = L.layers + (int64_t)n_layers * L.lstride * 4;
+  L.total = L.mark + (L.n <= WINO_BG_LDS_TILES ? 0 : (int64_t)n_layers * L.nb);
   return L;
 }
 unsigned wino_blocks(int64_t items) {
@@ -832,6 +896,7 @@
   p->post_scale = d->post_scale == 0.f ? 1.0f : d->post_scale;
   p->pmax = nullptr;
   p->bg = nullptr;
+  p->vis = nullptr; p->amax_dst = nullptr; p->hdr_copy = nullptr;
 #ifdef IVX_CONV_TIMELINE
   p->tl = g_wino_timeline;
 #endif
@@ -851,7 +916,8 @@
 }
 
 static int wino_input_impl(const ivx_conv_desc *d, int32_t tile, const void *in, void *workspace, int64_t workspace_bytes,
-                           const float *partials, int32_t n_partials, const int32_t *bg, ivx_stream_t stream) {
+                           const float *partials, int32_t n_partials, const int32_t *bg, ivx_stream_t stream, bool ready = false,
+                           const void *amax_word = nullptr) {
   WinoDims w;
   WinoP p;
   float dummy;
@@ -860,7 +926,16 @@
   if (rc != IVX_OK) return rc;
   if ((rc = wino_bg_check(d, tile, bg, "ivx_conv_winograd_input")) != IVX_OK) return rc;
   p.bg = bg;
-  if (d->wino_operands == IVX_F16_PAIR) {
+  if (d->wino_operands == IVX_F16_PAIR && ready) {
+    if (amax_word) {
+      p.hdr_copy = const_cast<unsigned *>(p.hdr);
+      p.hdr = (const unsigned *)amax_word;
+    }
+    if (tile == 4)
+      hipLaunchKernelGGL((wino_input_kernel<4, 2, 1>), dim3(wino_blocks(w.v_elems / 2)), dim3(256), 0, (hipStream_t)stream, p);
+    else
+      hipLaunchKernelGGL((wino_input_kernel<6, 2, 1>), dim3(wino_blocks(w.v_elems / 2)), dim3(256), 0, (hipStream_t)stream, p);
+  } else if (d->wino_operands == IVX_F16_PAIR) {
     static const bool one_wg = !(getenv("IVX_WINO_AMAX_ONE_WG") && atoi(getenv("IVX_WINO_AMAX_ONE_WG")) == 0);
     const bool write_form = partials && n_partials <= 65536 && one_wg;
     if (!write_form && hipMemsetAsync((void *)p.hdr, 0, 4, (hipStream_t)stream) != hipSuccess) {
@@ -910,6 +985,21 @@
                                           const float *partials, int32_t n_partials, const int32_t *bg, ivx_stream_t stream) {
   IVX_REQUIRE(!partials || n_partials > 0, "ivx_conv_winograd_input_bg: partials without a count");
   return wino_input_impl(d, tile, in, workspace, workspace_bytes, partials, n_partials, bg, stream);
+}
+
+extern "C" void *ivx_conv_winograd_amax_word(const ivx_conv_desc *d, int32_t tile, void *workspace, int64_t workspace_bytes) {
+  WinoDims w;
+  WinoP p;
+  float dummy;
+  if (!d || d->wino_operands != IVX_F16_PAIR) return nullptr;
+  if (wino_setup(d, tile, &dummy, nullptr, nullptr, &dummy, &dummy, workspace, workspace_bytes, &w, &p, "ivx_conv_winograd_amax_word") != IVX_OK) return nullptr;
+  return const_cast<unsigned *>(p.hdr);
+}
+
+extern "C" int ivx_conv_winograd_input_bg_ready(const ivx_conv_desc *d, int32_t tile, const void *in, void *workspace, int64_t workspace_bytes,
+                                                const int32_t *bg, const void *amax_word, ivx_stream_t stream) {
+  IVX_REQUIRE(d && d->wino_operands == IVX_F16_PAIR, "ivx_conv_winograd_input_bg_ready: for IVX_F16_PAIR operands (only they have a scale)");
+  return wino_input_impl(d, tile, in, workspace, workspace_bytes, nullptr, 0, bg, stream, true, amax_word);
 }
 
 static int wino_gemm_impl(const ivx_conv_desc *d, int32_t tile, const float *u, void *workspace, int64_t workspace_bytes, const int32_t *bg,
@@ -1015,17 +1105,22 @@
 }
 
 static int wino_output_impl(const ivx_conv_desc *d, int32_t tile, const float *scale, const float *shift, const void *res, void *out,
-                            void *workspace, int64_t workspace_bytes, float *partials, const int32_t *bg, ivx_stream_t stream) {
+                            void *workspace, int64_t workspace_bytes, float *partials, const int32_t *bg, ivx_stream_t stream, bool need = false,
+                            void *amax_word = nullptr) {
   WinoDims w;
   WinoP p;
   float dummy;
   IVX_REQUIRE(out, "ivx_conv_winograd_output: null argument");
+  IVX_REQUIRE(!need || (bg && tile == 6), "ivx_conv_winograd_output: the need form visits the tiles of a background block (F(6x6,3x3))");
+  IVX_REQUIRE(!amax_word || partials, "ivx_conv_winograd_output: the in-launch reduction goes with the partial maxima");
   IVX_REQUIRE(!d || d->res_mode == 0 || res, "ivx_conv_winograd_output: res_mode set but res is NULL");
   int rc = wino_setup(d, tile, &dummy, scale, shift, res, out, workspace, workspace_bytes, &w, &p, "ivx_conv_winograd_output");
   if (rc != IVX_OK) return rc;
   if ((rc = wino_bg_check(d, tile, bg, "ivx_conv_winograd_output")) != IVX_OK) return rc;
   p.pmax = partials;
   p.bg = bg;
+  if (need) p.vis = bg + WINO_BG_HDR + 2 * (int64_t)d->B * w.TX * w.TY;
+  p.amax_dst = (unsigned *)amax_word;
   if (tile == 2)
     hipLaunchKernelGGL((wino_output_kernel<2, 4>), dim3(wino_blocks(w.m_elems / 4)), dim3(256), 0, (hipStream_t)stream, p);
   else if (tile == 4)
@@ -1066,6 +1161,12 @@
   return wino_output_impl(d, tile, scale, shift, res, out, workspace, workspace_bytes, partials, bg, stream);
 }
 
+extern "C" int ivx_conv_winograd_output_bg_need(const ivx_conv_desc *d, int32_t tile, const float *scale, const float *shift, const void *res,
+                                                void *out, void *workspace, int64_t workspace_bytes, float *partials, const int32_t *bg,
+                                                int32_t need, void *amax_word, ivx_stream_t stream) {
+  return wino_output_impl(d, tile, scale, shift, res, out, workspace, workspace_bytes, partials, bg, stream, need != 0, amax_word);
+}
+
 extern "C" int ivx_conv_winograd_bg_supported(const ivx_conv_desc *d, int32_t tile) {
   WinoDims w;
   if (tile != 6 || !d || d->pd != 1 || d->ph != 1 || !ivx_conv_winograd_supported(d, tile)) return 0;
@@ -1090,8 +1191,14 @@
   return L.layers + (int64_t)layer * L.lstride * 4;
 }
 
-extern "C" int ivx_conv_winograd_bg_plan(const ivx_conv_desc *d, const uint8_t *valid, int32_t n_layers, const int32_t *out_slices, void *block,
-                                         int64_t block_bytes, ivx_stream_t stream) {
+extern "C" int64_t ivx_conv_winograd_bg_visit_offset(const ivx_conv_desc *d) {
+  WinoDims w;
+  if (wino_dims(d, 6, &w, "ivx_conv_winograd_bg_visit_offset") != IVX_OK) return -1;
+  return (int64_t)(WINO_BG_HDR + 2 * (int64_t)d->B * w.TX * w.TY) * 4;
+}
+
+extern "C" int ivx_conv_winograd_bg_plan_ex(const ivx_conv_desc *d, const uint8_t *valid, int32_t n_layers, const int32_t *out_slices,
+                                            const int32_t *consumers, void *block, int64_t block_bytes, ivx_stream_t stream) {
   WinoDims w;
   int rc = wino_dims(d, 6, &w, "ivx_conv_winograd_bg_plan");
   if (rc != IVX_OK) return rc;
@@ -1112,9 +1219,26 @@
   for (int l = 0; l < WINO_BG_MAXL; ++l) p.zo[l] = l < n_layers ? out_slices[l] : 0;
   hipLaunchKernelGGL(wino_bg_z1_kernel, dim3((unsigned)((L.n + 3) / 4)), dim3(256), 0, (hipStream_t)stream, valid, d->B, d->D, d->H, d->W, w.TX, w.TY,
                      (unsigned char *)(base + L.z1));
+  WinoBgNeedP q;
+  q.layers = p.layers; q.mark = (unsigned char *)(base + L.mark);
+  q.B = d->B; q.TX = w.TX; q.TY = w.TY; q.nl = n_layers; q.lstride = (int)L.lstride; q.nb = (int)L.nb;
+  for (int l = 0; l < WINO_BG_MAXL; ++l) {
+    q.next[l] = 0; q.resof[l] = -1; q.dense[l] = 1;
+    if (l >= n_layers || !consumers) continue;
+    q.next[l] = consumers[3 * l] != 0; q.resof[l] = consumers[3 * l + 1]; q.dense[l] = consumers[3 * l + 2] != 0;
+    IVX_REQUIRE(!q.next[l] || l + 1 < n_layers, "ivx_conv_winograd_bg_plan: layer %d has no next layer in the chain", l);
+    IVX_REQUIRE(q.resof[l] == -1 || (q.resof[l] > l && q.resof[l] < n_layers),
+                "ivx_conv_winograd_bg_plan: layer %d: a residual reader is a later layer of the chain (or -1)", l);
+  }
   hipLaunchKernelGGL(wino_bg_plan_kernel, dim3((unsigned)n_layers), dim3(1024), 0, (hipStream_t)stream, p);
+  hipLaunchKernelGGL(wino_bg_need_kernel, dim3((unsigned)n_layers), dim3(1024), 0, (hipStream_t)stream, q);
   IVX_CHECK_LAUNCH("ivx_conv_winograd_bg_plan");
   return IVX_OK;
+}
+
+extern "C" int ivx_conv_winograd_bg_plan(const ivx_conv_desc *d, const uint8_t *valid, int32_t n_layers, const int32_t *out_slices, void *block,
+                                         int64_t block_bytes, ivx_stream_t stream) {
+  return ivx_conv_winograd_bg_plan_ex(d, valid, n_layers, out_slices, nullptr, block, block_bytes, stream);
 }
 
 extern "C" int ivx_conv_winograd_fwd(const ivx_conv_desc *d, int32_t tile, const void *in, const float *u, const float *scale,
diff --git a/imvoxelnet_amd/ops.py b/imvoxelnet_amd/ops.py
--- a/imvoxelnet_amd/ops.py
+++ b/imvoxelnet_amd/ops.py
@@ -229,6 +229,68 @@
         off = L.ivx_conv_winograd_bg_layer_offset(C.byref(d), l)
         views.append(block[off:off + 4 * (4 + 2 * n)].view(torch.int32))
     return block, views
+
+
+def winograd_bg_plan_need(valid, x_shape, Cout, out_slices, consumers, wgt_layout=1, operands=IVX_F16_PAIR):
+    B, X, Y, Z, Cin = x_shape
+    if tuple(valid.shape) != (B, X, Y, Z) or not valid.is_cuda or not valid.is_contiguous() or valid.element_size() != 1:
+        raise ValueError('valid must be a contiguous [B,X,Y,Z] one-byte device tensor')
+    d = _wino_desc(B, X, Y, Z, Cin, Cout, 3, 1, (1, 1, 1), False, wgt_layout, operands=operands)
+    L = _lib.lib()
+    nl = len(out_slices)
+    nb = L.ivx_conv_winograd_bg_bytes(C.byref(d), nl)
+    if nb < 0:
+        check(-1, 'ivx_conv_winograd_bg_bytes')
+    block = torch.zeros((nb,), device=valid.device, dtype=torch.uint8)
+    zo = (C.c_int32 * nl)(*[int(z) for z in out_slices])
+    cons = None
+    if consumers is not None:
+        if len(consumers) != nl:
+            raise ValueError('one (next, residual of, other) triple per layer')
+        cons = (C.c_int32 * (3 * nl))(*[int(v) for c in consumers for v in c])
+    check(L.ivx_conv_winograd_bg_plan_ex(C.byref(d), _ptr(valid), nl, zo, cons, _ptr(block), nb, _stream()), 'ivx_conv_winograd_bg_plan_ex')
+    n = B * ((X + 5) // 6) * ((Y + 5) // 6)
+    voff = L.ivx_conv_winograd_bg_visit_offset(C.byref(d))
+    views, visits = [], []
+    for l in range(nl):
+        off = L.ivx_conv_winograd_bg_layer_offset(C.byref(d), l)
+        views.append(block[off:off + 4 * (4 + 2 * n)].view(torch.int32))
+        visits.append(block[off + voff:off + voff + 4 * (1 + n)].view(torch.int32))
+    return block, views, visits
+
+
+def conv_winograd_need_fwd(x, u, scale, shift, stride_w, res, out, ws, bg=None, need=False, amax_in=None, ready=None, word=None,
+                           want_amax=True, wgt_layout=1, relu=True):
+    _chk(x, 'x')
+    _chk(u, 'u')
+    B, D, H, W, Cin = x.shape
+    Cout = u.shape[1]
+    d = _wino_desc(B, D, H, W, Cin, Cout, 3, stride_w, (1, 1, 1), relu, wgt_layout, 1 if res is not None else 0, False, 1.0, IVX_F16_PAIR)
+    L = _lib.lib()
+    wsb = L.ivx_conv_winograd_workspace_bytes(C.byref(d), 6)
+    if wsb < 0:
+        check(-1, 'ivx_conv_winograd_workspace_bytes')
+    if ws.dtype != torch.uint8 or ws.numel() < wsb or not ws.is_cuda:
+        raise ValueError(f'ws must be a uint8 device tensor of at least {wsb} bytes')
+    _chk(out, 'out')
+    part = None
+    if want_amax:
+        part = torch.empty((L.ivx_conv_winograd_output_blocks(C.byref(d), 6),), device=x.device, dtype=torch.float32)
+    if ready is not None:
+        check(L.ivx_conv_winograd_input_bg_ready(C.byref(d), 6, _ptr(x), _ptr(ws), ws.numel(), _ptr(bg), _ptr(ready), _stream()),
+              'ivx_conv_winograd_input_bg_ready')
+    else:
+        check(L.ivx_conv_winograd_input_bg(C.byref(d), 6, _ptr(x), _ptr(ws), ws.numel(), _ptr(amax_in), 0 if amax_in is None else amax_in.numel(),
+                                           _ptr(bg), _stream()), 'ivx_conv_winograd_input_bg')
+    check(L.ivx_conv_winograd_gemm_bg(C.byref(d), 6, _ptr(u), _ptr(ws), ws.numel(), _ptr(bg), _stream()), 'ivx_conv_winograd_gemm_bg')
+    hp = L.ivx_conv_winograd_amax_word(C.byref(d), 6, _ptr(ws), ws.numel())
+    if not hp:
+        check(-1, 'ivx_conv_winograd_amax_word')
+    ho = hp - ws.data_ptr()
+    hdr = ws[ho:ho + 8].view(torch.int32).clone()
+    check(L.ivx_conv_winograd_output_bg_need(C.byref(d), 6, _ptr(scale), _ptr(shift), _ptr(res), _ptr(out), _ptr(ws), ws.numel(), _ptr(part), _ptr(bg),
+                                             1 if need else 0, _ptr(word), _stream()), 'ivx_conv_winograd_output_bg_need')
+    return out, part, hdr
 
 
 def conv_winograd_fwd(x, u, scale=None, shift=None, kw=3, stride_w=1, padding=(1, 1, 1), relu=False, res=None, out=None,
diff --git a/include/imvoxel.h b/include/imvoxel.h
--- a/include/imvoxel.h
+++ b/include/imvoxel.h
@@ -159,6 +159,15 @@
                               const int32_t *bg, ivx_stream_t stream);
 int ivx_conv_winograd_output_bg(const ivx_conv_desc *d, int32_t tile, const float *scale, const float *shift, const void *res, void *out,
                                 void *workspace, int64_t workspace_bytes, float *partials, const int32_t *bg, ivx_stream_t stream);
+int ivx_conv_winograd_bg_plan_ex(const ivx_conv_desc *d, const uint8_t *valid, int32_t n_layers, const int32_t *out_slices,
+                                 const int32_t *consumers, void *block, int64_t block_bytes, ivx_stream_t stream);
+int64_t ivx_conv_winograd_bg_visit_offset(const ivx_conv_desc *d);
+int ivx_conv_winograd_output_bg_need(const ivx_conv_desc *d, int32_t tile, const float *scale, const float *shift, const void *res, void *out,
+                                     void *workspace, int64_t workspace_bytes, float *partials, const int32_t *bg, int32_t need,
+                                     void *amax_word, ivx_stream_t stream);
+void *ivx_conv_winograd_amax_word(const ivx_conv_desc *d, int32_t tile, void *workspace, int64_t workspace_bytes);
+int ivx_conv_winograd_input_bg_ready(const ivx_conv_desc *d, int32_t tile, const void *in, void *workspace, int64_t workspace_bytes,
+                                     const int32_t *bg, const void *amax_word, ivx_stream_t stream);
 
 
 int ivx_dcn_im2col_fwd(const float *x, const float *offset_mask, int32_t B, int32_t H, int32_t W, int32_t C, int32_t kh,
```
